# ma921/SOBER

Measured on AMD Instinct MI355X. Metric: recombination-step candidates/sec (N_rec=100000, N_nys=500, d=10, batch=100), higher is better.
Workload: dtype f64

## Files before the change

include/sober_hip.h:

```cpp
#ifndef SOBER_HIP_H
#define SOBER_HIP_H

#include <stdint.h>

#ifdef __cplusplus
extern "C" {
#endif

#define SOBER_ABI_VERSION 7

#define SOBER_KIND_RBF       0
#define SOBER_KIND_MATERN52  1
#define SOBER_KIND_TANIMOTO  2

#define SOBER_E_ARG      -1
#define SOBER_E_DIM      -2
#define SOBER_E_WS       -3
#define SOBER_E_EXCHANGE -5

int sober_abi_version(void);
int sober_diag_build(void);
int sober_reload_switches(void);
int sober_level_job_size(void);
int sober_nystrom_job_size(void);

int sober_padded_dim(int d);
int sober_bit_words(int d);

int sober_mt19937_uniform53(uint8_t* state, int64_t state_bytes, int64_t numel, double* out);
int sober_box_muller(const double* u, int64_t numel, double* out, void* stream);

int sober_scale_points(const double* X, int64_t n, int d, int64_t ldx,
                       const double* lengthscale, int ls_len,
                       double* out, int dt, void* stream);

int sober_scale_points_idx(const double* X, const int32_t* idx, int64_t n, int d, int64_t ldx, const double* lengthscale,
                           int ls_len, double* out, int dt, const double* gather_src, double* gather_out, void* stream);
int sober_pack_bits(const double* X, int64_t n, int d, int64_t ldx,
                    uint64_t* words, int nwords, double* norms, int32_t* bad_flag, void* stream);

int sober_pairwise(int kind, const void* a, const double* a_norm, int64_t m,
                   const void* b, const double* b_norm, const int32_t* idx, int64_t n,
                   int dt, double outputscale, double* out, int64_t ldo, void* stream);

int sober_kernel_matvec(int kind, const void* a, const double* a_norm, const double* v, int64_t m,
                        const void* b, const double* b_norm, int64_t n,
                        int dt, double outputscale, double c0, double* out, void* stream);

int sober_level_reduce(int kind, const void* rows, const double* rows_norm, int n_rows,
                       const void* cand, const double* cand_norm, int dt,
                       const int32_t* idx, int64_t pos0, int64_t count, int S,
                       const double* mu, const double* wmul, double outputscale,
                       int n_chunks, double* partG, int ldg, int col0,
                       double* partTot, int64_t tot_limit, void* stream);
int sober_aug_dim(int d);
int sober_augment_plan(const double* X_nys, int64_t M, int64_t ld_nys, const double* X_obs, int64_t n_obs, int64_t ld_obs,
                       const double* X_cand, int64_t N, int64_t ld_cand, int d, const double* lengthscale, int ls_len,
                       double* center, double* rows_aug, double* cand_aug, int da, void* stream);
int sober_augment_points(const double* X, int64_t n, int d, int64_t ldx, const double* lengthscale,
                         int ls_len, const double* center, int side, double* out, int da, void* stream);
int sober_level_reduce_mfma(int kind, const double* rows, int n_rows, const double* cand, int da,
                            const int32_t* idx, int64_t pos0, int64_t count, int S,
                            const double* mu, const double* wmul, double outputscale,
                            int n_chunks, double* partG, int ldg, int col0,
                            double* partTot, int64_t tot_limit, void* stream);

int64_t sober_nonzero_ws_bytes(int64_t N);
int sober_nonzero_i32(const double* mu, int64_t N, int32_t* idx_out, int64_t* count_out, void* ws, int64_t ws_bytes,
                      void* stream);

int sober_level_chunks(int n_rows, int64_t pos0, int64_t count, int S);
int sober_level_parts_mfma(int n_rows, int64_t pos0, int64_t count, int S);
int sober_level_parts_mfma_cap(int n_rows, int64_t e_total_ub, int S);

int sober_sum_partials(const double* partG, const double* partTot, int n_chunks, int n_rows,
                       int ldg, int S, const double* extraG, const double* extraTot,
                       int n_xchunks, int n_xcols, double* G, int ldo, double* tot, void* stream);

int sober_dgemm(int transa, int transb, int m, int n, int k, double alpha,
                const double* A, int lda, const double* B, int ldb,
                double beta, double* C, int ldc, void* stream);

int sober_barycentres(const double* Xtr, int ldx, int n, int S, const double* tot,
                      double* X_tmp, void* stream);
int sober_dgemm_coldiv_t(int m, int n, int k, const double* A, int lda, const double* B, int ldb, const double* coldiv,
                         double* Ct, int ldct, void* stream);

int sober_level_update(const int32_t* idx_cur, int64_t pos0, int64_t count, int S, int64_t E,
                       const int32_t* keep_rank, const double* w_star, const double* tot,
                       int n_keep, double* mu, int32_t* idx_new, int64_t new_pos0, void* stream);

int sober_scatter_weights(const int32_t* idx_cur, const int32_t* sel, const double* w, int n_sel,
                          double* mu, int64_t* out_idx, void* stream);

int sober_gather_f64(const double* src, const int32_t* idx, int64_t n, double* out, void* stream);
int sober_final_scatter(const int32_t* idx, int n, const int32_t* keep_rank, const double* w_star,
                        int64_t row_offset, double* mu, int64_t* out_idx, double* out_w, void* stream);
int sober_final_commit(const int32_t* idx, int n, const int32_t* keep_rank, const double* w_star, const int32_t* n_keep,
                       int64_t row_offset, double* mu, int64_t N, int64_t* out_idx, double* out_w, void* stream);

int sober_i64_to_i32(const int64_t* in, int64_t n, int32_t* out, void* stream);

int sober_car_pivot_host(double* h_Phi, int N, int m, double* h_mu);
int sober_car_pivot_host_fast(double* h_Phi, int N, int m, double* h_mu);

int sober_car_supported(int N, int m);
int64_t sober_car_ws_bytes(int N, int m);
int sober_car_device(const double* X, int ldx, int N, int m, const double* mu_in,
                     int32_t* keep_rank, double* w_star, int32_t* n_keep, double* mu_out,
                     double* phi_out, void* ws, int64_t ws_bytes, void* stream);
int sober_probe_rcp(const double* x, double* out, int64_t n, void* stream);

#define SOBER_CAR_DEFAULT 0
#define SOBER_CAR_SAFE 1
int sober_car_safe_supported(int N, int m);
int sober_car_giveup_forced(void);
int sober_car_device_ex(const double* X, int ldx, int N, int m, const double* mu_in,
                        int32_t* keep_rank, double* w_star, int32_t* n_keep, double* mu_out,
                        double* phi_out, void* ws, int64_t ws_bytes, int mode, void* stream);
int sober_obj_set_sums(const double* obj, const double* mu, const int32_t* idx, int64_t pos0, int64_t count, int S, int64_t E,
                       double* out, void* stream);
int sober_second_elimination(const double* phi, const double* objp, const double* w1, const int32_t* rank1, int n1,
                             int Nsets, int32_t* keep_rank, double* w_star, int32_t* n_keep, void* stream);
int sober_null_vector_supported(int nfun);
int sober_null_vector(const double* X, int ldx, int Nsets, int nfun, const int32_t* rank1, const int32_t* n_keep1, int n1,
                      double* null_row, int32_t* status, void* stream);
int sober_second_elimination_rows(const double* null_row, const double* obj_row, const double* w1, const int32_t* rank1,
                                  const int32_t* n_keep1, const int32_t* status, int n1, int Nsets, int32_t* keep_rank,
                                  double* w_star, int32_t* n_keep, void* stream);
int sober_obj_set_sums_queued(const double* obj, const double* mu, const int32_t* idx, int S, const int64_t* dR, int64_t R_known,
                              const double* tot, double* xcol, int ldx, double* ocol, void* stream);

int sober_car_mc_supported(int N, int m);
int64_t sober_car_mc_ws_bytes(int N, int m);
int sober_car_mc_device(const double* X, int ldx, int N, int m, const double* mu_in,
                        int32_t* keep_rank, double* w_star, int32_t* n_keep, double* mu_out,
                        double* phi_out, void* ws, int64_t ws_bytes, void* stream);
int sober_car_big_supported(int N, int m);
int64_t sober_car_big_ws_bytes(int N, int m);
int sober_car_big_device(const double* X, int ldx, int N, int m, const double* mu_in,
                         int32_t* keep_rank, double* w_star, int32_t* n_keep, double* mu_out,
                         double* phi_out, void* ws, int64_t ws_bytes, void* stream);
int sober_mc_selftest(const double* in, double* out, void* stream);

int sober_chol_max_n(void);
int sober_nystrom_max_n(void);
int sober_cholesky_probe_batched(const double* src, int n, int ld_src, const double* shifts, int n_shifts,
                                 double* work, int32_t* info, double* min_pivot, void* xinv_ws, int64_t ws_bytes,
                                 void* stream);
int sober_cholesky(double* A, int n, int ld, double shift, int32_t* info, double* min_pivot, void* stream);
int sober_cholesky_inv(double* A, int n, int ld, double shift, int32_t* info, double* min_pivot, double* xinv,
                       void* stream);
int sober_cholesky_inv_ratio(double* A, int n, int ld, double shift, int32_t* info, double* min_pivot, double* xinv,
                             double* ratio_out, void* stream);
int sober_trsm_blocks(const double* Y, int64_t m, int q, int ldy, const double* L, int ldl, const double* Xinv,
                      double* Q, int ldq, void* stream);
int sober_cholesky_probe(const double* src, int n, int ld_src, const double* shifts, int n_shifts,
                         double* work, int32_t* info, void* stream);
int sober_cholesky_probe_piv(const double* src, int n, int ld_src, const double* shifts, int n_shifts,
                             double* work, int32_t* info, double* min_pivot, void* stream);

int64_t sober_cholesky_probe_mc_ws_bytes(int n, int n_shifts);
int sober_cholesky_probe_mc(const double* src, int n, int ld_src, const double* shifts, int n_shifts,
                            double* work, int32_t* info, double* min_pivot, void* ws, int64_t ws_bytes,
                            void* stream);
int sober_abs_sym(const double* C, int n, int ld, double* out, int ldo, int32_t* flag, void* stream);
int sober_abs_sym_dmax(const double* C, int n, int ld, double* out, int ldo, int32_t* flag, double* dmax,
                       void* stream);

int sober_jitter_ladder(double* A, int n, int ld, int k, void* stream);
int sober_jitter_ladder_auto(double* A, int n, int ld, const int32_t* info, int n_rungs, int32_t* k_out,
                             void* stream);

int sober_level_reduce_tani_supported(int dt);
int sober_level_reduce_tani(const void* rows, const double* rows_norm, int n_rows, const void* cand,
                            const double* cand_norm, int dt, const int32_t* idx, int64_t pos0, int64_t count, int S,
                            const double* mu, const double* wmul, double outputscale, int n_chunks, double* partG,
                            int ldg, int col0, double* partTot, int64_t tot_limit, void* stream);

int sober_rank_scatter(const double* X, int ldx, int N, int n, const double* ocol, const int32_t* rank, int n1,
                       double* Xp, double* objp, void* stream);
int sober_set_i64(int64_t* dst, int64_t v, void* stream);

int sober_level_reduce_mfma_queued(int kind, const double* rows, int n_rows, const double* cand, int da,
                                   const int32_t* idx, int64_t count_ub, int S, int S_main, int leftover,
                                   const double* mu, const double* wmul, double outputscale, int n_chunks_ub,
                                   double* partG, int ldg, double* partTot, const int64_t* dR, void* stream);
int sober_level_reduce_mfma_queued_pair(int kind, const double* rows, int n_rows, const double* cand, int da,
                                        const int32_t* idx, int64_t count_ub, int S, int n_xcols, const double* mu,
                                        const double* wmul, double outputscale, int n_chunks_ub, double* partG,
                                        int ldg, double* partTot, int n_xchunks_ub, double* extraG, double* extraTot,
                                        const int64_t* dR, void* stream);
int sober_sum_partials_queued(const double* partG, const double* partTot, int n_rows, int ldg, int S,
                              const double* extraG, const double* extraTot, int n_xcols, double* G, int ldo,
                              double* tot, const int64_t* dR, int chunked, void* stream);
int sober_level_reduce_tani_queued(const void* rows, const double* rows_norm, int n_rows, const void* cand,
                                   const double* cand_norm, int dt, const int32_t* idx, int64_t count_ub, int S,
                                   int S_main, int leftover, const double* mu, const double* wmul, double outputscale,
                                   int n_chunks_ub, double* partG, int ldg, double* partTot, const int64_t* dR,
                                   void* stream);
int sober_level_reduce_tani_queued_pair(const void* rows, const double* rows_norm, int n_rows, const void* cand,
                                        const double* cand_norm, int dt, const int32_t* idx, int64_t count_ub, int S,
                                        int n_xcols, const double* mu, const double* wmul, double outputscale,
                                        int n_chunks_ub, double* partG, int ldg, double* partTot, int n_xchunks_ub,
                                        double* extraG, double* extraTot, const int64_t* dR, void* stream);
int sober_level_chunks_cap(int n_rows, int64_t e_total_ub, int S);
int sober_level_chunks_tani(int n_rows, int64_t pos0, int64_t count, int S);
int sober_level_chunks_tani_cap(int n_rows, int64_t e_total_ub, int S);
int sober_level_update_queued(const int32_t* idx_cur, int64_t R_ub, int S, const int32_t* keep_rank,
                              const double* w_star, const double* tot, double* mu, int32_t* idx_new,
                              const int64_t* dR_cur, int64_t* dR_next, int64_t R_ub_next, void* stream);

int sober_level_class_wpt(int n_rows, int64_t e_total, int S);
int sober_level_class_slots(int wpt);
int sober_level_reduce_mfma_wpt(int kind, const double* rows, int n_rows, const double* cand, int da,
                                const int32_t* idx, int64_t count, int S, const double* mu, const double* wmul,
                                double outputscale, int wpt, int n_chunks, double* partG, int ldg, double* partTot,
                                void* stream);
int sober_class_sum(const double* partG, const double* partTot, int n_chunks, int n_rows, int S, int CL,
                    double* Gc, double* totc, double* G, double* tot, void* stream);
int sober_class_derive_queued(const double* Gc, const double* totc, int n_rows, int S, int CL, const double* scale,
                              const int32_t* sof, double* Gn, double* totn, double* G, double* tot, const int64_t* dR,
                              void* stream);
int sober_level_update_queued_ex(const int32_t* idx_cur, int64_t R_ub, int S, const int32_t* keep_rank,
                                 const double* w_star, const double* tot, double* mu, int32_t* idx_new,
                                 const int64_t* dR_cur, int64_t* dR_next, int64_t R_ub_next, int need_keep,
                                 double* cls_scale, int32_t* cls_sof, int64_t R_known, void* stream);
int sober_level_update_queued_cls(const int32_t* idx_cur, int64_t R_ub, int S, const int32_t* keep_rank,
                                  const double* w_star, const double* tot, double* mu, int32_t* idx_new,
                                  const int64_t* dR_cur, int64_t* dR_next, int64_t R_ub_next, int need_keep,
                                  double* cls_scale, int32_t* cls_sof, void* stream);
#define SOBER_CLASS_MAX_DEPTH 4
int sober_level_class_depth(int variant, int n_rows, int64_t R, int S);

int64_t sober_kmeans_ws_bytes(int64_t N, int d, int K);
int64_t sober_kmeans_stat_offset(int64_t N, int d, int K);
int64_t sober_kmeans_ws_bytes_screened(int64_t N, int d, int K);
int sober_kmeans_lloyd(const double* X, int64_t N, int d, int K, int iters,
                       double* centroids, int32_t* labels, void* ws, int64_t ws_bytes, void* stream);

int sober_predict_fused_supported(int kind, int n_obs, int dt);
int sober_predict_fused(int kind, const void* obs, const double* obs_norm, int n_obs, const void* cand,
                        const double* cand_norm, int64_t N, int dt, double outputscale, const double* W, int ldw,
                        const double* alpha, double c0, double kxx_const, double noise, double* mean_out, double* var_out,
                        double eta, const double* eta_ptr, double* lfi_out, int log_flag, void* stream);
int sober_predict_fused_root(int kind, const void* obs, const double* obs_norm, int n_obs, const void* cand,
                             const double* cand_norm, int64_t N, int dt, double outputscale, const double* St, int ldst,
                             const int32_t* tri_flag, const double* alpha, double c0, double kxx_const, double noise,
                             double* mean_out, double* var_out, double eta, const double* eta_ptr, double* lfi_out, int log_flag,
                             void* stream);
int sober_predict_finish(const double* KX, const double* V, int n_obs, int64_t N, int64_t ld,
                         const double* mean, double kxx_const, const double* norms, double outputscale,
                         double noise, double* var_out, double eta, double* lfi_out, int log_flag,
                         void* stream);

int64_t sober_reduce_ws_bytes(int64_t n);
int sober_cleansing_weights(double* w, int64_t n, double eps, void* ws, int64_t ws_bytes, void* stream);

int sober_wkde_draw(const double* eps, int64_t n, int d, const int32_t* comp, const double* Xobs, int ldx,
                    const double* L, const double* lo, const double* hi, double* x, int32_t* inside,
                    void* stream);

int sober_level_gather(const double* Kmat, int n_rows, int64_t ldk, const int32_t* idx, int64_t pos0,
                       int64_t count, int S, const double* mu, const double* wmul, int n_chunks,
                       double* partG, int ldg, int col0, double* partTot, int64_t tot_limit, void* stream);

int sober_gspace_finish(double* K, const double* corr, int64_t n, int m, int64_t ldk, int64_t ldc,
                        const double* mug_cand, const double* mug_rows, void* stream);

#define SOBER_LEVEL_VALU        0
#define SOBER_LEVEL_MFMA        1
#define SOBER_LEVEL_GATHER      2
#define SOBER_LEVEL_TANI        3
#define SOBER_LEVEL_MAX_CHUNKS  64
#define SOBER_LEVEL_XS          16
typedef struct sober_level_job {
    int32_t variant, kind;
    const void* rows;   const double* rows_norm;
    const void* cand;   const double* cand_norm;
    int32_t n_rows, dim;
    int64_t kmat_ld;
    const double* wmul; double outputscale;
    int32_t S, n;
    const double* P;
    double *partG, *partTot, *extraG, *extraTot;
    double *G, *Xtr, *tot;
    double *X_tmp;
    int32_t* keep_rank;
    double *w_star, *mu_out;
    void* car_ws; int64_t car_ws_bytes;
    int32_t* h_flags;
    void* ev[4];
    const int32_t* idx; int64_t pos0, count, E;
    double* mu;
    int32_t phase;
    int64_t* dR; int64_t* h_dR;
    int32_t car_mode;
    uint64_t ev_used[2];
    int32_t class_depth;
    double* Gc[2]; double* totc[2];
    double* cls_scale; int32_t* cls_sof;
} sober_level_job;
#define SOBER_LEVEL_QUEUE 24
int sober_level_moments(const sober_level_job* job, void* stream);
int sober_level_car(const sober_level_job* job, void* stream);
int sober_level_car_retry(sober_level_job* job, void* stream);
#define SOBER_E_NOPROGRESS -4
int sober_level_loop(sober_level_job* job, int64_t R, int32_t* idx_a, int32_t* idx_b, int first_sums_ready,
                     void** events, int max_levels, int64_t* level_R, int32_t* n_levels, int64_t* R_final,
// ... 90 lines not shown
```

sober_amd/_native.py:

```python
from __future__ import annotations

import ctypes as C
import os
from typing import Optional

import torch

_HERE = os.path.dirname(os.path.abspath(__file__))
LIB_PATH = os.environ.get("SOBER_HIP_LIB") or os.path.join(_HERE, "libsober_hip.so")
ABI_VERSION = 7

KIND_RBF, KIND_MATERN52, KIND_TANIMOTO = 0, 1, 2
KIND_BY_NAME = {"rbf": KIND_RBF, "matern52": KIND_MATERN52, "tanimoto": KIND_TANIMOTO}

_vp, _i32, _i64, _f64 = C.c_void_p, C.c_int, C.c_int64, C.c_double

SIGNATURES = {
    "sober_abi_version": (_i32, []),
    "sober_diag_build": (_i32, []),
    "sober_reload_switches": (_i32, []),
    "sober_level_job_size": (_i32, []),
    "sober_nystrom_job_size": (_i32, []),
    "sober_final_job_size": (_i32, []),
    "sober_set_i64": (_i32, [_vp, _i64, _vp]),
    "sober_rank_scatter": (_i32, [_vp, _i32, _i32, _i32, _vp, _vp, _i32, _vp, _vp, _vp]),
    "sober_plan_rows": (_i32, [_i32, _vp, _i32, _i64, _vp, _i32, _i64, _i32, _vp, _i32, _f64, _vp, _i32, _vp, _i32, _vp,
                               _vp, _vp, _vp, _vp]),
    "sober_level_loop_final": (_i32, [_vp, _vp, _i64, _vp, _vp, _i32, _vp, _i32, _vp, _vp, _vp, _vp, _vp]),
    "sober_padded_dim": (_i32, [_i32]),
    "sober_bit_words": (_i32, [_i32]),
    "sober_scale_points": (_i32, [_vp, _i64, _i32, _i64, _vp, _i32, _vp, _i32, _vp]),
    "sober_augment_plan": (_i32, [_vp, _i64, _i64, _vp, _i64, _i64, _vp, _i64, _i64, _i32, _vp, _i32, _vp, _vp, _vp, _i32, _vp]),
    "sober_scale_points_idx": (_i32, [_vp, _vp, _i64, _i32, _i64, _vp, _i32, _vp, _i32, _vp, _vp, _vp]),
    "sober_pack_bits": (_i32, [_vp, _i64, _i32, _i64, _vp, _i32, _vp, _vp, _vp]),
    "sober_mt19937_uniform53": (_i32, [_vp, _i64, _i64, _vp]),
    "sober_box_muller": (_i32, [_vp, _i64, _vp, _vp]),
    "sober_pairwise": (_i32, [_i32, _vp, _vp, _i64, _vp, _vp, _vp, _i64, _i32, _f64, _vp, _i64, _vp]),
    "sober_kernel_matvec": (_i32, [_i32, _vp, _vp, _vp, _i64, _vp, _vp, _i64, _i32, _f64, _f64, _vp, _vp]),
    "sober_level_reduce": (_i32, [_i32, _vp, _vp, _i32, _vp, _vp, _i32, _vp, _i64, _i64, _i32, _vp, _vp,
                                  _f64, _i32, _vp, _i32, _i32, _vp, _i64, _vp]),
    "sober_nonzero_ws_bytes": (_i64, [_i64]),
    "sober_nonzero_i32": (_i32, [_vp, _i64, _vp, _vp, _vp, _i64, _vp]),
    "sober_dgemm_coldiv_t": (_i32, [_i32, _i32, _i32, _vp, _i32, _vp, _i32, _vp, _vp, _i32, _vp]),
    "sober_level_chunks": (_i32, [_i32, _i64, _i64, _i32]),
    "sober_level_parts_mfma": (_i32, [_i32, _i64, _i64, _i32]),
    "sober_level_parts_mfma_cap": (_i32, [_i32, _i64, _i32]),
    "sober_aug_dim": (_i32, [_i32]),
    "sober_augment_points": (_i32, [_vp, _i64, _i32, _i64, _vp, _i32, _vp, _i32, _vp, _i32, _vp]),
    "sober_level_reduce_mfma": (_i32, [_i32, _vp, _i32, _vp, _i32, _vp, _i64, _i64, _i32, _vp, _vp, _f64, _i32,
                                       _vp, _i32, _i32, _vp, _i64, _vp]),
    "sober_sum_partials": (_i32, [_vp, _vp, _i32, _i32, _i32, _i32, _vp, _vp, _i32, _i32, _vp, _i32, _vp, _vp]),
    "sober_dgemm": (_i32, [_i32, _i32, _i32, _i32, _i32, _f64, _vp, _i32, _vp, _i32, _f64, _vp, _i32, _vp]),
    "sober_barycentres": (_i32, [_vp, _i32, _i32, _i32, _vp, _vp, _vp]),
    "sober_level_update": (_i32, [_vp, _i64, _i64, _i32, _i64, _vp, _vp, _vp, _i32, _vp, _vp, _i64, _vp]),
    "sober_scatter_weights": (_i32, [_vp, _vp, _vp, _i32, _vp, _vp, _vp]),
    "sober_i64_to_i32": (_i32, [_vp, _i64, _vp, _vp]),
    "sober_car_pivot_host": (_i32, [_vp, _i32, _i32, _vp]),
    "sober_car_pivot_host_fast": (_i32, [_vp, _i32, _i32, _vp]),
    "sober_car_supported": (_i32, [_i32, _i32]),
    "sober_car_ws_bytes": (_i64, [_i32, _i32]),
    "sober_car_device": (_i32, [_vp, _i32, _i32, _i32, _vp, _vp, _vp, _vp, _vp, _vp, _vp, _i64, _vp]),
    "sober_probe_rcp": (_i32, [_vp, _vp, _i64, _vp]),
    "sober_second_elimination": (_i32, [_vp, _vp, _vp, _vp, _i32, _i32, _vp, _vp, _vp, _vp]),
    "sober_car_mc_supported": (_i32, [_i32, _i32]),
    "sober_car_mc_ws_bytes": (_i64, [_i32, _i32]),
    "sober_car_mc_device": (_i32, [_vp, _i32, _i32, _i32, _vp, _vp, _vp, _vp, _vp, _vp, _vp, _i64, _vp]),
    "sober_car_big_supported": (_i32, [_i32, _i32]),
    "sober_car_big_ws_bytes": (_i64, [_i32, _i32]),
    "sober_car_big_device": (_i32, [_vp, _i32, _i32, _i32, _vp, _vp, _vp, _vp, _vp, _vp, _vp, _i64, _vp]),
    "sober_car_device_ex": (_i32, [_vp, _i32, _i32, _i32, _vp, _vp, _vp, _vp, _vp, _vp, _vp, _i64, _i32, _vp]),
    "sober_obj_set_sums": (_i32, [_vp, _vp, _vp, _i64, _i64, _i32, _i64, _vp, _vp]),
    "sober_null_vector_supported": (_i32, [_i32]),
    "sober_null_vector": (_i32, [_vp, _i32, _i32, _i32, _vp, _vp, _i32, _vp, _vp, _vp]),
    "sober_second_elimination_rows": (_i32, [_vp, _vp, _vp, _vp, _vp, _vp, _i32, _i32, _vp, _vp, _vp, _vp]),
    "sober_obj_set_sums_queued": (_i32, [_vp, _vp, _vp, _i32, _vp, _i64, _vp, _vp, _i32, _vp, _vp]),
    "sober_obj_job_size": (_i32, []),
    "sober_level_loop_obj": (_i32, [_vp, _vp, _i64, _vp, _vp, _i32, _i32, _vp, _vp, _vp, _vp, _vp]),
    "sober_car_safe_supported": (_i32, [_i32, _i32]),
    "sober_car_giveup_forced": (_i32, []),
    "sober_final_commit": (_i32, [_vp, _i32, _vp, _vp, _vp, _i64, _vp, _i64, _vp, _vp, _vp]),
    "sober_level_car_retry": (_i32, [_vp, _vp]),
    "sober_mc_selftest": (_i32, [_vp, _vp, _vp]),
    "sober_chol_max_n": (_i32, []),
    "sober_nystrom_max_n": (_i32, []),
    "sober_cholesky_probe_batched": (_i32, [_vp, _i32, _i32, _vp, _i32, _vp, _vp, _vp, _vp, _i64, _vp]),
    "sober_cholesky": (_i32, [_vp, _i32, _i32, _f64, _vp, _vp, _vp]),
    "sober_cholesky_inv": (_i32, [_vp, _i32, _i32, _f64, _vp, _vp, _vp, _vp]),
    "sober_cholesky_inv_ratio": (_i32, [_vp, _i32, _i32, _f64, _vp, _vp, _vp, _vp, _vp]),
    "sober_trsm_blocks": (_i32, [_vp, _i64, _i32, _i32, _vp, _i32, _vp, _vp, _i32, _vp]),
    "sober_cholesky_probe": (_i32, [_vp, _i32, _i32, _vp, _i32, _vp, _vp, _vp]),
    "sober_cholesky_probe_piv": (_i32, [_vp, _i32, _i32, _vp, _i32, _vp, _vp, _vp, _vp]),
    "sober_cholesky_probe_mc_ws_bytes": (_i64, [_i32, _i32]),
    "sober_cholesky_probe_mc": (_i32, [_vp, _i32, _i32, _vp, _i32, _vp, _vp, _vp, _vp, _i64, _vp]),
    "sober_abs_sym": (_i32, [_vp, _i32, _i32, _vp, _i32, _vp, _vp]),
    "sober_abs_sym_dmax": (_i32, [_vp, _i32, _i32, _vp, _i32, _vp, _vp, _vp]),
    "sober_jitter_ladder": (_i32, [_vp, _i32, _i32, _i32, _vp]),
    "sober_jitter_ladder_auto": (_i32, [_vp, _i32, _i32, _vp, _i32, _vp, _vp]),
    "sober_kmeans_ws_bytes": (_i64, [_i64, _i32, _i32]),
    "sober_kmeans_stat_offset": (_i64, [_i64, _i32, _i32]),
    "sober_kmeans_ws_bytes_screened": (_i64, [_i64, _i32, _i32]),
    "sober_kmeans_lloyd": (_i32, [_vp, _i64, _i32, _i32, _i32, _vp, _vp, _vp, _i64, _vp]),
    "sober_predict_fused_supported": (_i32, [_i32, _i32, _i32]),
    "sober_predict_fused": (_i32, [_i32, _vp, _vp, _i32, _vp, _vp, _i64, _i32, _f64, _vp, _i32, _vp, _f64, _f64, _f64, _vp, _vp,
                                   _f64, _vp, _vp, _i32, _vp]),
    "sober_predict_fused_root": (_i32, [_i32, _vp, _vp, _i32, _vp, _vp, _i64, _i32, _f64, _vp, _i32, _vp, _vp, _f64, _f64, _f64, _vp,
                                        _vp, _f64, _vp, _vp, _i32, _vp]),
    "sober_predict_finish": (_i32, [_vp, _vp, _i32, _i64, _i64, _vp, _f64, _vp, _f64, _f64, _vp, _f64, _vp, _i32, _vp]),
    "sober_reduce_ws_bytes": (_i64, [_i64]),
    "sober_cleansing_weights": (_i32, [_vp, _i64, _f64, _vp, _i64, _vp]),
    "sober_level_gather": (_i32, [_vp, _i32, _i64, _vp, _i64, _i64, _i32, _vp, _vp, _i32, _vp, _i32, _i32, _vp, _i64,
                                  _vp]),
    "sober_gspace_finish": (_i32, [_vp, _vp, _i64, _i32, _i64, _i64, _vp, _vp, _vp]),
    "sober_wkde_draw": (_i32, [_vp, _i64, _i32, _vp, _vp, _i32, _vp, _vp, _vp, _vp, _vp, _vp]),
    "sober_level_moments": (_i32, [_vp, _vp]),
    "sober_level_car": (_i32, [_vp, _vp]),
    "sober_level_reduce_tani_supported": (_i32, [_i32]),
    "sober_level_reduce_tani": (_i32, [_vp, _vp, _i32, _vp, _vp, _i32, _vp, _i64, _i64, _i32, _vp, _vp, _f64, _i32, _vp,
                                       _i32, _i32, _vp, _i64, _vp]),
    "sober_level_loop_sharded": (_i32, [_vp, _i32, _i32, _vp, _vp, _vp, _i32, _vp, _vp, _i64, _i32, _vp, _vp, _vp, _vp]),
    "sober_rccl_load": (_i32, [C.c_char_p]),
    "sober_rccl_unique_id": (_i32, [_vp]),
    "sober_rccl_comm_init": (_i32, [_vp, _i32, _i32, _vp]),
    "sober_rccl_comm_destroy": (_i32, [_vp]),
    "sober_rccl_allreduce_f64": (_i32, [_vp, _vp, _i64, _vp]),
    "sober_rccl_allreduce_ptr": (_i64, []),
    "sober_peer_region_bytes": (_i64, [_i64]),
    "sober_peer_create": (_i32, [_i32, _i32, _i64, _vp, _vp]),
    "sober_peer_connect": (_i32, [_vp, C.c_char_p]),
    "sober_peer_connect_ptrs": (_i32, [_vp, _vp]),
    "sober_peer_region": (_i64, [_vp]),
    "sober_peer_set_spin_limit": (_i32, [_vp, C.c_uint]),
    "sober_peer_allreduce_f64": (_i32, [_vp, _vp, _i64, _vp]),
    "sober_peer_allreduce_ptr": (_i64, []),
    "sober_peer_status": (_i32, [_vp, _vp, _i64, _vp]),
    "sober_peer_destroy": (_i32, [_vp]),
    "sober_level_reduce_mfma_queued": (_i32, [_i32, _vp, _i32, _vp, _i32, _vp, _i64, _i32, _i32, _i32, _vp, _vp, _f64,
                                              _i32, _vp, _i32, _vp, _vp, _vp]),
    "sober_level_reduce_mfma_queued_pair": (_i32, [_i32, _vp, _i32, _vp, _i32, _vp, _i64, _i32, _i32, _vp, _vp, _f64, _i32,
                                                   _vp, _i32, _vp, _i32, _vp, _vp, _vp, _vp]),
    "sober_sum_partials_queued": (_i32, [_vp, _vp, _i32, _i32, _i32, _vp, _vp, _i32, _vp, _i32, _vp, _vp, _i32, _vp]),
    "sober_level_reduce_tani_queued": (_i32, [_vp, _vp, _i32, _vp, _vp, _i32, _vp, _i64, _i32, _i32, _i32, _vp, _vp, _f64,
                                              _i32, _vp, _i32, _vp, _vp, _vp]),
    "sober_level_reduce_tani_queued_pair": (_i32, [_vp, _vp, _i32, _vp, _vp, _i32, _vp, _i64, _i32, _i32, _vp, _vp, _f64, _i32,
                                                   _vp, _i32, _vp, _i32, _vp, _vp, _vp, _vp]),
    "sober_level_chunks_cap": (_i32, [_i32, _i64, _i32]),
    "sober_level_chunks_tani": (_i32, [_i32, _i64, _i64, _i32]),
    "sober_level_chunks_tani_cap": (_i32, [_i32, _i64, _i32]),
    "sober_level_update_queued": (_i32, [_vp, _i64, _i32, _vp, _vp, _vp, _vp, _vp, _vp, _vp, _i64, _vp]),
    "sober_level_update_queued_ex": (_i32, [_vp, _i64, _i32, _vp, _vp, _vp, _vp, _vp, _vp, _vp, _i64, _i32, _vp, _vp, _i64, _vp]),
    "sober_level_update_queued_cls": (_i32, [_vp, _i64, _i32, _vp, _vp, _vp, _vp, _vp, _vp, _vp, _i64, _i32, _vp, _vp, _vp]),
    "sober_level_class_wpt": (_i32, [_i32, _i64, _i32]),
    "sober_level_class_slots": (_i32, [_i32]),
    "sober_level_class_depth": (_i32, [_i32, _i32, _i64, _i32]),
    "sober_level_reduce_mfma_wpt": (_i32, [_i32, _vp, _i32, _vp, _i32, _vp, _i64, _i32, _vp, _vp, _f64, _i32, _i32, _vp, _i32,
                                           _vp, _vp]),
    "sober_class_sum": (_i32, [_vp, _vp, _i32, _i32, _i32, _i32, _vp, _vp, _vp, _vp, _vp]),
    "sober_class_derive_queued": (_i32, [_vp, _vp, _i32, _i32, _i32, _vp, _vp, _vp, _vp, _vp, _vp, _vp, _vp]),
    "sober_record_event_pair": (_i32, [_vp, _vp, _vp]),
    "sober_set_launch_events": (_i32, [_vp, _vp]),
    "sober_projection": (_i32, [_vp, _i32, _i32, _vp, _vp, _i32, _vp, _vp]),
    "sober_nystrom_flags_bytes": (_i64, [_i32, _i32]),
    "sober_nystrom_basis": (_i32, [_vp, _i32, _vp]),
    "sober_gather_f64": (_i32, [_vp, _vp, _i64, _vp, _vp]),
    "sober_final_scatter": (_i32, [_vp, _i32, _vp, _vp, _i64, _vp, _vp, _vp, _vp]),
    "sober_level_final": (_i32, [_vp, _vp, _vp, _vp, _vp, _i32, _vp, _i32, _i64, _i64, _vp, _vp, _vp, _vp, _vp]),
    "sober_level_final_job": (_i32, [_vp, _vp, _vp, _i32, _vp]),
    "sober_level_loop": (_i32, [_vp, _i64, _vp, _vp, _i32, _vp, _i32, _vp, _vp, _vp, _vp, _vp]),
}

LEVEL_VALU, LEVEL_MFMA, LEVEL_GATHER, LEVEL_TANI = 0, 1, 2, 3
LEVEL_MAX_CHUNKS, LEVEL_XS, LEVEL_QUEUE = 64, 16, 24


class FinalJob(C.Structure):
    _fields_ = [
        ("rows_sc", _vp), ("rows_norm", _vp), ("cand_sc", _vp), ("cand_norm", _vp),
        ("dt", _i32), ("done", _i32), ("N", _i64), ("row_offset", _i64),
        ("K", _vp), ("mu_live", _vp), ("out_idx", _vp), ("out_w", _vp),
        ("cand_raw", _vp), ("ld_raw", _i64), ("d_raw", _i32), ("ls_len", _i32), ("ls", _vp), ("sc_buf", _vp),
    ]


class ObjJob(C.Structure):
    _fields_ = [("obj", _vp), ("X_tmp", _vp), ("ocol", _vp), ("kr1", _vp), ("w1", _vp), ("nk1", _vp), ("null_row", _vp),
                ("status", _vp)]


class NystromJob(C.Structure):
    _fields_ = [
        ("M", _i32), ("s", _i32), ("n_rungs", _i32), ("niter", _i32), ("probe_mc", _i32), ("_pad0", _i32),
        ("G", _vp), ("shifts", _vp), ("R", _vp), ("C", _vp), ("chol_work", _vp),
        ("probe_ws", _vp), ("probe_ws_bytes", _i64),
        ("Y", _vp * 2), ("Gm", _vp), ("xinv", _vp),
        ("flags_block", _vp), ("flags_bytes", _i64), ("h_flags_block", _vp),
        ("Ut", _vp),
        ("T", _vp), ("n_obs", _i32), ("mean_nys", _vp), ("P", _vp),
    ]


class LevelJob(C.Structure):
    _fields_ = [
        ("variant", _i32), ("kind", _i32),
        ("rows", _vp), ("rows_norm", _vp), ("cand", _vp), ("cand_norm", _vp),
        ("n_rows", _i32), ("dim", _i32), ("kmat_ld", _i64),
        ("wmul", _vp), ("outputscale", _f64),
        ("S", _i32), ("n", _i32), ("P", _vp),
        ("partG", _vp), ("partTot", _vp), ("extraG", _vp), ("extraTot", _vp),
        ("G", _vp), ("Xtr", _vp), ("tot", _vp), ("X_tmp", _vp),
        ("keep_rank", _vp), ("w_star", _vp), ("mu_out", _vp),
        ("car_ws", _vp), ("car_ws_bytes", _i64), ("h_flags", _vp),
        ("ev", _vp * 4),
        ("idx", _vp), ("pos0", _i64), ("count", _i64), ("E", _i64), ("mu", _vp),
        ("phase", _i32),
        ("dR", _vp), ("h_dR", _vp),
        ("car_mode", _i32),
        ("ev_used", C.c_uint64 * 2),
        ("class_depth", _i32), ("Gc", _vp * 2), ("totc", _vp * 2), ("cls_scale", _vp), ("cls_sof", _vp),
    ]

E_DIM = -2
E_EXCHANGE = -5
CLASS_MAX_DEPTH = 4
CAR_DEFAULT, CAR_SAFE, CAR_HOST = 0, 1, 2

_lib: Optional[C.CDLL] = None


class SoberHipError(RuntimeError):
    pass


def load() -> C.CDLL:
    global _lib
    if _lib is not None:
        return _lib
    if not os.path.exists(LIB_PATH):
        raise SoberHipError(
            f"{LIB_PATH} not found: build it with `make -C sober_amd/csrc` "
            "(python -c 'import __graft_entry__ as g; g.build()').  sober_amd has no CPU fallback.")
    lib = C.CDLL(LIB_PATH)
    lib.sober_abi_version.restype = _i32
    got = lib.sober_abi_version()
# ... 68 lines not shown

def fused_dim_supported(kind: int, d: int) -> bool:
    r = load().sober_bit_words(d) if kind == KIND_TANIMOTO else load().sober_padded_dim(d)
    return r > 0


def scale_points_idx(X, idx, n, lengthscale, out):
    _req(lengthscale, torch.float64, "lengthscale"); _req(out, torch.float64, "out"); _req(idx, torch.int32, "idx")
    if X.dtype != torch.float64 or X.stride(-1) != 1:
        raise SoberHipError("scale_points_idx: X must be float64 with unit inner stride")
    _check(load().sober_scale_points_idx(X.data_ptr(), idx.data_ptr(), int(n), X.shape[1], X.stride(0), lengthscale.data_ptr(),
                                         lengthscale.numel(), out.data_ptr(), out.shape[1], None, None, _stream(X)),
           "sober_scale_points_idx")


def scale_points(X, lengthscale, out):
    n, d = X.shape
    _req(X, torch.float64, "X"); _req(lengthscale, torch.float64, "lengthscale"); _req(out, torch.float64, "out")
    _check(load().sober_scale_points(X.data_ptr(), n, d, X.stride(0), lengthscale.data_ptr(),
                                     lengthscale.numel(), out.data_ptr(), out.shape[1], _stream(X)),
           "sober_scale_points")


def mt19937_uniform53(state, numel, out):
    _req(state, torch.uint8, "state"); _req(out, torch.float64, "out")
    if state.is_cuda or out.is_cuda or out.numel() < numel + 16:
        raise ValueError("mt19937_uniform53 takes host tensors, out of numel + 16 doubles")
    _check(load().sober_mt19937_uniform53(state.data_ptr(), state.numel(), numel, out.data_ptr()),
           "sober_mt19937_uniform53")


def box_muller(u, numel, out):
    _req(u, torch.float64, "u"); _req(out, torch.float64, "out")
    if u.numel() < numel + 16 or out.numel() < numel:
        raise ValueError("box_muller: u holds numel + 16 uniforms, out numel normals")
    _check(load().sober_box_muller(u.data_ptr(), numel, out.data_ptr(), _stream(out)), "sober_box_muller")


def pack_bits(X, words, norms, bad_flag):
    n, d = X.shape
    _req(X, torch.float64, "X"); _req(words, torch.int64, "words"); _req(norms, torch.float64, "norms")
    _req(bad_flag, torch.int32, "bad_flag")
    _check(load().sober_pack_bits(X.data_ptr(), n, d, X.stride(0), words.data_ptr(), words.shape[1],
                                  norms.data_ptr(), bad_flag.data_ptr(), _stream(X)), "sober_pack_bits")


def rank_scatter(X, n, ocol, rank, n1, Xp, objp):
    _req(X, torch.float64, "X"); _req(ocol, torch.float64, "ocol"); _req(rank, torch.int32, "rank")
    _check(load().sober_rank_scatter(X.data_ptr(), X.stride(0), X.shape[0], n, ocol.data_ptr(), rank.data_ptr(), n1,
                                     Xp.data_ptr(), objp.data_ptr(), _stream(X)), "sober_rank_scatter")


def plan_rows(kind, X_nys, X_obs, lengthscale, outputscale, S_cache, rows, Kall, W, T, G):
    M, d = X_nys.shape
    n_obs = 0 if X_obs is None else X_obs.shape[0]
    for t in (X_nys, X_obs, S_cache, rows, Kall, W, T, G):
        if t is not None and (t.dtype != torch.float64 or t.stride(-1) != 1):
            raise SoberHipError("plan_rows: float64 tensors with unit inner stride")
    _check(load().sober_plan_rows(kind, X_nys.data_ptr(), M, X_nys.stride(0), _ptr(X_obs), n_obs,
                                  X_obs.stride(0) if X_obs is not None else 0, d, lengthscale.data_ptr(),
                                  lengthscale.numel(), float(outputscale), _ptr(S_cache),
                                  S_cache.stride(0) if S_cache is not None else 0, rows.data_ptr(), rows.shape[1],
                                  _ptr(Kall), _ptr(W), _ptr(T), G.data_ptr(), _stream(G)), "sober_plan_rows")


def pairwise(kind, a, a_norm, b, b_norm, idx, n, dt, outputscale, out):
    _check(load().sober_pairwise(kind, a.data_ptr(), _ptr(a_norm), a.shape[0], b.data_ptr(), _ptr(b_norm),
                                 _ptr(idx), n, dt, float(outputscale), out.data_ptr(), out.stride(0),
                                 _stream(out)), "sober_pairwise")


def kernel_matvec(kind, a, a_norm, v, b, b_norm, dt, outputscale, c0, out):
    _check(load().sober_kernel_matvec(kind, a.data_ptr(), _ptr(a_norm), v.data_ptr(), a.shape[0],
                                      b.data_ptr(), _ptr(b_norm), b.shape[0], dt, float(outputscale),
                                      float(c0), out.data_ptr(), _stream(out)), "sober_kernel_matvec")


def nonzero_ws_bytes(N) -> int:
    r = load().sober_nonzero_ws_bytes(N)
    _check(min(int(r), 0), "sober_nonzero_ws_bytes")
    return int(r)


def nonzero_i32(mu, idx_out, count_out, ws):
    _req(mu, torch.float64, "mu"); _req(idx_out, torch.int32, "idx_out"); _req(count_out, torch.int64, "count_out")
    _check(load().sober_nonzero_i32(mu.data_ptr(), mu.numel(), idx_out.data_ptr(), count_out.data_ptr(), ws.data_ptr(),
                                    ws.numel() * ws.element_size(), _stream(mu)), "sober_nonzero_i32")


def level_chunks(n_rows, pos0, count, S) -> int:
    r = load().sober_level_chunks(n_rows, pos0, count, S)
    _check(min(r, 0), "sober_level_chunks")
    return r


def level_parts_mfma(n_rows, pos0, count, S) -> int:
    r = load().sober_level_parts_mfma(n_rows, pos0, count, S)
    _check(min(r, 0), "sober_level_parts_mfma")
    return r


def level_reduce(kind, rows, rows_norm, cand, cand_norm, dt, idx, idx_off, pos0, count, S, mu, wmul,
                 outputscale, n_chunks, partG, ldg, col0, partTot, tot_limit):
    _req(idx, torch.int32, "idx"); _req(mu, torch.float64, "mu")
    _check(load().sober_level_reduce(kind, rows.data_ptr(), _ptr(rows_norm), rows.shape[0], cand.data_ptr(),
                                     _ptr(cand_norm), dt, idx.data_ptr() + 4 * idx_off, pos0, count, S,
                                     mu.data_ptr(), _ptr(wmul), float(outputscale), n_chunks,
                                     partG.data_ptr(), ldg, col0, _ptr(partTot), tot_limit, _stream(mu)),
           "sober_level_reduce")


def aug_dim(d: int) -> int:
    r = load().sober_aug_dim(d)
    return r if r > 0 else -1


def augment_plan(X_nys, X_obs, X_cand, lengthscale, center, rows_aug, cand_aug):
    for t_, nm in ((X_nys, "X_nys"), (X_cand, "X_cand"), (X_obs, "X_obs")):
        if t_ is not None and (t_.dtype != torch.float64 or t_.stride(-1) != 1):
            raise SoberHipError(f"augment_plan: {nm} must be float64 with unit inner stride")
    _req(rows_aug, torch.float64, "rows_aug"); _req(cand_aug, torch.float64, "cand_aug"); _req(center, torch.float64, "center")
    n_obs = 0 if X_obs is None else X_obs.shape[0]
    _check(load().sober_augment_plan(X_nys.data_ptr(), X_nys.shape[0], X_nys.stride(0), _ptr(X_obs), n_obs,
                                     X_obs.stride(0) if n_obs else 0, X_cand.data_ptr(), X_cand.shape[0], X_cand.stride(0),
                                     X_nys.shape[1], lengthscale.data_ptr(), lengthscale.numel(), center.data_ptr(),
                                     rows_aug.data_ptr(), cand_aug.data_ptr(), rows_aug.shape[1], _stream(X_cand)),
           "sober_augment_plan")


def augment_points(X, lengthscale, center, side, out):
    n, d = X.shape
    _req(X, torch.float64, "X"); _req(out, torch.float64, "out"); _req(center, torch.float64, "center")
    _check(load().sober_augment_points(X.data_ptr(), n, d, X.stride(0), lengthscale.data_ptr(),
                                       lengthscale.numel(), center.data_ptr(), side, out.data_ptr(),
                                       out.shape[1], _stream(X)), "sober_augment_points")


def level_reduce_mfma(kind, rows, cand, da, idx, idx_off, pos0, count, S, mu, wmul, outputscale, n_chunks,
                      partG, ldg, col0, partTot, tot_limit):
    _req(idx, torch.int32, "idx"); _req(mu, torch.float64, "mu")
    _check(load().sober_level_reduce_mfma(kind, rows.data_ptr(), rows.shape[0], cand.data_ptr(), da,
                                          idx.data_ptr() + 4 * idx_off, pos0, count, S, mu.data_ptr(),
                                          _ptr(wmul), float(outputscale), n_chunks, partG.data_ptr(), ldg,
                                          col0, _ptr(partTot), tot_limit, _stream(mu)),
           "sober_level_reduce_mfma")


def sum_partials(partG, partTot, n_chunks, n_rows, ldg, S, extraG, extraTot, n_xchunks, n_xcols, G, tot):
    _check(load().sober_sum_partials(partG.data_ptr(), _ptr(partTot), n_chunks, n_rows, ldg, S,
                                     _ptr(extraG), _ptr(extraTot), n_xchunks, n_xcols, G.data_ptr(),
                                     G.stride(0), _ptr(tot), _stream(G)), "sober_sum_partials")


def dgemm(A, B, C_, transa=False, transb=False, alpha=1.0, beta=0.0):
    m, n = C_.shape
    k = A.shape[0] if transa else A.shape[1]
    for t, nm in ((A, "A"), (B, "B"), (C_, "C")):
        if t.dtype != torch.float64 or t.stride(1) != 1:
            raise SoberHipError(f"dgemm {nm}: need float64 with unit inner stride")
    ka = B.shape[1] if transb else B.shape[0]
    ma = A.shape[1] if transa else A.shape[0]
    na = B.shape[0] if transb else B.shape[1]
    if (ma, na, ka) != (m, n, k):
        raise SoberHipError(f"dgemm shape mismatch {A.shape} {B.shape} -> {C_.shape}")
    _check(load().sober_dgemm(int(transa), int(transb), m, n, k, float(alpha), A.data_ptr(), A.stride(0),
                              B.data_ptr(), B.stride(0), float(beta), C_.data_ptr(), C_.stride(0),
                              _stream(C_)), "sober_dgemm")


def barycentres(Xtr, n, S, tot, X_tmp):
    _check(load().sober_barycentres(Xtr.data_ptr(), Xtr.stride(0), n, S, _ptr(tot), X_tmp.data_ptr(),
                                    _stream(X_tmp)), "sober_barycentres")


def level_update(idx_cur, idx_off, pos0, count, S, E, keep_rank, w_star, tot, n_keep, mu, idx_new, new_pos0):
    _check(load().sober_level_update(idx_cur.data_ptr() + 4 * idx_off, pos0, count, S, E,
                                     keep_rank.data_ptr(), w_star.data_ptr(), tot.data_ptr(), n_keep,
                                     mu.data_ptr(), idx_new.data_ptr(), new_pos0, _stream(mu)),
           "sober_level_update")


def scatter_weights(idx_cur, sel, w, n_sel, mu, out_idx):
    _check(load().sober_scatter_weights(idx_cur.data_ptr(), sel.data_ptr(), w.data_ptr(), n_sel,
                                        mu.data_ptr(), out_idx.data_ptr(), _stream(mu)),
           "sober_scatter_weights")


def i64_to_i32(src, dst):
    _check(load().sober_i64_to_i32(src.data_ptr(), src.numel(), dst.data_ptr(), _stream(src)),
           "sober_i64_to_i32")


def car_pivot_host(Phi: torch.Tensor, mu: torch.Tensor, fast=None) -> int:
    if Phi.is_cuda or mu.is_cuda:
        raise SoberHipError("car_pivot_host takes host tensors")
    _req(Phi, torch.float64, "Phi"); _req(mu, torch.float64, "mu")
    N, m = Phi.shape
    fn = load().sober_car_pivot_host_fast if (fast or (fast is None and N > 200)) else load().sober_car_pivot_host
    r = fn(Phi.data_ptr(), N, m, mu.data_ptr())
    _check(min(r, 0), "sober_car_pivot_host")
    return r


_CAR_WS = {}


def car_supported(N: int, m: int) -> bool:
    return bool(load().sober_car_supported(N, m))


def car_safe_supported(N: int, m: int) -> bool:
    return bool(load().sober_car_safe_supported(N, m))


def probe_rcp(x):
    out = torch.empty_like(x)
    _check(load().sober_probe_rcp(x.data_ptr(), out.data_ptr(), x.numel(), _stream(x)), "sober_probe_rcp")
    return out


def car_device(X, mu_in, keep_rank, w_star, n_keep, mu_out, phi_out=None, multi_cu=False, mode=CAR_DEFAULT, big=False):
    N, n = X.shape
    lib = load()
    if mode != CAR_DEFAULT and not multi_cu and not big:
        nbytes = lib.sober_car_ws_bytes(N, n + 1)
        ws = _CAR_WS.get(X.device)
        if ws is None or ws.numel() * 8 < nbytes:
            ws = _CAR_WS[X.device] = torch.empty(max(nbytes // 8, 1), dtype=torch.float64, device=X.device)
        _check(lib.sober_car_device_ex(X.data_ptr(), X.stride(0), N, n + 1, mu_in.data_ptr(), keep_rank.data_ptr(),
                                       w_star.data_ptr(), n_keep.data_ptr(), mu_out.data_ptr(), _ptr(phi_out),
                                       ws.data_ptr(), nbytes, int(mode), _stream(X)), "sober_car_device_ex")
        return
    nbytes = max(lib.sober_car_ws_bytes(N, n + 1), lib.sober_car_mc_ws_bytes(N, n + 1) if multi_cu else 0,
                 lib.sober_car_big_ws_bytes(N, n + 1) if big else 0)
    ws = _CAR_WS.get(X.device)
    if ws is None or ws.numel() * 8 < nbytes:
        ws = torch.empty(max(nbytes // 8, 1), dtype=torch.float64, device=X.device)
        _CAR_WS[X.device] = ws
    fn, name = (lib.sober_car_big_device, "sober_car_big_device") if big else \
        (lib.sober_car_mc_device, "sober_car_mc_device") if multi_cu else (lib.sober_car_device, "sober_car_device")
    _check(fn(X.data_ptr(), X.stride(0), N, n + 1, mu_in.data_ptr(), keep_rank.data_ptr(),
              w_star.data_ptr(), n_keep.data_ptr(), mu_out.data_ptr(), _ptr(phi_out),
              ws.data_ptr(), nbytes, _stream(X)), name)


def obj_set_sums(obj, mu, idx, pos0, count, S, E, out):
    _req(obj, torch.float64, "obj"); _req(mu, torch.float64, "mu"); _req(idx, torch.int32, "idx"); _req(out, torch.float64, "out")
    _check(load().sober_obj_set_sums(obj.data_ptr(), mu.data_ptr(), idx.data_ptr(), int(pos0), int(count), int(S), int(E),
                                     out.data_ptr(), _stream(mu)), "sober_obj_set_sums")


def null_vector(X, nfun, rank1, n_keep1, n1, null_row, status):
    _check(load().sober_null_vector(X.data_ptr(), X.stride(0), X.shape[0], int(nfun), rank1.data_ptr(), n_keep1.data_ptr(),
                                    int(n1), null_row.data_ptr(), status.data_ptr(), _stream(X)), "sober_null_vector")


def second_elimination_rows(null_row, obj_row, w1, rank1, n_keep1, n1, keep_rank, w_star, n_keep, status=None):
    _check(load().sober_second_elimination_rows(null_row.data_ptr(), obj_row.data_ptr(), w1.data_ptr(), rank1.data_ptr(),
                                                n_keep1.data_ptr(), _ptr(status), int(n1), rank1.numel(), keep_rank.data_ptr(),
                                                w_star.data_ptr(), n_keep.data_ptr(), _stream(null_row)),
           "sober_second_elimination_rows")


def level_loop_obj(job, obj_job, R, idx_a, idx_b, first_sums_ready, stream):
    level_R = (_i64 * MAX_LEVELS)()
    n_levels, in_b, R_final = _i32(0), _i32(0), _i64(0)
    _check(load().sober_level_loop_obj(C.addressof(job), C.addressof(obj_job), R, idx_a.data_ptr(), idx_b.data_ptr(),
                                       int(bool(first_sums_ready)), MAX_LEVELS, level_R, C.byref(n_levels), C.byref(R_final),
                                       C.byref(in_b), stream), "sober_level_loop_obj")
    return list(level_R[:n_levels.value]), int(R_final.value), bool(in_b.value)


def second_elimination(phi, objp, w1, rank1, n1, keep_rank, w_star, n_keep):
    _check(load().sober_second_elimination(phi.data_ptr(), objp.data_ptr(), w1.data_ptr(), rank1.data_ptr(), int(n1),
                                           rank1.numel(), keep_rank.data_ptr(), w_star.data_ptr(), n_keep.data_ptr(),
                                           _stream(phi)), "sober_second_elimination")


def mc_selftest(x: torch.Tensor) -> torch.Tensor:
    out = torch.empty(128, dtype=torch.float64, device=x.device)
    _check(load().sober_mc_selftest(x.data_ptr(), out.data_ptr(), _stream(x)), "sober_mc_selftest")
    return out


def chol_max_n() -> int:
    return load().sober_chol_max_n()


def nystrom_max_n() -> int:
    return load().sober_nystrom_max_n()


def cholesky(A, shift, info, min_pivot=None):
    n = A.shape[0]
    _check(load().sober_cholesky(A.data_ptr(), n, A.stride(0), float(shift), info.data_ptr(), _ptr(min_pivot),
                                 _stream(A)), "sober_cholesky")


def cholesky_inv(A, shift, info, min_pivot, xinv, ratio=None):
    n = A.shape[0]
    if xinv.numel() < ((n + 31) // 32) * 1024:
        raise SoberHipError("cholesky_inv: xinv too small")
    _check(load().sober_cholesky_inv_ratio(A.data_ptr(), n, A.stride(0), float(shift), info.data_ptr(), _ptr(min_pivot),
                                           xinv.data_ptr(), _ptr(ratio), _stream(A)), "sober_cholesky_inv")


def trsm_blocks(Y, L, xinv, Q):
    m, q = Y.shape
    _check(load().sober_trsm_blocks(Y.data_ptr(), m, q, Y.stride(0), L.data_ptr(), L.stride(0), xinv.data_ptr(),
                                    Q.data_ptr(), Q.stride(0), _stream(Y)), "sober_trsm_blocks")


def cholesky_probe(src, shifts, work, info, min_pivot=None):
    n = src.shape[0]
    _check(load().sober_cholesky_probe_piv(src.data_ptr(), n, src.stride(0), shifts.data_ptr(), shifts.numel(),
                                           work.data_ptr(), info.data_ptr(), _ptr(min_pivot), _stream(src)),
           "sober_cholesky_probe_piv")


PROBE_NO_VERDICT = -7


def cholesky_probe_mc_ws_bytes(n: int, n_shifts: int) -> int:
    return int(load().sober_cholesky_probe_mc_ws_bytes(n, n_shifts))


def cholesky_probe_mc(src, shifts, work, info, min_pivot, ws):
    n = src.shape[0]
    _check(load().sober_cholesky_probe_mc(src.data_ptr(), n, src.stride(0), shifts.data_ptr(), shifts.numel(),
                                          work.data_ptr(), info.data_ptr(), _ptr(min_pivot), ws.data_ptr(),
                                          ws.numel() * ws.element_size(), _stream(src)), "sober_cholesky_probe_mc")


def abs_sym(C_, out, flag, dmax=None):
    n = C_.shape[0]
    _check(load().sober_abs_sym_dmax(C_.data_ptr(), n, C_.stride(0), out.data_ptr(), out.stride(0), flag.data_ptr(),
                                     _ptr(dmax), _stream(C_)), "sober_abs_sym")


def kmeans_lloyd(X, K, iters, centroids, labels):
    N, d = X.shape
    _req(X, torch.float64, "X"); _req(centroids, torch.float64, "centroids"); _req(labels, torch.int32, "labels")
    nbytes = int(load().sober_kmeans_ws_bytes(N, d, K))
    ws = torch.empty(max(nbytes, 8), dtype=torch.uint8, device=X.device)
    _check(load().sober_kmeans_lloyd(X.data_ptr(), N, d, K, iters, centroids.data_ptr(), labels.data_ptr(),
                                     ws.data_ptr(), nbytes, _stream(X)), "sober_kmeans_lloyd")


def predict_fused_supported(kind: int, n_obs: int, dt: int) -> bool:
    return bool(load().sober_predict_fused_supported(int(kind), int(n_obs), int(dt)))


def predict_fused(kind, obs, obs_norm, cand, cand_norm, n, dt, outputscale, W, alpha, c0, kxx_const, noise, mean_out,
                  var_out, eta=0.0, lfi_out=None, log=False, eta_dev=None, root_tri=None):
    if W.dtype != torch.float64 or W.dim() != 2 or W.stride(1) != 1:
        raise SoberHipError(f"predict_fused: W must be float64 with unit inner stride, got {W.dtype} strides {tuple(W.stride())}")
    if cand.dtype == torch.float64 and (cand.dim() != 2 or cand.stride(1) != 1 or cand.stride(0) != dt):
        raise SoberHipError(f"predict_fused: candidates must be rows of {dt} contiguous float64, got strides {tuple(cand.stride())}")
    for t_, nm in ((alpha, "alpha"), (mean_out, "mean_out"), (var_out, "var_out"), (lfi_out, "lfi_out"), (eta_dev, "eta_dev")):
        if t_ is not None:
            _req(t_, torch.float64, "predict_fused: " + nm)
    if alpha is not None and alpha.numel() != obs.shape[0]:
        raise SoberHipError(f"predict_fused: alpha has {alpha.numel()} entries for {obs.shape[0]} observations")
    if root_tri is not None:
        _req(root_tri, torch.int32, "predict_fused: root_tri")
        if W.shape[0] != W.shape[1] or W.shape[0] != obs.shape[0]:
            raise SoberHipError(f"predict_fused: the root must be {obs.shape[0]} x {obs.shape[0]}, got {tuple(W.shape)}")
        _check(load().sober_predict_fused_root(int(kind), obs.data_ptr(), _ptr(obs_norm), obs.shape[0], cand.data_ptr(),
                                               _ptr(cand_norm), int(n), int(dt), float(outputscale), W.data_ptr(), W.stride(0),
                                               root_tri.data_ptr(), _ptr(alpha), float(c0), float(kxx_const), float(noise),
                                               _ptr(mean_out), var_out.data_ptr(), float(eta), _ptr(eta_dev), _ptr(lfi_out),
                                               int(bool(log)), _stream(cand)), "sober_predict_fused_root")
        return
    _check(load().sober_predict_fused(int(kind), obs.data_ptr(), _ptr(obs_norm), obs.shape[0], cand.data_ptr(),
                                      _ptr(cand_norm), int(n), int(dt), float(outputscale), W.data_ptr(), W.stride(0),
                                      _ptr(alpha), float(c0), float(kxx_const), float(noise), _ptr(mean_out),
                                      var_out.data_ptr(), float(eta), _ptr(eta_dev), _ptr(lfi_out), int(bool(log)),
                                      _stream(cand)),
           "sober_predict_fused")


def predict_finish(KX, V, mean, kxx_const, norms, outputscale, noise, var_out, eta=0.0, lfi_out=None, log=False):
    n_obs, N = KX.shape
    _check(load().sober_predict_finish(KX.data_ptr(), V.data_ptr(), n_obs, N, KX.stride(0), _ptr(mean),
                                       float(kxx_const), _ptr(norms), float(outputscale), float(noise),
                                       var_out.data_ptr(), float(eta), _ptr(lfi_out), int(bool(log)),
                                       _stream(KX)), "sober_predict_finish")


def cleansing_weights(w, eps):
    _req(w, torch.float64, "weights")
    nbytes = load().sober_reduce_ws_bytes(w.numel())
    ws = torch.empty(nbytes // 8 + 1, dtype=torch.float64, device=w.device)
    _check(load().sober_cleansing_weights(w.data_ptr(), w.numel(), float(eps), ws.data_ptr(), nbytes,
                                          _stream(w)), "sober_cleansing_weights")


def wkde_draw(eps, comp, Xobs, L, lo, hi, x, inside):
    n, d = eps.shape
    _check(load().sober_wkde_draw(eps.data_ptr(), n, d, comp.data_ptr(), Xobs.data_ptr(), Xobs.stride(0),
                                  L.data_ptr(), lo.data_ptr() if lo is not None else None,
                                  hi.data_ptr() if hi is not None else None, x.data_ptr(),
                                  inside.data_ptr() if inside is not None else None, _stream(eps)),
           "sober_wkde_draw")


def level_gather(Kmat, idx, idx_off, pos0, count, S, mu, wmul, n_chunks, partG, ldg, col0, partTot, tot_limit):
    _req(idx, torch.int32, "idx"); _req(mu, torch.float64, "mu"); _req(Kmat, torch.float64, "Kmat")
    if Kmat.stride(1) != 1:
        raise SoberHipError("level_gather: Kmat needs unit inner stride")
    _check(load().sober_level_gather(Kmat.data_ptr(), Kmat.shape[1], Kmat.stride(0),
                                     idx.data_ptr() + 4 * idx_off, pos0, count, S, mu.data_ptr(), _ptr(wmul),
                                     n_chunks, partG.data_ptr(), ldg, col0, _ptr(partTot), tot_limit,
                                     _stream(partG)), "sober_level_gather")


def gspace_finish(K, corr, mug_cand, mug_rows):
    n, m = K.shape
    _check(load().sober_gspace_finish(K.data_ptr(), corr.data_ptr(), n, m, K.stride(0), corr.stride(0),
                                      mug_cand.data_ptr(), mug_rows.data_ptr(), _stream(K)), "sober_gspace_finish")


def car_ws_bytes(N: int, m: int) -> int:
    return load().sober_car_ws_bytes(N, m)


def level_moments(job: LevelJob, stream: int):
    _check(load().sober_level_moments(C.addressof(job), stream), "sober_level_moments")


def level_car(job: LevelJob, stream: int):
    _check(load().sober_level_car(C.addressof(job), stream), "sober_level_car")


def level_car_retry(job: LevelJob, stream: int) -> bool:
    rc = load().sober_level_car_retry(C.addressof(job), stream)
    if rc == E_EXCHANGE:
        return False
    _check(rc, "sober_level_car_retry")
    return True


E_NOPROGRESS = -4
MAX_LEVELS = 64


def level_loop(job: LevelJob, R: int, idx_a, idx_b, first_sums_ready: bool, events, stream: int, final: "FinalJob" = None):
    level_R = (_i64 * MAX_LEVELS)()
    n_levels, in_b, R_final = _i32(0), _i32(0), _i64(0)
    ev = None
    if events is not None:
        ev = (_vp * (4 * MAX_LEVELS))(*events)
    if final is not None:
        rc = load().sober_level_loop_final(C.addressof(job), C.addressof(final), R, idx_a.data_ptr(), idx_b.data_ptr(),
                                           int(bool(first_sums_ready)), ev, MAX_LEVELS, level_R, C.byref(n_levels),
                                           C.byref(R_final), C.byref(in_b), stream)
    else:
        rc = load().sober_level_loop(C.addressof(job), R, idx_a.data_ptr(), idx_b.data_ptr(), int(bool(first_sums_ready)),
                                     ev, MAX_LEVELS, level_R, C.byref(n_levels), C.byref(R_final), C.byref(in_b), stream)
    if rc == E_NOPROGRESS:
        raise RuntimeError("recombination made no progress (the Caratheodory step cancelled nothing, "
                           "SOBER/_rchq.py:241-242); the reference would loop forever here")
    if rc != E_EXCHANGE:
# ... 163 lines not shown
```

sober_amd/_ops_nystrom.py:

```python
from __future__ import annotations

import os
import warnings

import torch

from . import _native as nat
from . import _rng
from ._ops_plan import Plan


class _NystromOps:

    NITER = 2

    def nystrom_basis_device(self, p: Plan, s: int, max_iter: int = 10, overlap=None, early=None):
        dev, M = self.device, p.M
        if M > nat.nystrom_max_n() or s > 2 * nat.chol_max_n() or s >= M:
            if s < M:
                self.size_cliff("nystrom", f"N_nys = {M}, batch = {s + 1}: beyond the device Nystrom route (N_nys <= "
                                           f"{nat.nystrom_max_n()}, batch <= {2 * nat.chol_max_n() + 1}); make_cov_psd and svd_lowrank run on host LAPACK "
                                           "instead -- about 5-10x the device route's time for this phase")
            self.gram(p)
            return None
        G = self.gram(p)
        n_r, niter = max_iter + 1, self.NITER
        n_orth2 = 2 * (1 + 2 * niter)
        if getattr(p, "ws", None) is None:
            p.ws = {}
        key = ("nys", M, s, n_r)
        st = self._pin.get(key)
        if st is None:
            f64 = torch.float64
            nbytes = nat.nystrom_flags_bytes(n_r, niter)
            st = self._pin[key] = {
                "job": nat.NystromJob(), "C": torch.empty(M, M, dtype=f64, device=dev),
                "Y0": torch.empty(M, s, dtype=f64, device=dev), "Y1": torch.empty(M, s, dtype=f64, device=dev),
                "Gm": torch.empty(s, s, dtype=f64, device=dev),
                "xinv": torch.empty(((s + 31) // 32) * 1024, dtype=f64, device=dev),
                "flags": torch.empty(nbytes, dtype=torch.uint8, device=dev),
                "h_flags": torch.empty(nbytes, dtype=torch.uint8, pin_memory=True),
                "Ut": torch.empty(s, M, dtype=f64, device=dev),
            }
            skey = ("shifts", n_r)
            if skey not in self._pin:
                self._pin[skey] = torch.tensor([1e-5 * (2 ** k - 1) for k in range(n_r)], dtype=f64, device=dev)
            j = st["job"]
            j.M, j.s, j.n_rungs, j.niter = M, s, n_r, niter
            j.shifts, j.C = self._pin[skey].data_ptr(), st["C"].data_ptr()
            j.Y[0], j.Y[1], j.Gm, j.xinv = st["Y0"].data_ptr(), st["Y1"].data_ptr(), st["Gm"].data_ptr(), st["xinv"].data_ptr()
            j.flags_block, j.flags_bytes, j.h_flags_block = st["flags"].data_ptr(), nbytes, st["h_flags"].data_ptr()
            j.Ut = st["Ut"].data_ptr()
        j = st["job"]
        work = self._buf(p, "chol_work", n_r * M * M)
        j.G, j.chol_work = G.data_ptr(), work.data_ptr()
        j.probe_mc = 1 if (M >= self.PROBE_MC_MIN and n_r <= 16 and self._probe_mc and M <= nat.chol_max_n()) else 0
        if j.probe_mc:
            pws = self._buf_u8(p, "chol_mc_ws", nat.cholesky_probe_mc_ws_bytes(M, n_r))
            j.probe_ws, j.probe_ws_bytes = pws.data_ptr(), pws.numel()
        elif M > nat.chol_max_n():
            pws = self._buf_u8(p, "chol_cb_ws", n_r * 8192)
            j.probe_ws, j.probe_ws_bytes = pws.data_ptr(), pws.numel()
        proj = hasattr(p, "weighted")
        if proj:
            T = p.T
            P = torch.empty(s, p.Mtot if T is not None else M, dtype=torch.float64, device=dev)
            j.T, j.n_obs = nat._ptr(T), (T.shape[1] if T is not None else 0)
            j.mean_nys, j.P = (p.mean_nys.data_ptr() if p.weighted else None), P.data_ptr()
        else:
            j.P = None
        stream = torch.cuda.current_stream(dev)
        nat.nystrom_basis(j, 1, stream.cuda_stream)
        if early is not None:
            early()
        rng_state = torch.get_rng_state()
        R = _rng.device_randn(M, s, dev)
        j.R = R.data_ptr()
        nat.nystrom_basis(j, 2, stream.cuda_stream)
        ev = torch.cuda.Event()
        ev.record(stream)
        Ut = st["Ut"]
        if proj:
            p.P, p.n, p._proj_src = P, s, Ut
        if overlap is not None:
            overlap()
        ev.synchronize()
        hb = st["h_flags"]
        n8 = 8 * (n_r + 1 + n_orth2)
        f64s, i32s = hb[:n8].view(torch.float64), hb[n8:].view(torch.int32)
        piv_h, pivs_rf = f64s[:n_r + 1], f64s[n_r + 1:n_r + 1 + n_orth2]
        flags_h, infos_rf = i32s[:2 + n_r], i32s[2 + n_r:]
        if any(int(v) == nat.PROBE_NO_VERDICT for v in flags_h[2:]):
            self._probe_mc = False
            warnings.warn("sober_amd: the multi-CU Cholesky probe lost contact between its workgroups; "
                          "falling back to one workgroup per rung")
            torch.set_rng_state(rng_state)
            return None
        last = 2 * niter
        if os.environ.get("SOBER_NYSTROM_DEBUG"):
            print("nystrom: pivot ratios of the range finder's blocks", [float(pivs_rf[k + 1]) for k in range(0, n_orth2, 2)])
        single = [k for k in range(0, n_orth2, 2) if k // 2 != last]
        rank_lost = bool((infos_rf != 0).any()) or float(pivs_rf[2 * last + 1]) < 0.5 \
            or any(not (float(pivs_rf[k + 1]) >= self.ORTH1_MIN_RATIO) for k in single)
        if int(flags_h[0]) == 0 or rank_lost or self.ladder_borderline(flags_h[2:], piv_h[:n_r], float(piv_h[n_r])):
            torch.set_rng_state(rng_state)
            return None
        warnings.warn("Estimated covariance matrix was not positive semi-definite. Conveting...")
        return Ut, G

    LADDER_GUARD = 1e-9
    PROBE_MC_MIN = 160

    @classmethod
    def ladder_borderline(cls, info, min_pivot, dmax) -> bool:
        thr = cls.LADDER_GUARD * max(dmax, 0.0)
        ok = [int(v) == 0 for v in info]
        piv = [float(v) for v in min_pivot]
        if not (dmax == dmax) or any(v != v for v in piv):
            return True
        k = ok.index(True) if any(ok) else len(ok)
        if k < len(ok) and piv[k] < thr:
            return True
        if k > 0 and piv[k - 1] > -thr:
            return True
        return False

    def _orth(self, Y, infos, pivs, slot, passes: int = 2):
        q = Y.shape[1]
        for it in range(passes):
            Gm = torch.empty(q, q, dtype=torch.float64, device=self.device)
            nat.dgemm(Y, Y, Gm, transa=True)
            Lc = Gm
            xinv = torch.empty(((q + 31) // 32) * 1024, dtype=torch.float64, device=self.device)
            nat.cholesky_inv(Lc, 0.0, infos[slot + it:slot + it + 1], pivs[slot + it:slot + it + 1], xinv,
                             ratio=pivs[slot + 1:slot + 2] if passes == 1 else None)
            Q = torch.empty_like(Y)
            nat.trsm_blocks(Y, Lc, xinv, Q)
            Y = Q
        return Y

    ORTH1_MIN_RATIO = 1e-10
```

sober_amd/_ops_plan.py:

```python
from __future__ import annotations


import torch

from . import _native as nat
from ._kernel import KernelSpec, PointSet, posterior_mean, prepare_points, woodbury


class Plan:
    _POOL_FIELDS = ("cand", "cand_raw", "cand_aug", "rows_aug", "wmul")

    def __getattr__(self, name):
        if name in Plan._POOL_FIELDS:
            prep = self.__dict__.get("_pool_prep")
            if prep is not None:
                self.__dict__["_pool_prep"] = None
                prep()
                if name in self.__dict__:
                    return self.__dict__[name]
        raise AttributeError(name)



class _PlanOps:

    def build_plan(self, spec: KernelSpec, mode: str, X_nys, X_cand, pool_owner=None) -> Plan:
        p = Plan()
        pool_owner = X_cand if pool_owner is None else pool_owner
        p.spec, p.mode = spec, mode
        p.X_nys_raw, p.X_cand_raw = X_nys, X_cand
        p.kind = nat.KIND_BY_NAME[spec.kind]
        p.M = X_nys.shape[0]
        dev = self.device
        corrected = mode != "kernel"
        p.n_obs = spec.X_obs.shape[0] if corrected else 0
        p.weighted = mode == "weighted_predictive_covariance"
        p.mean_nys = None
        p.T = None
        Xn64 = X_nys.to(torch.float64)
        native_rows = (p.kind != nat.KIND_TANIMOTO and not p.weighted and Xn64.stride(-1) == 1
                       and (not corrected or (spec.X_obs.dtype == torch.float64 and spec.X_obs.stride(-1) == 1
                                              and spec.S_cache.dtype == torch.float64 and spec.S_cache.stride(-1) == 1
                                              and spec.S_cache.dim() == 2
                                              and spec.S_cache.shape[0] == spec.S_cache.shape[1] == spec.X_obs.shape[0])))
        if native_rows:
            f64 = torch.float64
            p.Mtot = p.M + p.n_obs
            dt = nat.padded_dim(X_nys.shape[1], generic=True)
            rows = torch.empty(p.Mtot, dt, dtype=f64, device=dev)
            G = torch.empty(p.M, p.M, dtype=f64, device=dev)
            Kall = W = T = None
            if corrected:
                Kall = torch.empty(p.Mtot, p.M, dtype=f64, device=dev)
                W = torch.empty(p.n_obs, p.n_obs, dtype=f64, device=dev)
                T = torch.empty(p.M, p.n_obs, dtype=f64, device=dev)
            nat.plan_rows(p.kind, Xn64, spec.X_obs if corrected else None, spec.lengthscale, spec.outputscale,
                          spec.S_cache if corrected else None, rows, Kall, W, T, G)
            p.rows = PointSet(rows, None, dt)
            p.T, p._gram = T, G
            if corrected:
                p.Kall = Kall
            stacked = None
        else:
            stacked = torch.cat([Xn64, spec.X_obs], 0) if corrected else X_nys
            p.rows = prepare_points(spec, stacked)
            p.Mtot = len(p.rows)
            if p.weighted:
                p.mean_nys = posterior_mean(spec, p.rows.rows(0, p.M))
            if corrected:
                Kall = torch.empty(p.Mtot, p.M, dtype=torch.float64, device=dev)
                nys = p.rows.rows(0, p.M)
                nat.pairwise(p.kind, p.rows.data, p.rows.norm, nys.data, nys.norm, None, p.M, p.rows.dt,
                             spec.outputscale, Kall)
                p.Kall = Kall
                W = woodbury(spec)
                p.T = torch.empty(p.M, p.n_obs, dtype=torch.float64, device=dev)
                nat.dgemm(Kall[p.M:], W, p.T, transa=True)
        p.da = nat.aug_dim(X_nys.shape[1]) if (p.kind != nat.KIND_TANIMOTO and self.use_mfma) else -1

        def pool_prep():
            Xc64 = X_cand if (X_cand.dtype == torch.float64 and X_cand.stride(-1) == 1) else X_cand.to(torch.float64).contiguous()
            if p.da > 0 and not p.weighted and p.kind != nat.KIND_TANIMOTO and self.lazy_scaled_pool:
                p.cand, p.cand_raw = None, Xc64
            else:
                p.cand = self._packed_pool(spec, X_cand, pool_owner)
                p.cand_raw = None
            p.wmul = self._pool_mean(spec, p.cand, X_cand, pool_owner) if p.weighted else None
            if p.da > 0:
                p.rows_aug = torch.empty(p.Mtot, p.da, dtype=torch.float64, device=dev)
                p.cand_aug = torch.empty(X_cand.shape[0], p.da, dtype=torch.float64, device=dev)
                Xo = spec.X_obs if corrected else None
                if Xn64.shape[1] <= 30 and (Xo is None or (Xo.dtype == torch.float64 and Xo.stride(-1) == 1)):
                    center = torch.empty(Xn64.shape[1], dtype=torch.float64, device=dev)
                    nat.augment_plan(Xn64 if Xn64.stride(-1) == 1 else Xn64.contiguous(), Xo, Xc64, spec.lengthscale, center,
                                     p.rows_aug, p.cand_aug)
                else:
                    st = stacked if stacked is not None else (torch.cat([Xn64, spec.X_obs], 0) if corrected else Xn64)
                    center = Xn64.mean(0).contiguous()
                    nat.augment_points(st.to(torch.float64).contiguous(), spec.lengthscale, center, 0, p.rows_aug)
                    nat.augment_points(Xc64, spec.lengthscale, center, 1, p.cand_aug)
            else:
                p.rows_aug = p.cand_aug = None
        p._pool_prep = pool_prep
        p.P = None
        p.ws = {}
        return p

    def _packed_pool(self, spec, X_cand, owner):
        if spec.kind != "tanimoto":
            return prepare_points(spec, X_cand)
        if not self._shares_storage(X_cand, owner):
            self._pool_cache = None
            return prepare_points(spec, X_cand)
        import weakref
        key = (X_cand.data_ptr(), tuple(X_cand.shape), tuple(X_cand.stride()), X_cand.dtype, X_cand._version,
               owner.data_ptr(), owner._version)
        hit = getattr(self, "_pool_cache", None)
        if hit is not None and hit[0] == key and hit[1]() is owner:
            return hit[2]
        self._pool_cache = None
        pts = prepare_points(spec, X_cand)
        self._pool_cache = (key, weakref.ref(owner), pts)
        return pts

    def _pool_mean(self, spec, cand, X_cand, owner):
        if not self._shares_storage(X_cand, owner):
            self._mean_cache = None
            return posterior_mean(spec, cand)
        key = (X_cand.data_ptr(), tuple(X_cand.shape), tuple(X_cand.stride()), X_cand.dtype, X_cand._version,
               owner.data_ptr(), owner._version,
               id(spec.alpha), spec.alpha._version, id(spec.X_obs), spec.X_obs._version,
               id(spec.lengthscale), spec.lengthscale._version, spec.kind, float(spec.outputscale), float(spec.mean_const))
        hit = getattr(self, "_mean_cache", None)
        if hit is not None and hit[0] == key and hit[1]() is owner and hit[2]() is spec.alpha and hit[3]() is spec.X_obs:
            return hit[4]
        import weakref
        self._mean_cache = None
        out = posterior_mean(spec, cand)
        self._mean_cache = (key, weakref.ref(owner), weakref.ref(spec.alpha), weakref.ref(spec.X_obs), out)
        return out

    @staticmethod
    def _shares_storage(X_cand, owner):
        return (isinstance(owner, torch.Tensor) and owner.device == X_cand.device and owner.dtype == X_cand.dtype
                and owner.data_ptr() == X_cand.data_ptr())

    def clear_cache(self):
        self._pool_cache = None
        self._mean_cache = None

    def gram(self, p: Plan):
        dev = self.device
        G = getattr(p, "_gram", None)
        if G is not None:
            p._gram = None
            return G
        if p.T is None:
            nys = p.rows
            G = torch.empty(p.M, p.M, dtype=torch.float64, device=dev)
            nat.pairwise(p.kind, nys.data, nys.norm, nys.data, nys.norm, None, p.M, nys.dt,
                         p.spec.outputscale, G)
            return G
        G = p.Kall[:p.M].clone()
        nat.dgemm(p.T, p.Kall[p.M:], G, alpha=-1.0, beta=1.0)
        if p.weighted:
            G = p.mean_nys.unsqueeze(1) * G * p.mean_nys.unsqueeze(0)
        return G

    def set_projection(self, p: Plan, U):
        if getattr(p, "_proj_src", None) is U:
            return
        p._proj_src = U
        U = U.to(self.device, torch.float64).contiguous()
        p.n = U.shape[0]
        P = torch.empty(p.n, p.Mtot if p.T is not None else p.M, dtype=torch.float64, device=self.device)
        nat.projection(U, p.mean_nys if p.weighted else None, p.T, P)
        p.P = P
```

sober_amd/csrc/chol.hip:

```cpp
#include "common.hpp"
#include "internal.hpp"

namespace sober {

constexpr int CH_NB = 32;
constexpr int CH_T = 512;
constexpr int CH_LDPP = CH_NB + 4;
constexpr int CH_MAXN = 536;

typedef double ch_double4 __attribute__((ext_vector_type(4)));

constexpr int CH_G = 4;
__device__ double ch_sink[CH_T];
#ifdef CM_STAMPS
__device__ double ch_dbg[2];
#endif

__device__ __forceinline__ double ch_rdlane(double v, int l) {
    return __hiloint2double(__builtin_amdgcn_readlane(__double2hiint(v), l),
                            __builtin_amdgcn_readlane(__double2loint(v), l));
}

template <int NC>
__device__ __attribute__((noinline)) void ch_diag_block_n(double* __restrict__ D, double* __restrict__ Xs, double* __restrict__ s_dinv,
                                              int* __restrict__ s_fail_p, double* __restrict__ s_minp_p, int nb, int kb,
                                              int lane, double* __restrict__ xout) {
    constexpr int LDP = CH_NB + 1;
    int& s_fail = *s_fail_p;
    double& s_minp = *s_minp_p;

            const int i = lane & (CH_NB - 1);
            const bool xh = lane >= CH_NB;
            double v[CH_NB];
#ifdef CM_STAMPS
            const long long dbg0 = wall_clock64();
#endif
#pragma unroll
            for (int c = 0; c < CH_NB; ++c) {
                double dv = D[i * LDP + c];
                asm volatile("" : "+v"(dv));
                v[c] = (xh | (i >= nb)) ? ((c == i) ? 1.0 : 0.0) : dv;
            }
            const bool xw = xout != nullptr && xh;
            double* xo = xw ? xout + (size_t)(kb / CH_NB) * CH_NB * CH_NB : ch_sink;
            const int xo_ld = xw ? CH_NB : 0, xo_i = xw ? i : lane;
            double* const o_base = xh ? Xs + i : D + i * LDP;
            const int o_step = xh ? LDP : 1;
            int fail = 0;
            double minp = s_minp;
#pragma unroll
            for (int j = 0; j < NC; ++j) {
                const double djj = ch_rdlane(v[j], j);
                const bool live = (j < nb) & (fail == 0);
                minp = live ? fmin(minp, djj) : minp;
                fail = (live & !(djj > 0.0)) ? kb + j + 1 : fail;
                double rinv = __builtin_amdgcn_rsq(djj);
                {
                    double h = 0.5 * rinv, e = fma(-(djj * rinv), h, 0.5);
                    rinv = fma(rinv, e, rinv);
                    h = 0.5 * rinv; e = fma(-(djj * rinv), h, 0.5);
                    rinv = fma(rinv, e, rinv);
                }
                double l = djj * rinv;
                l = fma(fma(-l, l, djj), 0.5 * rinv, l);
                const double sc = v[j] * rinv;
                v[j] = xh ? sc : ((i == j) ? l : ((i > j) ? sc : 0.0));
                o_base[j * o_step] = v[j];
                xo[j * xo_ld + xo_i] = v[j];
#pragma unroll
                for (int c = j + 1; c < NC; ++c) {
                    const double lcj = ch_rdlane(v[j], c);
                    v[c] = fma(-v[j], lcj, v[c]);
                }
            }
#pragma unroll
            for (int j = NC; j < CH_NB; ++j) { o_base[j * o_step] = v[j]; xo[j * xo_ld + xo_i] = v[j]; }
            if (lane == 0) { s_fail = fail; s_minp = minp; }
#ifdef CM_STAMPS
            if (lane == 0) { ch_dbg[0] = (double)(wall_clock64() - dbg0); ch_dbg[1] = 0.0; }
#endif
        }

__device__ __forceinline__ void ch_diag_block(double* __restrict__ D, double* __restrict__ Xs, double* __restrict__ s_dinv,
                                              int* __restrict__ s_fail_p, double* __restrict__ s_minp_p, int nb, int kb,
                                              int lane, double* __restrict__ xout) {
    if (nb <= 8) ch_diag_block_n<8>(D, Xs, s_dinv, s_fail_p, s_minp_p, nb, kb, lane, xout);
    else if (nb <= 16) ch_diag_block_n<16>(D, Xs, s_dinv, s_fail_p, s_minp_p, nb, kb, lane, xout);
    else ch_diag_block_n<CH_NB>(D, Xs, s_dinv, s_fail_p, s_minp_p, nb, kb, lane, xout);
}

constexpr int CH_SMALLN = 120;
template <bool SMALL>
__global__ __launch_bounds__(CH_T) void k_chol(double* __restrict__ A, int n, int ld, double shift,
                                              int32_t* __restrict__ info, double* __restrict__ min_pivot,
                                              const double* __restrict__ src, int lds_src,
                                              const double* __restrict__ shifts, double* __restrict__ xout,
                                              double* __restrict__ ratio_out) {
    extern __shared__ double lds[];
    if (src != nullptr) {
        A += (size_t)blockIdx.x * n * ld;
        info += blockIdx.x;
        if (min_pivot) min_pivot += blockIdx.x;
        shift = shifts[blockIdx.x];
        for (int i = threadIdx.x >> 6; i < n; i += CH_T / 64)
            for (int j = threadIdx.x & 63; j <= i; j += 64) A[(size_t)i * ld + j] = src[(size_t)i * lds_src + j];
        __threadfence_block();
        __syncthreads();
    }
    constexpr int LDP = CH_NB + 1;
    double* D = lds;
    double* Xs = lds + CH_NB * LDP;
    constexpr int LDPP = CH_LDPP;
    double* P = lds + 2 * CH_NB * LDP;
    double* const A_glob = A;
    const int ld_glob = ld;
    double* As = nullptr;
    if constexpr (SMALL) {
        As = P + (size_t)(n > CH_NB ? n - CH_NB : 0) * LDPP;
    }
    __shared__ int s_fail;
    __shared__ double s_minp;
    __shared__ double s_dinv[CH_NB];
    const int tid = threadIdx.x, lane = tid & 63, wave = tid >> 6;
    const int li = lane & 15, lk = lane >> 4;
    if (tid == 0) { s_fail = 0; s_minp = __builtin_inf(); }
    __shared__ double s_dm[CH_T / 64];
    if (ratio_out != nullptr) {
        double dl = -__builtin_inf();
        for (int i = tid; i < n; i += CH_T) dl = fmax(dl, A_glob[(size_t)i * ld_glob + i] + shift);
#pragma unroll
        for (int o = 32; o > 0; o >>= 1) dl = fmax(dl, __shfl_xor(dl, o, 64));
        if (lane == 0) s_dm[wave] = dl;
    }
    __syncthreads();
    bool ahead0 = false;
    if constexpr (SMALL) {
        const int nb0 = min(CH_NB, n);
#pragma unroll
        for (int t = tid; t < CH_NB * CH_NB; t += CH_T) {
            const int i = t >> 5, j = t & 31;
            double v = (i < nb0 && j <= i) ? A_glob[(size_t)i * ld_glob + j] : 0.0;
            if (i == j && i < nb0) v += shift;
            D[i * LDP + j] = v;
        }
        __syncthreads();
        if (wave == 0) {
            ch_diag_block(D, Xs, s_dinv, &s_fail, &s_minp, nb0, 0, lane, xout);
        } else {
            for (int i = wave - 1; i < n; i += CH_T / 64 - 1)
                for (int j = lane; j <= i; j += 64) As[i * (n + 1) + j] = A_glob[(size_t)i * ld_glob + j];
        }
        A = As;
        ld = n + 1;
        __syncthreads();
        ahead0 = true;
    }
#ifdef CH_STAMPS
    long long st_t[5] = {0, 0, 0, 0, 0}, st_last = wall_clock64();
#define CH_STAMP(K) { const long long now_ = wall_clock64(); st_t[K] += now_ - st_last; st_last = now_; }
#else
#define CH_STAMP(K)
#endif

    bool ahead = ahead0;
    for (int kb = 0; kb < n; kb += CH_NB) {
        const int nb = min(CH_NB, n - kb);
        const int nr = n - kb - nb;
        if (!ahead) {
#pragma unroll
            for (int t = tid; t < CH_NB * CH_NB; t += CH_T) {
                const int i = t >> 5, j = t & 31;
                double v = (i < nb && j <= i) ? A[(size_t)(kb + i) * ld + kb + j] : 0.0;
                if (i == j && i < nb) v += shift;
                D[i * LDP + j] = v;
            }
            __syncthreads();
            CH_STAMP(0)
            if (wave == 0) ch_diag_block(D, Xs, s_dinv, &s_fail, &s_minp, nb, kb, lane, xout);
            __syncthreads();
            CH_STAMP(1)
        }
        if (s_fail != 0) break;
#pragma unroll
        for (int t = tid; t < CH_NB * CH_NB; t += CH_T) {
            const int i = t >> 5, j = t & 31;
            if (i < nb && j <= i) A[(size_t)(kb + i) * ld + kb + j] = D[i * LDP + j];
        }
        if (nr == 0) break;
        {
            const int ntile = (nr + 15) / 16;
            double af[8], an[8];
            if (wave < ntile) {
                const double* arow = A + (size_t)(kb + nb + min(wave * 16 + li, nr - 1)) * ld + kb;
#pragma unroll
                for (int u = 0; u < 8; ++u) af[u] = arow[min(4 * u + lk, nb - 1)];
            }
            for (int t = wave; t < ntile; t += CH_T / 64) {
                const int r0 = t * 16;
                {
                    const int tn = min(t + CH_T / 64, ntile - 1);
                    const double* arow = A + (size_t)(kb + nb + min(tn * 16 + li, nr - 1)) * ld + kb;
#pragma unroll
                    for (int u = 0; u < 8; ++u) an[u] = arow[min(4 * u + lk, nb - 1)];
                }
                ch_double4 acc0 = (ch_double4){0.0, 0.0, 0.0, 0.0}, acc1 = acc0;
#pragma unroll
                for (int u = 0; u < 8; ++u) {
                    const int k = 4 * u + lk;
                    const double a = (k < nb) ? af[u] : 0.0;
                    acc0 = __builtin_amdgcn_mfma_f64_16x16x4f64(a, Xs[li * LDP + k], acc0, 0, 0, 0);
                    acc1 = __builtin_amdgcn_mfma_f64_16x16x4f64(a, Xs[(16 + li) * LDP + k], acc1, 0, 0, 0);
                }
#pragma unroll
                for (int r = 0; r < 4; ++r) {
                    const int row = r0 + lk + 4 * r;
                    if (row < nr) {
                        P[row * LDPP + li] = acc0[r];
                        P[row * LDPP + 16 + li] = acc1[r];
                    }
                }
#pragma unroll
                for (int u = 0; u < 8; ++u) af[u] = an[u];
            }
        }
        __syncthreads();
        CH_STAMP(2)
        for (int r = tid >> 5; r < nr; r += CH_T / 32) {
            const int j = tid & 31;
            if (j < nb) A[(size_t)(kb + nb + r) * ld + kb + j] = P[r * LDPP + j];
        }
        {
            const int nt = (nr + 15) / 16;
            const int wv = __builtin_amdgcn_readfirstlane(wave);
            const bool look = nt * (nt + 1) / 2 >= 8;
            const int t_step = look ? (wv == 0 ? 1 : CH_T / 64 - 1) : CH_T / 64;
            const int nt_mine = (look && wv == 0) ? min(nt, 2) : nt;
            int ntr = 0, ntc = look ? (wv == 0 ? 0 : 2 + wv) : wv;
            while (ntc > ntr) { ntc -= ntr + 1; ++ntr; }
            int tr[CH_G], tc[CH_G], trn[CH_G], tcn[CH_G];
            double cv[CH_G][4], cn[CH_G][4];
            double* const a22 = A + (size_t)(kb + nb) * ld + kb + nb;
#define CH_TAKE(R, C)                                                       \
            { R = ntr; C = ntc; ntc += t_step; while (ntc > ntr) { ntc -= ntr + 1; ++ntr; } }
#define CH_LOAD(DST, R, C)                                                  \
            _Pragma("unroll") for (int e = 0; e < 4; ++e)                   \
                DST[e] = a22[(size_t)min((R) * 16 + lk + 4 * e, nr - 1) * ld + min((C) * 16 + li, nr - 1)];
#pragma unroll
            for (int g = 0; g < CH_G; ++g) { CH_TAKE(tr[g], tc[g]) CH_LOAD(cv[g], tr[g], tc[g]) }
            while (tr[0] < nt_mine) {
#pragma unroll
                for (int g = 0; g < CH_G; ++g) { CH_TAKE(trn[g], tcn[g]) CH_LOAD(cn[g], trn[g], tcn[g]) }
                ch_double4 acc[CH_G][2];
#pragma unroll
                for (int g = 0; g < CH_G; ++g) {
                    acc[g][0] = (ch_double4){0.0, 0.0, 0.0, 0.0};
                    acc[g][1] = acc[g][0];
                    const int ra = min(tr[g] * 16 + li, nr - 1), rb = min(tc[g] * 16 + li, nr - 1);
#pragma unroll
                    for (int u = 0; u < 8; u += 2) {
                        acc[g][0] = __builtin_amdgcn_mfma_f64_16x16x4f64(P[ra * LDPP + 4 * u + lk],
                                                                         P[rb * LDPP + 4 * u + lk], acc[g][0], 0, 0, 0);
                        acc[g][1] = __builtin_amdgcn_mfma_f64_16x16x4f64(P[ra * LDPP + 4 * u + 4 + lk],
                                                                         P[rb * LDPP + 4 * u + 4 + lk], acc[g][1], 0, 0, 0);
                    }
                }
#pragma unroll
                for (int g = 0; g < CH_G; ++g) {
#pragma unroll
                    for (int e = 0; e < 4; ++e) {
                        const int row = tr[g] * 16 + lk + 4 * e, col = tc[g] * 16 + li;
                        double* dst = (row < nr && col <= row && tr[g] < nt_mine) ? a22 + (size_t)row * ld + col : ch_sink + tid;
                        *dst = cv[g][e] - (acc[g][0][e] + acc[g][1][e]);
                    }
                }
#pragma unroll
                for (int g = 0; g < CH_G; ++g) {
                    tr[g] = trn[g]; tc[g] = tcn[g];
#pragma unroll
                    for (int e = 0; e < 4; ++e) cv[g][e] = cn[g][e];
                }
            }
#undef CH_TAKE
#undef CH_LOAD
            if (look && wave == 0) {
                __builtin_amdgcn_s_waitcnt(0);
                const int kb2 = kb + nb, nb2 = min(CH_NB, n - kb2);
#pragma unroll
                for (int t = lane; t < CH_NB * CH_NB; t += 64) {
                    const int i = t >> 5, j = t & 31;
                    double v = (i < nb2 && j <= i) ? A[(size_t)(kb2 + i) * ld + kb2 + j] : 0.0;
                    if (i == j && i < nb2) v += shift;
                    D[i * LDP + j] = v;
                }
                __builtin_amdgcn_wave_barrier();
                ch_diag_block(D, Xs, s_dinv, &s_fail, &s_minp, nb2, kb2, lane, xout);
            }
            ahead = look;
        }
        __threadfence_block();
        __syncthreads();
        CH_STAMP(3)
    }
    if constexpr (SMALL) {
        __syncthreads();
        for (int i = tid >> 6; i < n; i += CH_T / 64)
            for (int j = tid & 63; j <= i; j += 64) A_glob[(size_t)i * ld_glob + j] = A[i * (n + 1) + j];
    }
#ifdef CH_STAMPS
    {
        CH_STAMP(4)
        if (tid == 0 && n >= 16)
            for (int k = 0; k < 5; ++k) A_glob[8 + k] = (double)st_t[k];
    }
#endif
    if (tid == 0) {
        *info = s_fail;
        if (min_pivot) *min_pivot = s_minp;
        if (ratio_out) {
            double dm = s_dm[0];
#pragma unroll
            for (int w = 1; w < CH_T / 64; ++w) dm = fmax(dm, s_dm[w]);
            *ratio_out = s_minp / dm;
        }
    }
}

constexpr int CM_G = 8;
constexpr int CM_MAXB = (CH_MAXN + CH_NB - 1) / CH_NB;
constexpr unsigned CM_SPIN = 1u << 19;
constexpr unsigned CM_OFF_TICKET = 0, CM_OFF_ERR = 64, CM_HDR = 128;
constexpr unsigned CM_RUNG_BYTES = 1024;
constexpr unsigned CM_OFF_FX = 0, CM_OFF_FP = CM_MAXB * 4, CM_OFF_MP = 768;
static_assert(CM_OFF_FP + CM_MAXB * CM_G * 4 <= CM_OFF_MP && CM_OFF_MP + CM_MAXB * 8 <= CM_RUNG_BYTES, "flag layout");
__device__ __forceinline__ int cm_owner(int j) { const int r = j % (2 * CM_G); return r < CM_G ? r : 2 * CM_G - 1 - r; }
__device__ __forceinline__ int cm_row(int g, int idx) { return (idx >> 1) * 2 * CM_G + ((idx & 1) ? 2 * CM_G - 1 - g : g); }
constexpr int CM_INFO_EXCHANGE = -7;
typedef __amdgpu_buffer_rsrc_t ch_rsrc_t;
typedef unsigned int ch_u32x4 __attribute__((ext_vector_type(4)));

constexpr int CM_POLL = 16 | (int)0x80000000;
__device__ __forceinline__ unsigned cm_poll(ch_rsrc_t rs, unsigned off) {
    unsigned spins = 0, v;
    while ((v = (unsigned)__builtin_amdgcn_raw_buffer_load_b32(rs, off, 0, CM_POLL)) == 0u) {
        if (++spins > CM_SPIN) return 0xffu;
        if ((spins & 255u) == 0u && (unsigned)__builtin_amdgcn_raw_buffer_load_b32(rs, CM_OFF_ERR, 0, CM_POLL) != 0u) return 0xffu;
        __builtin_amdgcn_s_sleep(1);
    }
    return v;
}

__global__ __launch_bounds__(CH_T) void k_chol_mc(double* __restrict__ work, int n, int ld, int32_t* __restrict__ info,
                                                  double* __restrict__ min_pivot, const double* __restrict__ src,
                                                  int lds_src, const double* __restrict__ shifts, int n_rungs,
                                                  unsigned char* ws, unsigned ws_bytes, unsigned x_off) {
    extern __shared__ double lds[];
    constexpr int LDP = CH_NB + 1, LDPP = CH_LDPP;
    double* D = lds;
    double* Xs = lds + CH_NB * LDP;
    double* P = lds + 2 * CH_NB * LDP;
    __shared__ int s_role, s_fail;
    __shared__ double s_minp;
    __shared__ double s_dinv[CH_NB];
    __shared__ unsigned s_flag;
    __shared__ int s_sub;
    int sub_epoch = 0;
    const int tid = threadIdx.x, lane = tid & 63, wave = __builtin_amdgcn_readfirstlane(tid >> 6);
    const int li = lane & 15, lk = lane >> 4;
    const ch_rsrc_t rs = __builtin_amdgcn_make_buffer_rsrc(ws, 0, (int)ws_bytes, 0x00020000);
    if (tid == 0) {
        const unsigned xcc = __builtin_amdgcn_s_getreg(20 | (0 << 6) | (3 << 11)) & 7u;
        const unsigned t = __hip_atomic_fetch_add((unsigned*)(ws + CM_OFF_TICKET) + xcc, 1u, __ATOMIC_RELAXED,
                                                  __HIP_MEMORY_SCOPE_AGENT);
        const unsigned rung = xcc + 8u * (t / CM_G);
        s_role = rung < (unsigned)n_rungs ? (int)(rung * CM_G + t % CM_G) : -1;
        s_fail = 0;
        s_flag = 0u;
        s_sub = 0;
        s_minp = __builtin_inf();
    }
    __syncthreads();
    if (s_role < 0) return;
    const int rung = s_role / CM_G, g = s_role % CM_G;
    const int nblk = (n + CH_NB - 1) / CH_NB;
    if (g >= nblk) return;
    int jmax = g;
    for (int q = 1; cm_row(g, q) < nblk; ++q) jmax = cm_row(g, q);
    double* const A = work + (size_t)rung * n * ld;
    const ch_rsrc_t ra = __builtin_amdgcn_make_buffer_rsrc(A, 0, (int)((size_t)n * ld * sizeof(double)), 0x00020000);
    const double shift = shifts[rung];
    const unsigned fbase = CM_HDR + (unsigned)rung * CM_RUNG_BYTES;
    const unsigned xbase = x_off + (unsigned)rung * CM_MAXB * (CH_NB * CH_NB * 8);
    for (int q = 0; cm_row(g, q) < nblk; ++q) {
        const int j = cm_row(g, q);
        const int r1 = min(n, CH_NB * (j + 1));
        for (int i = CH_NB * j + (tid >> 6); i < r1; i += CH_T / 64)
            for (int c = lane; c <= i; c += 64) A[(size_t)i * ld + c] = src[(size_t)i * lds_src + c];
    }
    __threadfence_block();
    __syncthreads();

#ifdef CM_STAMPS
    long long cs_t[8] = {0, 0, 0, 0, 0, 0, 0, 0}, cs_last = wall_clock64();
#define CM_STAMP(K) { const long long now_ = wall_clock64(); cs_t[K] += now_ - cs_last; cs_last = now_; if (tid == 0 && n >= 480 && k < 16) A[(size_t)g * ld + 300 + 6 * k + K] = (double)now_; }
#else
#define CM_STAMP(K)
#endif
    bool ahead = false;
    int verdict = -1;
    for (int k = 0; k <= jmax; ++k) {
        const int kb = CH_NB * k, nb = min(CH_NB, n - kb);
        const bool own_k = cm_owner(k) == g;
        if (own_k) {
            if (!ahead) {
#pragma unroll
                for (int t = tid; t < CH_NB * CH_NB; t += CH_T) {
                    const int i = t >> 5, j = t & 31;
                    double v = (i < nb && j <= i) ? A[(size_t)(kb + i) * ld + kb + j] : 0.0;
                    if (i == j && i < nb) v += shift;
                    D[i * LDP + j] = v;
                }
                __syncthreads();
                if (wave == 0) ch_diag_block(D, Xs, s_dinv, &s_fail, &s_minp, nb, kb, lane, nullptr);
                __syncthreads();
            }
            if (tid == 0) {
                const double mp = s_minp;
                __builtin_amdgcn_raw_buffer_store_b32(__double2loint(mp), rs, fbase + CM_OFF_MP + 8 * k, 0, 0);
                __builtin_amdgcn_raw_buffer_store_b32(__double2hiint(mp), rs, fbase + CM_OFF_MP + 8 * k + 4, 0, 0);
            }
            if (s_fail != 0 || k == nblk - 1) {
                if (tid == 0) {
                    __builtin_amdgcn_s_waitcnt(0);
                    __builtin_amdgcn_raw_buffer_store_b32(2, rs, fbase + CM_OFF_FX + 4 * k, 0, 0);
                }
                verdict = k;
                break;
            }
            for (int t = tid; t < CH_NB * CH_NB / 2; t += CH_T) {
                const int i = t >> 4, j = (t & 15) * 2;
                ch_u32x4 v;
                v.x = (unsigned)__double2loint(Xs[i * LDP + j]);     v.y = (unsigned)__double2hiint(Xs[i * LDP + j]);
                v.z = (unsigned)__double2loint(Xs[i * LDP + j + 1]); v.w = (unsigned)__double2hiint(Xs[i * LDP + j + 1]);
                __builtin_amdgcn_raw_buffer_store_b128(v, rs, xbase + (unsigned)k * (CH_NB * CH_NB * 8) + (unsigned)t * 16, 0, 0);
            }
            __builtin_amdgcn_s_waitcnt(0);
            __syncthreads();
            if (tid == 0) __builtin_amdgcn_raw_buffer_store_b32(1, rs, fbase + CM_OFF_FX + 4 * k, 0, 0);
        } else {
            if (tid == 0) s_flag = cm_poll(rs, fbase + CM_OFF_FX + 4 * k);
            __syncthreads();
            if (s_flag != 1u) {
                if (s_flag == 0xffu && tid == 0) {
                    __builtin_amdgcn_raw_buffer_store_b32(1, rs, CM_OFF_ERR, 0, 16);
                    info[rung] = CM_INFO_EXCHANGE;
                }
                break;
            }
            for (int t = tid; t < CH_NB * CH_NB / 2; t += CH_T) {
                const int i = t >> 4, j = (t & 15) * 2;
                const ch_u32x4 v = __builtin_amdgcn_raw_buffer_load_b128(rs, xbase + (unsigned)k * (CH_NB * CH_NB * 8) + (unsigned)t * 16, 0, 16);
                Xs[i * LDP + j] = __hiloint2double((int)v.y, (int)v.x);
                Xs[i * LDP + j + 1] = __hiloint2double((int)v.w, (int)v.z);
            }
            __syncthreads();
        }
        CM_STAMP(0)
        ahead = false;
        if (k == jmax) break;
        int i_first = 0;
        while (cm_row(g, i_first) <= k) ++i_first;
        int n_own = 0;
        while (cm_row(g, i_first + n_own) < nblk) ++n_own;
        for (int t = wave; t < 2 * n_own; t += CH_T / 64) {
            const int j = cm_row(g, i_first + (t >> 1)), r0 = CH_NB * j + 16 * (t & 1);
            const double* arow = A + (size_t)min(r0 + li, n - 1) * ld + kb;
            double af[8];
#pragma unroll
// ... 41 lines not shown
                unsigned v = 1u;
                if (jf <= jmax) v = cm_poll(rs, fbase + CM_OFF_FP + 4 * (k * CM_G + o));
                if (v != 1u) s_flag = 0xffu;
            }
        };
        auto gather = [&](int t0, int nthr) {
            for (int cb = k + 1; cb <= jmax; cb += 8)
                for (int gi = t0; gi < CH_NB * CH_NB / 2; gi += nthr) {
                    const int i = gi >> 4, j = (gi & 15) * 2;
                    ch_u32x4 v[8];
#pragma unroll
                    for (int q = 0; q < 8; ++q) {
                        const int c = cb + q, row = min(CH_NB * c + i, n - 1);
                        if (c <= jmax && cm_owner(c) != g)
                            v[q] = __builtin_amdgcn_raw_buffer_load_b128(ra, (unsigned)(((size_t)row * ld + kb + j) * 8), 0, 16);
                    }
#pragma unroll
                    for (int q = 0; q < 8; ++q) {
                        const int c = cb + q, row = CH_NB * c + i;
                        if (c <= jmax && cm_owner(c) != g && row < n) {
                            double* pr = P + (size_t)(row - kb - CH_NB) * LDPP + j;
                            pr[0] = __hiloint2double((int)v[q].y, (int)v[q].x);
                            pr[1] = __hiloint2double((int)v[q].w, (int)v[q].z);
                        }
                    }
                }
        };
        auto walk = [&](int cs0, int wslot, int nwalk) {
            int cs = cs0, ct = wslot;
                int tr[CH_G], tc[CH_G], trn[CH_G], tcn[CH_G];
                double cv[CH_G][4], cn[CH_G][4];
#define CM_TAKE(R, C)                                                                           \
                { while (cs < n_strips && ct > strip_r0(cs) / 16) { ct -= strip_r0(cs) / 16 + 1; ++cs; }   \
                  R = cs < n_strips ? strip_r0(cs) : -1; C = cs < n_strips ? 16 * ct : 0; ct += nwalk; }
#define CM_LOAD(DST, R, C)                                                                      \
                _Pragma("unroll") for (int e = 0; e < 4; ++e)                                   \
                    DST[e] = a22[(size_t)min(max(R, 0) + lk + 4 * e, nr - 1) * ld + min((C) + li, nr - 1)];
#pragma unroll
                for (int q = 0; q < CH_G; ++q) { CM_TAKE(tr[q], tc[q]) CM_LOAD(cv[q], tr[q], tc[q]) }
                while (tr[0] >= 0) {
#pragma unroll
                    for (int q = 0; q < CH_G; ++q) { CM_TAKE(trn[q], tcn[q]) CM_LOAD(cn[q], trn[q], tcn[q]) }
                    ch_double4 acc[CH_G][2];
#pragma unroll
                    for (int q = 0; q < CH_G; ++q) {
                        acc[q][0] = (ch_double4){0.0, 0.0, 0.0, 0.0};
                        acc[q][1] = acc[q][0];
                        const int pa = min(max(tr[q], 0) + li, nr - 1), pb = min(tc[q] + li, nr - 1);
#pragma unroll
                        for (int u = 0; u < 8; u += 2) {
                            acc[q][0] = __builtin_amdgcn_mfma_f64_16x16x4f64(P[pa * LDPP + 4 * u + lk], P[pb * LDPP + 4 * u + lk], acc[q][0], 0, 0, 0);
                            acc[q][1] = __builtin_amdgcn_mfma_f64_16x16x4f64(P[pa * LDPP + 4 * u + 4 + lk], P[pb * LDPP + 4 * u + 4 + lk], acc[q][1], 0, 0, 0);
                        }
                    }
#pragma unroll
                    for (int q = 0; q < CH_G; ++q)
#pragma unroll
                        for (int e = 0; e < 4; ++e) {
                            const int row = tr[q] + lk + 4 * e, col = tc[q] + li;
                            double* dst = (tr[q] >= 0 && row < nr && col <= row) ? a22 + (size_t)row * ld + col : ch_sink + tid;
                            *dst = cv[q][e] - (acc[q][0][e] + acc[q][1][e]);
                        }
#pragma unroll
                    for (int q = 0; q < CH_G; ++q) {
                        tr[q] = trn[q]; tc[q] = tcn[q];
#pragma unroll
                        for (int e = 0; e < 4; ++e) cv[q][e] = cn[q][e];
                    }
                }
#undef CM_TAKE
#undef CM_LOAD
        };
        if (!look) {
            poll_others(tid);
            __syncthreads();
            CM_STAMP(2)
            if (s_flag != 0xffu) gather(tid, CH_T);
            __syncthreads();
            CM_STAMP(3)
            if (s_flag != 0xffu) walk(0, wave, CH_T / 64);
        } else if (wave == 0) {
            __builtin_amdgcn_s_setprio(3);
            const int R0[3] = {0, 16, 16}, C0[3] = {0, 0, 16};
            double cv[3][4];
#pragma unroll
            for (int q = 0; q < 3; ++q)
#pragma unroll
                for (int e = 0; e < 4; ++e)
                    cv[q][e] = a22[(size_t)min(R0[q] + lk + 4 * e, nr - 1) * ld + min(C0[q] + li, nr - 1)];
#pragma unroll
            for (int q = 0; q < 3; ++q) {
                ch_double4 acc0 = (ch_double4){0.0, 0.0, 0.0, 0.0}, acc1 = acc0;
                const int pa = min(R0[q] + li, nr - 1), pb = min(C0[q] + li, nr - 1);
#pragma unroll
                for (int u = 0; u < 8; u += 2) {
                    acc0 = __builtin_amdgcn_mfma_f64_16x16x4f64(P[pa * LDPP + 4 * u + lk], P[pb * LDPP + 4 * u + lk], acc0, 0, 0, 0);
                    acc1 = __builtin_amdgcn_mfma_f64_16x16x4f64(P[pa * LDPP + 4 * u + 4 + lk], P[pb * LDPP + 4 * u + 4 + lk], acc1, 0, 0, 0);
                }
#pragma unroll
                for (int e = 0; e < 4; ++e) {
                    const int row = R0[q] + lk + 4 * e, col = C0[q] + li;
                    double* dst = (row < nr && col <= row) ? a22 + (size_t)row * ld + col : ch_sink + tid;
                    *dst = cv[q][e] - (acc0[e] + acc1[e]);
                }
            }
            __builtin_amdgcn_s_waitcnt(0);
            const int kb2 = kb + CH_NB, nb2 = min(CH_NB, n - kb2);
#pragma unroll
            for (int t = lane; t < CH_NB * CH_NB; t += 64) {
                const int i = t >> 5, j = t & 31;
                double v = (i < nb2 && j <= i) ? A[(size_t)(kb2 + i) * ld + kb2 + j] : 0.0;
                if (i == j && i < nb2) v += shift;
                D[i * LDP + j] = v;
            }
            __builtin_amdgcn_wave_barrier();
            ch_diag_block(D, Xs, s_dinv, &s_fail, &s_minp, nb2, kb2, lane, nullptr);
            __builtin_amdgcn_s_setprio(0);
        } else {
            if (wave == 1) poll_others(lane);
            sub_barrier();
            if (s_flag != 0xffu) gather(tid - 64, CH_T - 64);
            sub_barrier();
            if (s_flag != 0xffu) walk(2, wave - 1, CH_T / 64 - 1);
        }
        CM_STAMP(4)
        ahead = look;
        __threadfence_block();
        __syncthreads();
        CM_STAMP(5)
        if (s_flag == 0xffu) {
            if (tid == 0) {
                __builtin_amdgcn_raw_buffer_store_b32(1, rs, CM_OFF_ERR, 0, 16);
                info[rung] = CM_INFO_EXCHANGE;
            }
            break;
        }
    }
#ifdef CM_STAMPS
    if (tid == 0 && n >= 480) { for (int q = 0; q < 6; ++q) A[(size_t)g * ld + 400 + q] = (double)cs_t[q]; A[(size_t)g * ld + 410] = ch_dbg[0]; A[(size_t)g * ld + 411] = ch_dbg[1]; }
#endif
    if (verdict >= 0 && tid == 0) {
        double mp = s_minp;
        for (int q = 0; q < verdict; ++q) {
            const unsigned lo = (unsigned)__builtin_amdgcn_raw_buffer_load_b32(rs, fbase + CM_OFF_MP + 8 * q, 0, 16);
            const unsigned hi = (unsigned)__builtin_amdgcn_raw_buffer_load_b32(rs, fbase + CM_OFF_MP + 8 * q + 4, 0, 16);
            mp = fmin(mp, __hiloint2double((int)hi, (int)lo));
        }
        info[rung] = s_fail;
        if (min_pivot) min_pivot[rung] = mp;
    }
}

constexpr int TB_WAVES = 2;
__global__ __launch_bounds__(TB_WAVES * 64) void k_trsm_blocks(const double* __restrict__ Y, int64_t m, int q, int ldy,
                                                              const double* __restrict__ L, int ldl,
                                                              const double* __restrict__ Xinv,
                                                              double* __restrict__ Q, int ldq) {
    extern __shared__ double tb_lds[];
    const int lane = threadIdx.x & 63, wave = threadIdx.x >> 6;
    const int li = lane & 15, lk = lane >> 4;
    const int qpad = ((q + 31) / 32) * 32, LS = qpad + 4;
    double* stash = tb_lds + (size_t)wave * (16 * LS + 16 * 36);
    double* tbuf = stash + 16 * LS;
    const int64_t R0 = ((int64_t)blockIdx.x * TB_WAVES + wave) * 16;
    if (R0 >= m) return;
    const int nblk = qpad / 32;
    for (int jb = 0; jb < nblk; ++jb) {
        const int c0 = 32 * jb;
        ch_double4 acc[2];
#pragma unroll
        for (int jt = 0; jt < 2; ++jt)
#pragma unroll
            for (int r = 0; r < 4; ++r) {
                const int64_t row = min(R0 + lk + 4 * r, m - 1);
                const int col = c0 + 16 * jt + li;
                const double v = Y[row * ldy + min(col, q - 1)];
                acc[jt][r] = (col < q) ? v : 0.0;
            }
        for (int kb = 0; kb < jb; ++kb) {
#pragma unroll
            for (int u = 0; u < 8; ++u) {
                const int kc = 32 * kb + 4 * u + lk;
                const double a = -stash[li * LS + kc];
#pragma unroll
                for (int jt = 0; jt < 2; ++jt) {
                    const int lr = c0 + 16 * jt + li;
                    const double b = L[(size_t)min(lr, q - 1) * ldl + kc];
                    acc[jt] = __builtin_amdgcn_mfma_f64_16x16x4f64(a, (lr < q) ? b : 0.0, acc[jt], 0, 0, 0);
                }
            }
        }
#pragma unroll
        for (int jt = 0; jt < 2; ++jt)
#pragma unroll
            for (int r = 0; r < 4; ++r) tbuf[(lk + 4 * r) * 36 + 16 * jt + li] = acc[jt][r];
        __builtin_amdgcn_wave_barrier();
        const double* X = Xinv + (size_t)jb * 32 * 32;
        ch_double4 out[2] = {(ch_double4){0.0, 0.0, 0.0, 0.0}, (ch_double4){0.0, 0.0, 0.0, 0.0}};
#pragma unroll
        for (int u = 0; u < 8; ++u) {
            const double a = tbuf[li * 36 + 4 * u + lk];
#pragma unroll
            for (int jt = 0; jt < 2; ++jt)
                out[jt] = __builtin_amdgcn_mfma_f64_16x16x4f64(a, X[(16 * jt + li) * 32 + 4 * u + lk], out[jt], 0, 0, 0);
        }
        __builtin_amdgcn_wave_barrier();
#pragma unroll
        for (int jt = 0; jt < 2; ++jt)
#pragma unroll
            for (int r = 0; r < 4; ++r) {
                const int64_t row = R0 + lk + 4 * r;
                const int col = c0 + 16 * jt + li;
                stash[(lk + 4 * r) * LS + col] = out[jt][r];
                if (row < m && col < q) Q[row * ldq + col] = out[jt][r];
            }
        __builtin_amdgcn_wave_barrier();
    }
}

__global__ __launch_bounds__(256) void k_abs_sym(const double* __restrict__ C, int n, int ld,
                                                 double* __restrict__ out, int ldo, int32_t* __restrict__ flag,
                                                 unsigned long long* __restrict__ dmax_bits) {
    __shared__ double tm[32][33];
    const int tx = threadIdx.x & 31, ty = threadIdx.x >> 5;
    const int i0 = blockIdx.y * 32, j0 = blockIdx.x * 32;
    for (int r = ty; r < 32; r += 8) {
        const int i = j0 + r, j = i0 + tx;
        tm[r][tx] = (i < n && j < n) ? C[(size_t)i * ld + j] : 0.0;
    }
    __syncthreads();
    bool asym = false;
    const double big = 1.7976931348623157e308;
    for (int r = ty; r < 32; r += 8) {
        const int i = i0 + r, j = j0 + tx;
        if (i < n && j < n) {
            double a = C[(size_t)i * ld + j], b = tm[tx][r];
            asym |= !(a == b);
            a = (a != a) ? 0.0 : fmin(fmax(a, -big), big);
            b = (b != b) ? 0.0 : fmin(fmax(b, -big), big);
            const double v = sqrt(a * b);
            out[(size_t)i * ldo + j] = v;
            if (dmax_bits != nullptr && i == j) atomicMax(dmax_bits, (unsigned long long)__double_as_longlong(v));
        }
    }
    if (__syncthreads_or(asym) && threadIdx.x == 0) atomicOr(flag, 1);
}

__global__ void k_jitter_ladder(double* __restrict__ A, int n, int ld, int k) {
    const int i = blockIdx.x * blockDim.x + threadIdx.x;
    if (i >= n) return;
    double d = A[(size_t)i * ld + i], jit = 1e-5;
    for (int t = 0; t < k; ++t) { d = __dadd_rn(d, jit); jit = __dmul_rn(jit, 2.0); }
    A[(size_t)i * ld + i] = d;
}

__global__ void k_jitter_ladder_auto(double* __restrict__ A, int n, int ld, const int32_t* __restrict__ info,
                                     int n_rungs, int32_t* __restrict__ k_out) {
    const int j = blockIdx.x * blockDim.x + threadIdx.x, i = blockIdx.y;
    int k = 0;
    while (k < n_rungs && info[k] != 0) ++k;
    if (i == 0 && j == 0) *k_out = k;
    if (j >= n) return;
    if (i == j) {
        double d = A[(size_t)i * ld + i], jit = 1e-5;
        for (int t = 0; t < k; ++t) { d = __dadd_rn(d, jit); jit = __dmul_rn(jit, 2.0); }
        A[(size_t)i * ld + i] = d;
    } else if (k == n_rungs) {
        A[(size_t)i * ld + j] = 0.0;
    }
}

}

namespace sober {
__global__ void k_probe_mc_init(uint32_t* __restrict__ ws, int64_t n_words, int32_t* __restrict__ info, int n_info, int32_t value,
                                uint32_t* __restrict__ pre, int64_t n_pre) {
    const int64_t t = (int64_t)blockIdx.x * blockDim.x + threadIdx.x;
    if (t < n_words) ws[t] = 0u;
    if (pre != nullptr) {
        const int64_t i0 = (uint32_t*)info - pre;
        if (t < n_pre && !(t >= i0 && t < i0 + n_info)) pre[t] = 0u;
    }
    if (t < n_info) info[t] = value;
}
}

namespace sober {
constexpr int CB_MAXN = 2048;
constexpr int CB_TILE = 64;

__global__ __launch_bounds__(256) void k_cb_init(double* __restrict__ work, int n, const double* __restrict__ src, int ld_src,
                                                 int32_t* __restrict__ info, double* __restrict__ min_pivot, int n_rungs) {
    const int i = blockIdx.x, rung = blockIdx.y;
    double* A = work + (size_t)rung * n * n;
    for (int c = threadIdx.x; c <= i; c += 256) A[(size_t)i * n + c] = src[(size_t)i * ld_src + c];
    if (i == 0 && threadIdx.x == 0) { info[rung] = 0; if (min_pivot) min_pivot[rung] = __builtin_inf(); }
}

__global__ __launch_bounds__(64) void k_cb_diag(double* __restrict__ work, int n, int kb, const double* __restrict__ shifts,
                                                double* __restrict__ xinv, int32_t* __restrict__ info,
                                                double* __restrict__ min_pivot) {
    constexpr int LDP = CH_NB + 1;
    __shared__ double D[CH_NB * LDP], Xs[CH_NB * LDP], s_dinv[CH_NB];
    __shared__ int s_fail;
    __shared__ double s_minp;
    const int rung = blockIdx.x, lane = threadIdx.x;
    double* A = work + (size_t)rung * n * n;
    const int nb = min(CH_NB, n - kb);
    const double shift = shifts[rung];
#pragma unroll
    for (int t = lane; t < CH_NB * CH_NB; t += 64) {
        const int i = t >> 5, j = t & 31;
        double v = (i < nb && j <= i) ? A[(size_t)(kb + i) * n + kb + j] : 0.0;
        if (i == j && i < nb) v += shift;
        D[i * LDP + j] = v;
    }
    if (lane == 0) { s_fail = 0; s_minp = __builtin_inf(); }
    __syncthreads();
    ch_diag_block(D, Xs, s_dinv, &s_fail, &s_minp, nb, kb, lane, nullptr);
    __syncthreads();
    double* xo = xinv + (size_t)rung * CH_NB * CH_NB;
#pragma unroll
    for (int t = lane; t < CH_NB * CH_NB; t += 64) xo[t] = Xs[(t >> 5) * LDP + (t & 31)];
    if (lane == 0 && info[rung] == 0) {
        if (min_pivot) min_pivot[rung] = fmin(min_pivot[rung], s_minp);
        if (s_fail != 0) info[rung] = s_fail;
    }
}

__global__ __launch_bounds__(256) void k_cb_update(double* __restrict__ work, int n, int kb, const double* __restrict__ xinv) {
    constexpr int LDP = CH_NB + 1, LDPP = CH_LDPP;
    __shared__ double Xs[CH_NB * LDP], Pr[CB_TILE * LDPP], Pc[CB_TILE * LDPP];
    const int rung = blockIdx.y, tid = threadIdx.x, lane = tid & 63, wave = tid >> 6;
    const int li = lane & 15, lk = lane >> 4;
    double* A = work + (size_t)rung * n * n;
    const int base = kb + CH_NB;
    int bi = 0, rest = blockIdx.x;
    while (rest > bi) { rest -= bi + 1; ++bi; }
    const int bj = rest;
    const int R0 = base + CB_TILE * bi, C0 = base + CB_TILE * bj;
    const double* xi = xinv + (size_t)rung * CH_NB * CH_NB;
    for (int t = tid; t < CH_NB * CH_NB; t += 256) Xs[(t >> 5) * LDP + (t & 31)] = xi[t];
    __syncthreads();
#pragma unroll
    for (int side = 0; side < 2; ++side) {
        if (side == 1 && bi == bj) break;
        const int r0 = (side == 0 ? R0 : C0) + 16 * wave;
        const double* arow = A + (size_t)min(r0 + li, n - 1) * n + kb;
        double af[8];
#pragma unroll
        for (int u = 0; u < 8; ++u) af[u] = arow[4 * u + lk];
        ch_double4 acc0 = (ch_double4){0.0, 0.0, 0.0, 0.0}, acc1 = acc0;
#pragma unroll
        for (int u = 0; u < 8; ++u) {
            const int k = 4 * u + lk;
            acc0 = __builtin_amdgcn_mfma_f64_16x16x4f64(af[u], Xs[li * LDP + k], acc0, 0, 0, 0);
            acc1 = __builtin_amdgcn_mfma_f64_16x16x4f64(af[u], Xs[(16 + li) * LDP + k], acc1, 0, 0, 0);
        }
        double* P = side == 0 ? Pr : Pc;
#pragma unroll
        for (int r = 0; r < 4; ++r) {
            const int row = 16 * wave + lk + 4 * r;
            P[row * LDPP + li] = acc0[r];
            P[row * LDPP + 16 + li] = acc1[r];
        }
    }
    __syncthreads();
    const double* Pcol = (bi == bj) ? Pr : Pc;
#pragma unroll
    for (int ct = 0; ct < 4; ++ct) {
        if (bi == bj && ct > wave) break;
        double cv[4];
#pragma unroll
        for (int e = 0; e < 4; ++e)
            cv[e] = A[(size_t)min(R0 + 16 * wave + lk + 4 * e, n - 1) * n + min(C0 + 16 * ct + li, n - 1)];
        ch_double4 acc0 = (ch_double4){0.0, 0.0, 0.0, 0.0}, acc1 = acc0;
        const int pa = 16 * wave + li, pb = 16 * ct + li;
#pragma unroll
        for (int u = 0; u < 8; u += 2) {
            acc0 = __builtin_amdgcn_mfma_f64_16x16x4f64(Pr[pa * LDPP + 4 * u + lk], Pcol[pb * LDPP + 4 * u + lk], acc0, 0, 0, 0);
            acc1 = __builtin_amdgcn_mfma_f64_16x16x4f64(Pr[pa * LDPP + 4 * u + 4 + lk], Pcol[pb * LDPP + 4 * u + 4 + lk], acc1, 0, 0, 0);
        }
#pragma unroll
        for (int e = 0; e < 4; ++e) {
            const int row = R0 + 16 * wave + lk + 4 * e, col = C0 + 16 * ct + li;
            if (row < n && col <= row) A[(size_t)row * n + col] = cv[e] - (acc0[e] + acc1[e]);
        }
    }
}
}

namespace sober {
__global__ void k_orth_merge(int32_t* __restrict__ info, double* __restrict__ piv, double* __restrict__ ratio,
                             const int32_t* __restrict__ info2, const double* __restrict__ piv2, const double* __restrict__ ratio2) {
    if (threadIdx.x != 0 || blockIdx.x != 0) return;
    if (*info == 0) *info = *info2;
    *piv = fmin(*piv, *piv2);
    if (*piv2 != *piv2) *piv = *piv2;
    if (ratio != nullptr) {
        *ratio = fmin(*ratio, *ratio2);
        if (*ratio2 != *ratio2) *ratio = *ratio2;
    }
}
}
int sober::orth_merge(int32_t* info, double* piv, double* ratio, const int32_t* info2, const double* piv2, const double* ratio2,
                      void* stream) {
    if (!info || !piv || !info2 || !piv2 || (ratio && !ratio2)) return SOBER_E_ARG;
    hipLaunchKernelGGL(sober::k_orth_merge, dim3(1), dim3(64), 0, (hipStream_t)stream, info, piv, ratio, info2, piv2, ratio2);
    LAUNCH_CHECK();
    return 0;
}

extern "C" int sober_nystrom_max_n(void) { return sober::CB_MAXN; }

extern "C" int sober_cholesky_probe_batched(const double* src, int n, int ld_src, const double* shifts, int n_shifts,
                                            double* work, int32_t* info, double* min_pivot, void* xinv_ws,
                                            int64_t ws_bytes, void* stream) {
    if (!src || !shifts || !work || !info || !xinv_ws || n <= 0 || ld_src < n || n_shifts <= 0) return SOBER_E_ARG;
    if (n > sober::CB_MAXN || n_shifts > 64) return SOBER_E_DIM;
    if (ws_bytes < (int64_t)n_shifts * sober::CH_NB * sober::CH_NB * 8) return SOBER_E_WS;
    hipStream_t st = (hipStream_t)stream;
    hipLaunchKernelGGL(sober::k_cb_init, dim3(n, n_shifts), dim3(256), 0, st, work, n, src, ld_src, info, min_pivot, n_shifts);
    LAUNCH_CHECK();
    for (int kb = 0; kb < n; kb += sober::CH_NB) {
        hipLaunchKernelGGL(sober::k_cb_diag, dim3(n_shifts), dim3(64), 0, st, work, n, kb, shifts, (double*)xinv_ws, info,
                           min_pivot);
        LAUNCH_CHECK();
        const int rest = n - kb - sober::CH_NB;
        if (rest <= 0) break;
        const int T = (rest + sober::CB_TILE - 1) / sober::CB_TILE;
        hipLaunchKernelGGL(sober::k_cb_update, dim3(T * (T + 1) / 2, n_shifts), dim3(256), 0, st, work, n, kb,
                           (const double*)xinv_ws);
        LAUNCH_CHECK();
    }
    return 0;
}

namespace sober {
}

extern "C" int sober_chol_max_n(void) { return sober::CH_MAXN; }

extern "C" int sober_cholesky_inv_ratio(double* A, int n, int ld, double shift, int32_t* info, double* min_pivot,
                                        double* xinv, double* ratio_out, void* stream);
extern "C" int sober_cholesky_inv(double* A, int n, int ld, double shift, int32_t* info, double* min_pivot,
                                  double* xinv, void* stream) {
    return sober_cholesky_inv_ratio(A, n, ld, shift, info, min_pivot, xinv, nullptr, stream);
}

extern "C" int sober_cholesky_inv_ratio(double* A, int n, int ld, double shift, int32_t* info, double* min_pivot,
                                        double* xinv, double* ratio_out, void* stream) {
    if (!A || !info || n <= 0 || ld < n) return SOBER_E_ARG;
    if (n > sober::CH_MAXN) return SOBER_E_DIM;
    const int nr = n > sober::CH_NB ? n - sober::CH_NB : 0;
    size_t bytes = ((size_t)2 * sober::CH_NB * (sober::CH_NB + 1) + (size_t)nr * sober::CH_LDPP) * sizeof(double);
    static std::atomic<unsigned long long> attr_set{0};
    if (sober_attr_needed(attr_set)) {
        HIP_TRY(hipFuncSetAttribute((const void*)sober::k_chol<false>, hipFuncAttributeMaxDynamicSharedMemorySize,
                                    160 * 1024 - 512));
        HIP_TRY(hipFuncSetAttribute((const void*)sober::k_chol<true>, hipFuncAttributeMaxDynamicSharedMemorySize,
                                    160 * 1024 - 512));
        sober_attr_done(attr_set);
    }
    if (n <= sober::CH_SMALLN) {
        bytes += (size_t)n * (n + 1) * sizeof(double);
        hipLaunchKernelGGL(sober::k_chol<true>, dim3(1), dim3(sober::CH_T), bytes, (hipStream_t)stream, A, n, ld, shift,
                           info, min_pivot, (const double*)nullptr, 0, (const double*)nullptr, xinv, ratio_out);
    } else {
        hipLaunchKernelGGL(sober::k_chol<false>, dim3(1), dim3(sober::CH_T), bytes, (hipStream_t)stream, A, n, ld, shift,
                           info, min_pivot, (const double*)nullptr, 0, (const double*)nullptr, xinv, ratio_out);
    }
    LAUNCH_CHECK();
    return 0;
}

extern "C" int sober_cholesky(double* A, int n, int ld, double shift, int32_t* info, double* min_pivot,
                              void* stream) {
    return sober_cholesky_inv(A, n, ld, shift, info, min_pivot, nullptr, stream);
}

extern "C" int sober_trsm_blocks(const double* Y, int64_t m, int q, int ldy, const double* L, int ldl,
                                 const double* Xinv, double* Q, int ldq, void* stream) {
    if (!Y || !L || !Xinv || !Q || m <= 0 || q <= 0 || q > sober::CH_MAXN || ldy < q || ldl < q || ldq < q) return SOBER_E_ARG;
    const int qpad = ((q + 31) / 32) * 32;
    const size_t bytes = (size_t)sober::TB_WAVES * (16 * (qpad + 4) + 16 * 36) * sizeof(double);
    static std::atomic<unsigned long long> attr_set{0};
    if (sober_attr_needed(attr_set)) {
        HIP_TRY(hipFuncSetAttribute((const void*)sober::k_trsm_blocks, hipFuncAttributeMaxDynamicSharedMemorySize,
                                    160 * 1024 - 512));
        sober_attr_done(attr_set);
    }
    const int64_t row_blocks = (m + 15) / 16;
    hipLaunchKernelGGL(sober::k_trsm_blocks, dim3((unsigned)((row_blocks + sober::TB_WAVES - 1) / sober::TB_WAVES)),
                       dim3(sober::TB_WAVES * 64), bytes, (hipStream_t)stream, Y, m, q, ldy, L, ldl, Xinv, Q, ldq);
    LAUNCH_CHECK();
    return 0;
}

extern "C" int sober_cholesky_probe_piv(const double* src, int n, int ld_src, const double* shifts, int n_shifts,
                                        double* work, int32_t* info, double* min_pivot, void* stream);
extern "C" int sober_cholesky_probe(const double* src, int n, int ld_src, const double* shifts, int n_shifts,
                                    double* work, int32_t* info, void* stream) {
    return sober_cholesky_probe_piv(src, n, ld_src, shifts, n_shifts, work, info, nullptr, stream);
}

extern "C" int sober_cholesky_probe_piv(const double* src, int n, int ld_src, const double* shifts, int n_shifts,
                                        double* work, int32_t* info, double* min_pivot, void* stream) {
    if (!src || !shifts || !work || !info || n <= 0 || ld_src < n || n_shifts <= 0) return SOBER_E_ARG;
    if (n > sober::CH_MAXN) return SOBER_E_DIM;
    const int nr = n > sober::CH_NB ? n - sober::CH_NB : 0;
    const size_t bytes = ((size_t)2 * sober::CH_NB * (sober::CH_NB + 1) + (size_t)nr * sober::CH_LDPP) * sizeof(double);
    HIP_TRY(hipFuncSetAttribute((const void*)sober::k_chol<false>, hipFuncAttributeMaxDynamicSharedMemorySize,
                                160 * 1024 - 512));
    hipLaunchKernelGGL(sober::k_chol<false>, dim3(n_shifts), dim3(sober::CH_T), bytes, (hipStream_t)stream, work, n, n, 0.0,
                       info, min_pivot, src, ld_src, shifts, (double*)nullptr, (double*)nullptr);
    LAUNCH_CHECK();
    return 0;
}

extern "C" int64_t sober_cholesky_probe_mc_ws_bytes(int n, int n_shifts) {
    if (n <= 0 || n_shifts <= 0 || n_shifts > 16 || n > sober::CH_MAXN) return 0;
    const int64_t flags = ((int64_t)sober::CM_HDR + (int64_t)n_shifts * sober::CM_RUNG_BYTES + 255) / 256 * 256;
    return flags + (int64_t)n_shifts * sober::CM_MAXB * sober::CH_NB * sober::CH_NB * 8;
}

int64_t sober::probe_mc_flag_bytes(int n_shifts) {
    return ((int64_t)sober::CM_HDR + (int64_t)n_shifts * sober::CM_RUNG_BYTES + 255) / 256 * 256;
}

int sober::nystrom_flags_init(void* flags_block, int64_t flags_bytes, void* probe_ws, int64_t ws_flag_bytes, int32_t* info,
                              int n_info, void* stream) {
    if (!flags_block || !probe_ws || !info || flags_bytes <= 0 || (flags_bytes & 3) || ws_flag_bytes <= 0 || n_info <= 0)
        return SOBER_E_ARG;
    const int64_t n_pre = flags_bytes / 4, n_ws = ws_flag_bytes / 4;
    const int64_t n = n_pre > n_ws ? n_pre : n_ws;
    hipLaunchKernelGGL(sober::k_probe_mc_init, dim3((unsigned)((n + 255) / 256)), dim3(256), 0, (hipStream_t)stream,
                       (uint32_t*)probe_ws, n_ws, info, n_info, (int32_t)sober::CM_INFO_EXCHANGE, (uint32_t*)flags_block, n_pre);
    LAUNCH_CHECK();
    return 0;
}

int sober::cholesky_probe_mc(const double* src, int n, int ld_src, const double* shifts, int n_shifts, double* work,
                             int32_t* info, double* min_pivot, void* ws, int64_t ws_bytes, bool init, void* stream) {
    if (!src || !shifts || !work || !info || !ws || n <= 0 || ld_src < n || n_shifts <= 0) return SOBER_E_ARG;
    if (n > sober::CH_MAXN || n_shifts > 16) return SOBER_E_DIM;
    const int64_t need = sober_cholesky_probe_mc_ws_bytes(n, n_shifts);
    if (ws_bytes < need || need > 0x7fffffff) return SOBER_E_WS;
    const int64_t flags = sober::probe_mc_flag_bytes(n_shifts);
    const int nr = n > sober::CH_NB ? n - sober::CH_NB : 0;
    const size_t bytes = ((size_t)2 * sober::CH_NB * (sober::CH_NB + 1) + (size_t)nr * sober::CH_LDPP) * sizeof(double);
    static std::atomic<unsigned long long> attr_set{0};
    if (sober_attr_needed(attr_set)) {
        HIP_TRY(hipFuncSetAttribute((const void*)sober::k_chol_mc, hipFuncAttributeMaxDynamicSharedMemorySize,
                                    160 * 1024 - 512));
        sober_attr_done(attr_set);
    }
    if (init) {
        hipLaunchKernelGGL(sober::k_probe_mc_init, dim3((unsigned)((flags / 4 + 255) / 256)), dim3(256), 0, (hipStream_t)stream,
                           (uint32_t*)ws, (int64_t)(flags / 4), info, n_shifts, (int32_t)sober::CM_INFO_EXCHANGE,
                           (uint32_t*)nullptr, (int64_t)0);
        LAUNCH_CHECK();
    }
    const size_t lds_bytes = bytes > (size_t)84 * 1024 ? bytes : (size_t)84 * 1024;
    hipLaunchKernelGGL(sober::k_chol_mc, dim3(256), dim3(sober::CH_T), lds_bytes, (hipStream_t)stream, work, n, n, info,
                       min_pivot, src, ld_src, shifts, n_shifts, (unsigned char*)ws, (unsigned)need, (unsigned)flags);
    LAUNCH_CHECK();
    return 0;
}

extern "C" int sober_cholesky_probe_mc(const double* src, int n, int ld_src, const double* shifts, int n_shifts,
                                       double* work, int32_t* info, double* min_pivot, void* ws, int64_t ws_bytes,
                                       void* stream) {
    return sober::cholesky_probe_mc(src, n, ld_src, shifts, n_shifts, work, info, min_pivot, ws, ws_bytes, true, stream);
}

extern "C" int sober_abs_sym_dmax(const double* C, int n, int ld, double* out, int ldo, int32_t* flag, double* dmax,
                                  void* stream) {
    if (!C || !out || !flag || n <= 0 || ld < n || ldo < n || n > 65535) return SOBER_E_ARG;
    hipLaunchKernelGGL(sober::k_abs_sym, dim3((n + 31) / 32, (n + 31) / 32), dim3(256), 0, (hipStream_t)stream, C, n,
                       ld, out, ldo, flag, (unsigned long long*)dmax);
    LAUNCH_CHECK();
    return 0;
}

extern "C" int sober_abs_sym(const double* C, int n, int ld, double* out, int ldo, int32_t* flag, void* stream) {
    return sober_abs_sym_dmax(C, n, ld, out, ldo, flag, nullptr, stream);
}

extern "C" int sober_jitter_ladder(double* A, int n, int ld, int k, void* stream) {
    if (!A || n <= 0 || ld < n || k < 0) return SOBER_E_ARG;
    if (k == 0) return 0;
    hipLaunchKernelGGL(sober::k_jitter_ladder, dim3((n + 255) / 256), dim3(256), 0, (hipStream_t)stream, A, n, ld, k);
    LAUNCH_CHECK();
    return 0;
}

extern "C" int sober_jitter_ladder_auto(double* A, int n, int ld, const int32_t* info, int n_rungs, int32_t* k_out,
                                        void* stream) {
    if (!A || !info || !k_out || n <= 0 || ld < n || n_rungs <= 0) return SOBER_E_ARG;
    hipLaunchKernelGGL(sober::k_jitter_ladder_auto, dim3((n + 255) / 256, n), dim3(256), 0, (hipStream_t)stream, A, n,
                       ld, info, n_rungs, k_out);
    LAUNCH_CHECK();
    return 0;
}
```

sober_amd/csrc/dgemm.hip:

```cpp
#include "common.hpp"

namespace sober {

typedef double double4_t __attribute__((ext_vector_type(4)));

__device__ __forceinline__ double ld_op(const double* M, int ld, int trans, int r, int c, int R, int C) {
    const bool ok = (r < R) & (c < C);
    const int rc = min(r, R - 1), cc = min(c, C - 1);
    const double v = trans ? M[(size_t)cc * ld + rc] : M[(size_t)rc * ld + cc];
    return ok ? v : 0.0;
}

template <int SPLIT>
__global__ __launch_bounds__(256) void k_dgemm(int transa, int transb, int m, int n, int k,
                                               double alpha, const double* __restrict__ A, int lda,
                                               const double* __restrict__ B, int ldb, double beta,
                                               double* __restrict__ C, int ldc,
                                               const double* __restrict__ coldiv, double* __restrict__ Ct, int ldct) {
    __shared__ double red[SPLIT == 4 ? 3 * 256 : 1];
    const int wave = threadIdx.x >> 6, lane = threadIdx.x & 63;
    int i0, j0, kbeg, kend;
    if constexpr (SPLIT == 4) {
        i0 = blockIdx.y * 16;
        j0 = blockIdx.x * 16;
        const int kq = (((k + 3) / 4) + 15) / 16 * 16;
        kbeg = min(wave * kq, k);
        kend = min(kbeg + kq, k);
    } else {
        i0 = blockIdx.y * 32 + (wave >> 1) * 16;
        j0 = blockIdx.x * 32 + (wave & 1) * 16;
        kbeg = 0;
        kend = k;
        if (i0 >= m || j0 >= n) return;
    }
    const int li = lane & 15, lk = lane >> 4;

    double4_t acc = (double4_t){0.0, 0.0, 0.0, 0.0};
    double af[4], bf[4], an[4], bn[4];
#define DG_LOAD(AF, BF, K0)                                                                   \
    _Pragma("unroll") for (int u = 0; u < 4; ++u) {                                           \
        AF[u] = ld_op(A, lda, transa, i0 + li, (K0) + 4 * u + lk, m, kend);                   \
        BF[u] = ld_op(B, ldb, transb, (K0) + 4 * u + lk, j0 + li, kend, n);                   \
    }
    DG_LOAD(af, bf, kbeg)
    for (int k0 = kbeg; k0 < kend; k0 += 16) {
        DG_LOAD(an, bn, k0 + 16)
#pragma unroll
        for (int u = 0; u < 4; ++u)
            acc = __builtin_amdgcn_mfma_f64_16x16x4f64(af[u], bf[u], acc, 0, 0, 0);
#pragma unroll
        for (int u = 0; u < 4; ++u) { af[u] = an[u]; bf[u] = bn[u]; }
    }
#undef DG_LOAD
    if constexpr (SPLIT == 4) {
        if (wave > 0) {
#pragma unroll
            for (int r = 0; r < 4; ++r) red[(wave - 1) * 256 + r * 64 + lane] = acc[r];
        }
        __syncthreads();
        if (wave > 0) return;
#pragma unroll
        for (int r = 0; r < 4; ++r) acc[r] = ((acc[r] + red[r * 64 + lane]) + red[256 + r * 64 + lane]) + red[512 + r * 64 + lane];
    }
#pragma unroll
    for (int r = 0; r < 4; ++r) {
        const int row = i0 + lk + 4 * r;
        const int col = j0 + li;
        if (row < m && col < n) {
            const double v = alpha * acc[r];
            if (Ct != nullptr) {
                Ct[(size_t)col * ldct + row] = coldiv ? v / coldiv[col] : v;
            } else {
                double* c = C + (size_t)row * ldc + col;
                *c = (beta == 0.0) ? v : fma(beta, *c, v);
            }
        }
    }
}

}

extern "C" int sober_dgemm(int transa, int transb, int m, int n, int k, double alpha, const double* A,
                           int lda, const double* B, int ldb, double beta, double* C, int ldc,
                           void* stream) {
    if (!A || !B || !C || m <= 0 || n <= 0 || k <= 0) return SOBER_E_ARG;
    if (lda < (transa ? m : k) || ldb < (transb ? k : n) || ldc < n) return SOBER_E_ARG;
    const long tiles = (long)((n + 15) / 16) * ((m + 15) / 16);
    if (tiles <= 2048 && k >= 64) {
        dim3 grid((n + 15) / 16, (m + 15) / 16);
        hipLaunchKernelGGL(sober::k_dgemm<4>, grid, dim3(256), 0, (hipStream_t)stream, transa, transb, m, n, k,
                           alpha, A, lda, B, ldb, beta, C, ldc, (const double*)nullptr, (double*)nullptr, 0);
    } else {
        dim3 grid((n + 31) / 32, (m + 31) / 32);
        hipLaunchKernelGGL(sober::k_dgemm<1>, grid, dim3(256), 0, (hipStream_t)stream, transa, transb, m, n, k,
                           alpha, A, lda, B, ldb, beta, C, ldc, (const double*)nullptr, (double*)nullptr, 0);
    }
    LAUNCH_CHECK();
    return 0;
}

extern "C" int sober_dgemm_coldiv_t(int m, int n, int k, const double* A, int lda, const double* B, int ldb,
                                    const double* coldiv, double* Ct, int ldct, void* stream) {
    if (!A || !B || !Ct || m <= 0 || n <= 0 || k <= 0 || lda < k || ldb < n || ldct < m) return SOBER_E_ARG;
    const long tiles = (long)((n + 15) / 16) * ((m + 15) / 16);
    if (tiles <= 2048 && k >= 64) {
        dim3 grid((n + 15) / 16, (m + 15) / 16);
        hipLaunchKernelGGL(sober::k_dgemm<4>, grid, dim3(256), 0, (hipStream_t)stream, 0, 0, m, n, k, 1.0, A, lda, B, ldb,
                           0.0, (double*)nullptr, 0, coldiv, Ct, ldct);
    } else {
        dim3 grid((n + 31) / 32, (m + 31) / 32);
        hipLaunchKernelGGL(sober::k_dgemm<1>, grid, dim3(256), 0, (hipStream_t)stream, 0, 0, m, n, k, 1.0, A, lda, B, ldb,
                           0.0, (double*)nullptr, 0, coldiv, Ct, ldct);
    }
    LAUNCH_CHECK();
    return 0;
}
```

sober_amd/csrc/internal.hpp:

```cpp
#pragma once
#include <cstdint>

namespace sober {

int scale_points2(const double* Xa, int64_t na, int64_t lda, const double* Xb, int64_t nb, int64_t ldb, int d,
                  const double* lengthscale, int ls_len, double* out, int dt, void* stream);

int transpose_projection(const double* Q, int s, int M, const double* mean, double* Ut, double* P, int ldp, void* stream);

int64_t probe_mc_flag_bytes(int n_shifts);
int nystrom_flags_init(void* flags_block, int64_t flags_bytes, void* probe_ws, int64_t ws_flag_bytes, int32_t* info,
                       int n_info, void* stream);
int cholesky_probe_mc(const double* src, int n, int ld_src, const double* shifts, int n_shifts, double* work, int32_t* info,
                      double* min_pivot, void* ws, int64_t ws_bytes, bool init, void* stream);

int orth_merge(int32_t* info, double* piv, double* ratio, const int32_t* info2, const double* piv2, const double* ratio2, void* stream);

}
```

sober_amd/csrc/nystrom_exec.cpp:

```cpp
#include <hip/hip_runtime.h>

#include "../../include/sober_hip.h"
#include "internal.hpp"

extern "C" int sober_nystrom_job_size(void) { return (int)sizeof(sober_nystrom_job); }

#define NX_TRY(call)                 \
    do {                             \
        const int rc_ = (call);      \
        if (rc_ != 0) return rc_;    \
    } while (0)
#define NX_HIP(call)                                   \
    do {                                               \
        const hipError_t e_ = (call);                  \
        if (e_ != hipSuccess) return (int)e_;          \
    } while (0)

extern "C" int64_t sober_nystrom_flags_bytes(int n_rungs, int niter) {
    const int64_t n_orth2 = 2 * (1 + 2 * (int64_t)niter);
    return 8 * (n_rungs + 1 + n_orth2) + 4 * (2 + n_rungs + n_orth2);
}

static int nx_orth_halves(const sober_nystrom_job* j, double* Y, double* O, int32_t* info, double* piv, double* ratio, void* stream) {
    const int M = j->M, s = j->s, s1 = (s + 1) / 2, s2 = s - s1;
    double* G1 = j->Gm;
    double* W = j->Gm + (size_t)s1 * s1;
    double* tail = j->xinv + (size_t)((s + 31) / 32 - 1) * 1024;
    double *piv2 = tail, *ratio2 = tail + 1;
    int32_t* info2 = (int32_t*)(tail + 2);
    NX_TRY(sober_dgemm(1, 0, s1, s1, M, 1.0, Y, s, Y, s, 0.0, G1, s1, stream));
    NX_TRY(sober_cholesky_inv_ratio(G1, s1, s1, 0.0, info, piv, j->xinv, ratio, stream));
    NX_TRY(sober_trsm_blocks(Y, M, s1, s, G1, s1, j->xinv, O, s, stream));
    NX_TRY(sober_dgemm(1, 0, s1, s2, M, 1.0, O, s, Y + s1, s, 0.0, W, s2, stream));
    NX_TRY(sober_dgemm(0, 0, M, s2, s1, -1.0, O, s, W, s2, 1.0, Y + s1, s, stream));
    NX_TRY(sober_dgemm(1, 0, s2, s2, M, 1.0, Y + s1, s, Y + s1, s, 0.0, G1, s2, stream));
    NX_TRY(sober_cholesky_inv_ratio(G1, s2, s2, 0.0, info2, piv2, j->xinv, ratio ? ratio2 : nullptr, stream));
    NX_TRY(sober_trsm_blocks(Y + s1, M, s2, s, G1, s2, j->xinv, O + s1, s, stream));
    return sober::orth_merge(info, piv, ratio, info2, piv2, ratio ? ratio2 : nullptr, stream);
}

static int nx_orth(const sober_nystrom_job* j, double** Y, double** other, int32_t* infos, double* pivs, int slot,
                   int passes, void* stream) {
    const int M = j->M, s = j->s;
    for (int it = 0; it < passes; ++it) {
        if (s > sober_chol_max_n()) {
            NX_TRY(nx_orth_halves(j, *Y, *other, infos + slot + it, pivs + slot + it, passes == 1 ? pivs + slot + 1 : nullptr, stream));
        } else {
            NX_TRY(sober_dgemm(1, 0, s, s, M, 1.0, *Y, s, *Y, s, 0.0, j->Gm, s, stream));
            NX_TRY(sober_cholesky_inv_ratio(j->Gm, s, s, 0.0, infos + slot + it, pivs + slot + it, j->xinv,
                                            passes == 1 ? pivs + slot + 1 : nullptr, stream));
            NX_TRY(sober_trsm_blocks(*Y, M, s, s, j->Gm, s, j->xinv, *other, s, stream));
        }
        double* t = *Y; *Y = *other; *other = t;
    }
    return 0;
}

extern "C" int sober_nystrom_basis(const sober_nystrom_job* j, int phase, void* stream) {
    if (phase < 0 || phase > 2) return SOBER_E_ARG;
    if (!j || !j->G || !j->shifts || (!j->R && phase != 1) || !j->C || !j->chol_work || !j->Y[0] || !j->Y[1] || !j->Gm ||
        !j->xinv || !j->flags_block || !j->h_flags_block || !j->Ut)
        return SOBER_E_ARG;
    const int M = j->M, s = j->s, n_r = j->n_rungs, niter = j->niter;
    if (M <= 0 || s <= 0 || s >= M || s > 2 * sober_chol_max_n() || n_r <= 0 || n_r > 64 || niter < 0 || niter > 8) return SOBER_E_ARG;
    if (M > sober_nystrom_max_n()) return SOBER_E_DIM;
    if (j->flags_bytes < sober_nystrom_flags_bytes(n_r, niter)) return SOBER_E_WS;
    hipStream_t st = (hipStream_t)stream;
    const int n_orth2 = 2 * (1 + 2 * niter);
    double* pivots = (double*)j->flags_block;
    double* pivs_rf = pivots + n_r + 1;
    int32_t* flags = (int32_t*)(pivs_rf + n_orth2);
    int32_t* infos_rf = flags + 2 + n_r;
    if (phase != 2) {
        const bool mc = M <= sober_chol_max_n() && j->probe_mc && j->probe_ws && (j->flags_bytes & 3) == 0 &&
                        j->probe_ws_bytes >= sober_cholesky_probe_mc_ws_bytes(M, n_r);
        if (mc) NX_TRY(sober::nystrom_flags_init(j->flags_block, j->flags_bytes, j->probe_ws, sober::probe_mc_flag_bytes(n_r),
                                                 flags + 2, n_r, stream));
        else NX_HIP(hipMemsetAsync(j->flags_block, 0, (size_t)j->flags_bytes, st));
        NX_TRY(sober_abs_sym_dmax(j->G, M, M, j->C, M, flags, pivots + n_r, stream));
        if (M > sober_chol_max_n()) {
            if (!j->probe_ws) return SOBER_E_ARG;
            NX_TRY(sober_cholesky_probe_batched(j->C, M, M, j->shifts, n_r, j->chol_work, flags + 2, pivots, j->probe_ws,
                                                j->probe_ws_bytes, stream));
        } else if (j->probe_mc) {
            if (!j->probe_ws) return SOBER_E_ARG;
            NX_TRY(sober::cholesky_probe_mc(j->C, M, M, j->shifts, n_r, j->chol_work, flags + 2, pivots, j->probe_ws,
                                            j->probe_ws_bytes, !mc, stream));
        } else {
            NX_TRY(sober_cholesky_probe_piv(j->C, M, M, j->shifts, n_r, j->chol_work, flags + 2, pivots, stream));
        }
        NX_TRY(sober_jitter_ladder_auto(j->C, M, M, flags + 2, n_r, flags + 1, stream));
    }
    if (phase == 1) return 0;
    const int last = 2 * niter;
    double *Q = j->Y[0], *free_buf = j->Y[1];
    NX_TRY(sober_dgemm(0, 0, M, s, M, 1.0, j->C, M, j->R, s, 0.0, Q, s, stream));
    NX_TRY(nx_orth(j, &Q, &free_buf, infos_rf, pivs_rf, 0, last > 0 ? 1 : 2, stream));
    int slot = 2, k = 0;
    for (int it = 0; it < niter; ++it) {
        for (int half = 0; half < 2; ++half) {
            ++k;
            NX_TRY(sober_dgemm(half == 0 ? 1 : 0, 0, M, s, M, 1.0, j->C, M, Q, s, 0.0, free_buf, s, stream));
            double* t = Q; Q = free_buf; free_buf = t;
            NX_TRY(nx_orth(j, &Q, &free_buf, infos_rf, pivs_rf, slot, (half == 1 && k == last) ? 2 : 1, stream));
            slot += 2;
        }
    }
    if (j->P && (j->T ? j->n_obs <= 0 : false)) return SOBER_E_ARG;
    const int ldp = M + (j->T ? j->n_obs : 0);
    NX_TRY(sober::transpose_projection(Q, s, M, j->mean_nys, j->Ut, j->P, ldp, stream));
    if (j->P && j->T) NX_TRY(sober_dgemm(0, 0, s, j->n_obs, M, -1.0, j->P, ldp, j->T, j->n_obs, 0.0, j->P + M, ldp, stream));
    NX_HIP(hipMemcpyAsync(j->h_flags_block, j->flags_block, (size_t)sober_nystrom_flags_bytes(n_r, niter),
                          hipMemcpyDeviceToHost, st));
    return 0;
}

extern "C" int sober_plan_rows(int kind, const double* X_nys, int M, int64_t ld_nys, const double* X_obs, int n_obs,
                               int64_t ld_obs, int d, const double* lengthscale, int ls_len, double outputscale,
                               const double* S_cache, int ld_s, double* rows, int dt, double* Kall, double* W, double* T,
                               double* G, void* stream) {
    if (!X_nys || !lengthscale || !rows || !G || M <= 0 || d <= 0 || n_obs < 0 || dt < d) return SOBER_E_ARG;
    if (kind != SOBER_KIND_RBF && kind != SOBER_KIND_MATERN52) return SOBER_E_ARG;
    if (n_obs == 0) {
        NX_TRY(sober_scale_points(X_nys, M, d, ld_nys, lengthscale, ls_len, rows, dt, stream));
        return sober_pairwise(kind, rows, nullptr, M, rows, nullptr, nullptr, M, dt, outputscale, G, M, stream);
    }
    if (!X_obs || !S_cache || !Kall || !W || !T || ld_s < n_obs) return SOBER_E_ARG;
    NX_TRY(sober::scale_points2(X_nys, M, ld_nys, X_obs, n_obs, ld_obs, d, lengthscale, ls_len, rows, dt, stream));
    NX_TRY(sober_pairwise(kind, rows, nullptr, (int64_t)M + n_obs, rows, nullptr, nullptr, M, dt, outputscale, Kall, M, stream));
    NX_TRY(sober_dgemm(0, 1, n_obs, n_obs, n_obs, 1.0, S_cache, ld_s, S_cache, ld_s, 0.0, W, n_obs, stream));
    const double* KXn = Kall + (size_t)M * M;
    NX_TRY(sober_dgemm(1, 0, M, n_obs, n_obs, 1.0, KXn, M, W, n_obs, 0.0, T, n_obs, stream));
    NX_HIP(hipMemcpyAsync(G, Kall, sizeof(double) * (size_t)M * M, hipMemcpyDeviceToDevice, (hipStream_t)stream));
    return sober_dgemm(0, 0, M, M, n_obs, -1.0, T, n_obs, KXn, M, 1.0, G, M, stream);
}
```

Baseline: 27.42 million.

## Fuse CholQR factor and triangular solve into one pass; fold copy into dgemm addend

Replaces the separate Cholesky-inverse and block-triangular-solve launches in the Nyström orthogonalisation with a single cholqr_pass kernel. On the final pass it can also carry out the transpose projection. Separately, the device-to-device copy of Kall before the rank update is removed by giving dgemm a distinct input addend (Cin). The aim is fewer kernel launches and less memory traffic in the Nyström/plan setup, at the cost of a larger fused kernel with more complex synchronisation.

```diff
diff --git a/include/sober_hip.h b/include/sober_hip.h
--- a/include/sober_hip.h
+++ b/include/sober_hip.h
@@ -7,7 +7,7 @@
 extern "C" {
 #endif
 
-#define SOBER_ABI_VERSION 7
+#define SOBER_ABI_VERSION 8
 
 #define SOBER_KIND_RBF       0
 #define SOBER_KIND_MATERN52  1
@@ -80,6 +80,9 @@
 int sober_dgemm(int transa, int transb, int m, int n, int k, double alpha,
                 const double* A, int lda, const double* B, int ldb,
                 double beta, double* C, int ldc, void* stream);
+int sober_dgemm_add(int transa, int transb, int m, int n, int k, double alpha,
+                    const double* A, int lda, const double* B, int ldb,
+                    double beta, const double* Cin, int ldcin, double* C, int ldc, void* stream);
 
 int sober_barycentres(const double* Xtr, int ldx, int n, int S, const double* tot,
                       double* X_tmp, void* stream);
@@ -155,6 +158,8 @@
                              double* ratio_out, void* stream);
 int sober_trsm_blocks(const double* Y, int64_t m, int q, int ldy, const double* L, int ldl, const double* Xinv,
                       double* Q, int ldq, void* stream);
+int sober_cholqr_pass(double* G, int q, int ldg, const double* Y, int64_t m, int ldy, double* Q, int ldq,
+                      int32_t* info, double* min_pivot, double* ratio, double* xinv, double* L, int ldl, void* stream);
 int sober_cholesky_probe(const double* src, int n, int ld_src, const double* shifts, int n_shifts,
                          double* work, int32_t* info, void* stream);
 int sober_cholesky_probe_piv(const double* src, int n, int ld_src, const double* shifts, int n_shifts,
diff --git a/sober_amd/_native.py b/sober_amd/_native.py
--- a/sober_amd/_native.py
+++ b/sober_amd/_native.py
@@ -8,7 +8,7 @@
 
 _HERE = os.path.dirname(os.path.abspath(__file__))
 LIB_PATH = os.environ.get("SOBER_HIP_LIB") or os.path.join(_HERE, "libsober_hip.so")
-ABI_VERSION = 7
+ABI_VERSION = 8
 
 KIND_RBF, KIND_MATERN52, KIND_TANIMOTO = 0, 1, 2
 KIND_BY_NAME = {"rbf": KIND_RBF, "matern52": KIND_MATERN52, "tanimoto": KIND_TANIMOTO}
@@ -51,6 +51,7 @@
                                        _vp, _i32, _i32, _vp, _i64, _vp]),
     "sober_sum_partials": (_i32, [_vp, _vp, _i32, _i32, _i32, _i32, _vp, _vp, _i32, _i32, _vp, _i32, _vp, _vp]),
     "sober_dgemm": (_i32, [_i32, _i32, _i32, _i32, _i32, _f64, _vp, _i32, _vp, _i32, _f64, _vp, _i32, _vp]),
+    "sober_dgemm_add": (_i32, [_i32, _i32, _i32, _i32, _i32, _f64, _vp, _i32, _vp, _i32, _f64, _vp, _i32, _vp, _i32, _vp]),
     "sober_barycentres": (_i32, [_vp, _i32, _i32, _i32, _vp, _vp, _vp]),
     "sober_level_update": (_i32, [_vp, _i64, _i64, _i32, _i64, _vp, _vp, _vp, _i32, _vp, _vp, _i64, _vp]),
     "sober_scatter_weights": (_i32, [_vp, _vp, _vp, _i32, _vp, _vp, _vp]),
@@ -88,6 +89,7 @@
     "sober_cholesky_inv": (_i32, [_vp, _i32, _i32, _f64, _vp, _vp, _vp, _vp]),
     "sober_cholesky_inv_ratio": (_i32, [_vp, _i32, _i32, _f64, _vp, _vp, _vp, _vp, _vp]),
     "sober_trsm_blocks": (_i32, [_vp, _i64, _i32, _i32, _vp, _i32, _vp, _vp, _i32, _vp]),
+    "sober_cholqr_pass": (_i32, [_vp, _i32, _i32, _vp, _i64, _i32, _vp, _i32, _vp, _vp, _vp, _vp, _vp, _i32, _vp]),
     "sober_cholesky_probe": (_i32, [_vp, _i32, _i32, _vp, _i32, _vp, _vp, _vp]),
     "sober_cholesky_probe_piv": (_i32, [_vp, _i32, _i32, _vp, _i32, _vp, _vp, _vp, _vp]),
     "sober_cholesky_probe_mc_ws_bytes": (_i64, [_i32, _i32]),
@@ -462,17 +464,24 @@
                                      G.stride(0), _ptr(tot), _stream(G)), "sober_sum_partials")
 
 
-def dgemm(A, B, C_, transa=False, transb=False, alpha=1.0, beta=0.0):
+def dgemm(A, B, C_, transa=False, transb=False, alpha=1.0, beta=0.0, Cin=None):
     m, n = C_.shape
     k = A.shape[0] if transa else A.shape[1]
-    for t, nm in ((A, "A"), (B, "B"), (C_, "C")):
-        if t.dtype != torch.float64 or t.stride(1) != 1:
+    if Cin is not None and Cin.shape != C_.shape:
+        raise SoberHipError(f"dgemm: addend {tuple(Cin.shape)} for a result {tuple(C_.shape)}")
+    for t, nm in ((A, "A"), (B, "B"), (C_, "C"), (Cin, "Cin")):
+        if t is not None and (t.dtype != torch.float64 or t.stride(1) != 1):
             raise SoberHipError(f"dgemm {nm}: need float64 with unit inner stride")
     ka = B.shape[1] if transb else B.shape[0]
     ma = A.shape[1] if transa else A.shape[0]
     na = B.shape[0] if transb else B.shape[1]
     if (ma, na, ka) != (m, n, k):
         raise SoberHipError(f"dgemm shape mismatch {A.shape} {B.shape} -> {C_.shape}")
+    if Cin is not None:
+        _check(load().sober_dgemm_add(int(transa), int(transb), m, n, k, float(alpha), A.data_ptr(), A.stride(0),
+                                      B.data_ptr(), B.stride(0), float(beta), Cin.data_ptr(), Cin.stride(0), C_.data_ptr(),
+                                      C_.stride(0), _stream(C_)), "sober_dgemm_add")
+        return
     _check(load().sober_dgemm(int(transa), int(transb), m, n, k, float(alpha), A.data_ptr(), A.stride(0),
                               B.data_ptr(), B.stride(0), float(beta), C_.data_ptr(), C_.stride(0),
                               _stream(C_)), "sober_dgemm")
@@ -619,6 +628,20 @@
     m, q = Y.shape
     _check(load().sober_trsm_blocks(Y.data_ptr(), m, q, Y.stride(0), L.data_ptr(), L.stride(0), xinv.data_ptr(),
                                     Q.data_ptr(), Q.stride(0), _stream(Y)), "sober_trsm_blocks")
+
+
+def cholqr_pass(G, Y, Q, info, min_pivot, xinv, ratio=None, L=None):
+    m, q = Y.shape
+    for t, nm in ((G, "G"), (Y, "Y"), (Q, "Q"), (L, "L")):
+        if t is not None and (t.dtype != torch.float64 or t.dim() != 2 or t.stride(1) != 1):
+            raise SoberHipError(f"cholqr_pass {nm}: need a float64 matrix with unit inner stride")
+    if G.shape != (q, q) or Q.shape != (m, q) or (L is not None and L.shape != (q, q)):
+        raise SoberHipError(f"cholqr_pass shape mismatch: G {tuple(G.shape)}, Y {tuple(Y.shape)}, Q {tuple(Q.shape)}")
+    if xinv.numel() < ((q + 31) // 32) * 1024:
+        raise SoberHipError("cholqr_pass: xinv too small")
+    _check(load().sober_cholqr_pass(G.data_ptr(), q, G.stride(0), Y.data_ptr(), m, Y.stride(0), Q.data_ptr(), Q.stride(0),
+                                    info.data_ptr(), _ptr(min_pivot), _ptr(ratio), xinv.data_ptr(), _ptr(L),
+                                    L.stride(0) if L is not None else 0, _stream(Y)), "sober_cholqr_pass")
 
 
 def cholesky_probe(src, shifts, work, info, min_pivot=None):
diff --git a/sober_amd/_ops_nystrom.py b/sober_amd/_ops_nystrom.py
--- a/sober_amd/_ops_nystrom.py
+++ b/sober_amd/_ops_nystrom.py
@@ -130,12 +130,10 @@
         for it in range(passes):
             Gm = torch.empty(q, q, dtype=torch.float64, device=self.device)
             nat.dgemm(Y, Y, Gm, transa=True)
-            Lc = Gm
             xinv = torch.empty(((q + 31) // 32) * 1024, dtype=torch.float64, device=self.device)
-            nat.cholesky_inv(Lc, 0.0, infos[slot + it:slot + it + 1], pivs[slot + it:slot + it + 1], xinv,
-                             ratio=pivs[slot + 1:slot + 2] if passes == 1 else None)
             Q = torch.empty_like(Y)
-            nat.trsm_blocks(Y, Lc, xinv, Q)
+            nat.cholqr_pass(Gm, Y, Q, infos[slot + it:slot + it + 1], pivs[slot + it:slot + it + 1], xinv,
+                            ratio=pivs[slot + 1:slot + 2] if passes == 1 else None)
             Y = Q
         return Y
 
diff --git a/sober_amd/_ops_plan.py b/sober_amd/_ops_plan.py
--- a/sober_amd/_ops_plan.py
+++ b/sober_amd/_ops_plan.py
@@ -161,8 +161,8 @@
             nat.pairwise(p.kind, nys.data, nys.norm, nys.data, nys.norm, None, p.M, nys.dt,
                          p.spec.outputscale, G)
             return G
-        G = p.Kall[:p.M].clone()
-        nat.dgemm(p.T, p.Kall[p.M:], G, alpha=-1.0, beta=1.0)
+        G = torch.empty(p.M, p.M, dtype=torch.float64, device=dev)
+        nat.dgemm(p.T, p.Kall[p.M:], G, alpha=-1.0, beta=1.0, Cin=p.Kall[:p.M])
         if p.weighted:
             G = p.mean_nys.unsqueeze(1) * G * p.mean_nys.unsqueeze(0)
         return G
diff --git a/sober_amd/csrc/chol.hip b/sober_amd/csrc/chol.hip
--- a/sober_amd/csrc/chol.hip
+++ b/sober_amd/csrc/chol.hip
@@ -24,7 +24,7 @@
 template <int NC>
 __device__ __attribute__((noinline)) void ch_diag_block_n(double* __restrict__ D, double* __restrict__ Xs, double* __restrict__ s_dinv,
                                               int* __restrict__ s_fail_p, double* __restrict__ s_minp_p, int nb, int kb,
-                                              int lane, double* __restrict__ xout) {
+                                              int lane, double* __restrict__ xout, int xld) {
     constexpr int LDP = CH_NB + 1;
     int& s_fail = *s_fail_p;
     double& s_minp = *s_minp_p;
@@ -42,8 +42,8 @@
                 v[c] = (xh | (i >= nb)) ? ((c == i) ? 1.0 : 0.0) : dv;
             }
             const bool xw = xout != nullptr && xh;
-            double* xo = xw ? xout + (size_t)(kb / CH_NB) * CH_NB * CH_NB : ch_sink;
-            const int xo_ld = xw ? CH_NB : 0, xo_i = xw ? i : lane;
+            double* xo = xw ? xout + (size_t)(kb / CH_NB) * CH_NB * xld : ch_sink;
+            const int xo_ld = xw ? xld : 0, xo_i = xw ? i : lane;
             double* const o_base = xh ? Xs + i : D + i * LDP;
             const int o_step = xh ? LDP : 1;
             int fail = 0;
@@ -83,13 +83,240 @@
 
 __device__ __forceinline__ void ch_diag_block(double* __restrict__ D, double* __restrict__ Xs, double* __restrict__ s_dinv,
                                               int* __restrict__ s_fail_p, double* __restrict__ s_minp_p, int nb, int kb,
-                                              int lane, double* __restrict__ xout) {
-    if (nb <= 8) ch_diag_block_n<8>(D, Xs, s_dinv, s_fail_p, s_minp_p, nb, kb, lane, xout);
-    else if (nb <= 16) ch_diag_block_n<16>(D, Xs, s_dinv, s_fail_p, s_minp_p, nb, kb, lane, xout);
-    else ch_diag_block_n<CH_NB>(D, Xs, s_dinv, s_fail_p, s_minp_p, nb, kb, lane, xout);
+                                              int lane, double* __restrict__ xout, int xld = CH_NB) {
+    if (nb <= 8) ch_diag_block_n<8>(D, Xs, s_dinv, s_fail_p, s_minp_p, nb, kb, lane, xout, xld);
+    else if (nb <= 16) ch_diag_block_n<16>(D, Xs, s_dinv, s_fail_p, s_minp_p, nb, kb, lane, xout, xld);
+    else ch_diag_block_n<CH_NB>(D, Xs, s_dinv, s_fail_p, s_minp_p, nb, kb, lane, xout, xld);
 }
 
 constexpr int CH_SMALLN = 120;
+struct ch_verdict {
+    int fail;
+    double minp;
+    double dm[CH_T / 64];
+};
+#ifdef CH_STAMPS
+#define CH_STAMP_PARAMS , long long (&st_t)[5], long long& st_last
+#define CH_STAMP_ARGS , st_t, st_last
+#else
+#define CH_STAMP_PARAMS
+#define CH_STAMP_ARGS
+#endif
+
+template <bool SMALL>
+__device__ __forceinline__ void ch_factor(double* A, int n, int ld, double shift, double* __restrict__ lds,
+                                          double* As, double* __restrict__ xout, int xld, bool want_dm,
+                                          ch_verdict* __restrict__ sh CH_STAMP_PARAMS) {
+    constexpr int LDP = CH_NB + 1;
+    double* D = lds;
+    double* Xs = lds + CH_NB * LDP;
+    constexpr int LDPP = CH_LDPP;
+    double* P = lds + 2 * CH_NB * LDP;
+    double* const A_glob = A;
+    const int ld_glob = ld;
+    int& s_fail = sh->fail;
+    double& s_minp = sh->minp;
+    double* const s_dinv = nullptr;
+    double* const s_dm = sh->dm;
+    const int tid = threadIdx.x, lane = tid & 63, wave = tid >> 6;
+    const int li = lane & 15, lk = lane >> 4;
+    if (tid == 0) { s_fail = 0; s_minp = __builtin_inf(); }
+    if (want_dm) {
+        double dl = -__builtin_inf();
+        for (int i = tid; i < n; i += CH_T) dl = fmax(dl, A_glob[(size_t)i * ld_glob + i] + shift);
+#pragma unroll
+        for (int o = 32; o > 0; o >>= 1) dl = fmax(dl, __shfl_xor(dl, o, 64));
+        if (lane == 0) s_dm[wave] = dl;
+    }
+    __syncthreads();
+    bool ahead0 = false;
+    if constexpr (SMALL) {
+        const int nb0 = min(CH_NB, n);
+#pragma unroll
+        for (int t = tid; t < CH_NB * CH_NB; t += CH_T) {
+            const int i = t >> 5, j = t & 31;
+            double v = (i < nb0 && j <= i) ? A_glob[(size_t)i * ld_glob + j] : 0.0;
+            if (i == j && i < nb0) v += shift;
+            D[i * LDP + j] = v;
+        }
+        __syncthreads();
+        if (wave == 0) {
+            ch_diag_block(D, Xs, s_dinv, &s_fail, &s_minp, nb0, 0, lane, xout, xld);
+        } else {
+            for (int i = wave - 1; i < n; i += CH_T / 64 - 1)
+                for (int j = lane; j <= i; j += 64) As[i * (n + 1) + j] = A_glob[(size_t)i * ld_glob + j];
+        }
+        A = As;
+        ld = n + 1;
+        __syncthreads();
+        ahead0 = true;
+    }
+#ifdef CH_STAMPS
+    st_last = wall_clock64();
+#define CH_STAMP(K) { const long long now_ = wall_clock64(); st_t[K] += now_ - st_last; st_last = now_; }
+#else
+#define CH_STAMP(K)
+#endif
+
+    bool ahead = ahead0;
+    for (int kb = 0; kb < n; kb += CH_NB) {
+        const int nb = min(CH_NB, n - kb);
+        const int nr = n - kb - nb;
+        if (!ahead) {
+#pragma unroll
+            for (int t = tid; t < CH_NB * CH_NB; t += CH_T) {
+                const int i = t >> 5, j = t & 31;
+                double v = (i < nb && j <= i) ? A[(size_t)(kb + i) * ld + kb + j] : 0.0;
+                if (i == j && i < nb) v += shift;
+                D[i * LDP + j] = v;
+            }
+            __syncthreads();
+            CH_STAMP(0)
+            if (wave == 0) ch_diag_block(D, Xs, s_dinv, &s_fail, &s_minp, nb, kb, lane, xout, xld);
+            __syncthreads();
+            CH_STAMP(1)
+        }
+        if (s_fail != 0) break;
+#pragma unroll
+        for (int t = tid; t < CH_NB * CH_NB; t += CH_T) {
+            const int i = t >> 5, j = t & 31;
+            if (i < nb && j <= i) A[(size_t)(kb + i) * ld + kb + j] = D[i * LDP + j];
+        }
+        if (nr == 0) break;
+        {
+            const int ntile = (nr + 15) / 16;
+            double af[8], an[8];
+            if (wave < ntile) {
+                const double* arow = A + (size_t)(kb + nb + min(wave * 16 + li, nr - 1)) * ld + kb;
+#pragma unroll
+                for (int u = 0; u < 8; ++u) af[u] = arow[min(4 * u + lk, nb - 1)];
+            }
+            for (int t = wave; t < ntile; t += CH_T / 64) {
+                const int r0 = t * 16;
+                {
+                    const int tn = min(t + CH_T / 64, ntile - 1);
+                    const double* arow = A + (size_t)(kb + nb + min(tn * 16 + li, nr - 1)) * ld + kb;
+#pragma unroll
+                    for (int u = 0; u < 8; ++u) an[u] = arow[min(4 * u + lk, nb - 1)];
+                }
+                ch_double4 acc0 = (ch_double4){0.0, 0.0, 0.0, 0.0}, acc1 = acc0;
+#pragma unroll
+                for (int u = 0; u < 8; ++u) {
+                    const int k = 4 * u + lk;
+                    const double a = (k < nb) ? af[u] : 0.0;
+                    acc0 = __builtin_amdgcn_mfma_f64_16x16x4f64(a, Xs[li * LDP + k], acc0, 0, 0, 0);
+                    acc1 = __builtin_amdgcn_mfma_f64_16x16x4f64(a, Xs[(16 + li) * LDP + k], acc1, 0, 0, 0);
+                }
+#pragma unroll
+                for (int r = 0; r < 4; ++r) {
+                    const int row = r0 + lk + 4 * r;
+                    if (row < nr) {
+                        P[row * LDPP + li] = acc0[r];
+                        P[row * LDPP + 16 + li] = acc1[r];
+                    }
+                }
+#pragma unroll
+                for (int u = 0; u < 8; ++u) af[u] = an[u];
+            }
+        }
+        __syncthreads();
+        CH_STAMP(2)
+        for (int r = tid >> 5; r < nr; r += CH_T / 32) {
+            const int j = tid & 31;
+            if (j < nb) A[(size_t)(kb + nb + r) * ld + kb + j] = P[r * LDPP + j];
+        }
+        {
+            const int nt = (nr + 15) / 16;
+            const int wv = __builtin_amdgcn_readfirstlane(wave);
+            const bool look = nt * (nt + 1) / 2 >= 8;
+            const int t_step = look ? (wv == 0 ? 1 : CH_T / 64 - 1) : CH_T / 64;
+            const int nt_mine = (look && wv == 0) ? min(nt, 2) : nt;
+            int ntr = 0, ntc = look ? (wv == 0 ? 0 : 2 + wv) : wv;
+            while (ntc > ntr) { ntc -= ntr + 1; ++ntr; }
+            int tr[CH_G], tc[CH_G], trn[CH_G], tcn[CH_G];
+            double cv[CH_G][4], cn[CH_G][4];
+            double* const a22 = A + (size_t)(kb + nb) * ld + kb + nb;
+#define CH_TAKE(R, C)                                                       \
+            { R = ntr; C = ntc; ntc += t_step; while (ntc > ntr) { ntc -= ntr + 1; ++ntr; } }
+#define CH_LOAD(DST, R, C)                                                  \
+            _Pragma("unroll") for (int e = 0; e < 4; ++e)                   \
+                DST[e] = a22[(size_t)min((R) * 16 + lk + 4 * e, nr - 1) * ld + min((C) * 16 + li, nr - 1)];
+#pragma unroll
+            for (int g = 0; g < CH_G; ++g) { CH_TAKE(tr[g], tc[g]) CH_LOAD(cv[g], tr[g], tc[g]) }
+            while (tr[0] < nt_mine) {
+#pragma unroll
+                for (int g = 0; g < CH_G; ++g) { CH_TAKE(trn[g], tcn[g]) CH_LOAD(cn[g], trn[g], tcn[g]) }
+                ch_double4 acc[CH_G][2];
+#pragma unroll
+                for (int g = 0; g < CH_G; ++g) {
+                    acc[g][0] = (ch_double4){0.0, 0.0, 0.0, 0.0};
+                    acc[g][1] = acc[g][0];
+                    const int ra = min(tr[g] * 16 + li, nr - 1), rb = min(tc[g] * 16 + li, nr - 1);
+#pragma unroll
+                    for (int u = 0; u < 8; u += 2) {
+                        acc[g][0] = __builtin_amdgcn_mfma_f64_16x16x4f64(P[ra * LDPP + 4 * u + lk],
+                                                                         P[rb * LDPP + 4 * u + lk], acc[g][0], 0, 0, 0);
+                        acc[g][1] = __builtin_amdgcn_mfma_f64_16x16x4f64(P[ra * LDPP + 4 * u + 4 + lk],
+                                                                         P[rb * LDPP + 4 * u + 4 + lk], acc[g][1], 0, 0, 0);
+                    }
+                }
+#pragma unroll
+                for (int g = 0; g < CH_G; ++g) {
+#pragma unroll
+                    for (int e = 0; e < 4; ++e) {
+                        const int row = tr[g] * 16 + lk + 4 * e, col = tc[g] * 16 + li;
+                        double* dst = (row < nr && col <= row && tr[g] < nt_mine) ? a22 + (size_t)row * ld + col : ch_sink + tid;
+                        *dst = cv[g][e] - (acc[g][0][e] + acc[g][1][e]);
+                    }
+                }
+#pragma unroll
+                for (int g = 0; g < CH_G; ++g) {
+                    tr[g] = trn[g]; tc[g] = tcn[g];
+#pragma unroll
+                    for (int e = 0; e < 4; ++e) cv[g][e] = cn[g][e];
+                }
+            }
+#undef CH_TAKE
+#undef CH_LOAD
+            if (look && wave == 0) {
+                __builtin_amdgcn_s_waitcnt(0);
+                const int kb2 = kb + nb, nb2 = min(CH_NB, n - kb2);
+#pragma unroll
+                for (int t = lane; t < CH_NB * CH_NB; t += 64) {
+                    const int i = t >> 5, j = t & 31;
+                    double v = (i < nb2 && j <= i) ? A[(size_t)(kb2 + i) * ld + kb2 + j] : 0.0;
+                    if (i == j && i < nb2) v += shift;
+                    D[i * LDP + j] = v;
+                }
+                __builtin_amdgcn_wave_barrier();
+                ch_diag_block(D, Xs, s_dinv, &s_fail, &s_minp, nb2, kb2, lane, xout, xld);
+            }
+            ahead = look;
+        }
+        __threadfence_block();
+        __syncthreads();
+        CH_STAMP(3)
+    }
+}
+
+__device__ __forceinline__ void ch_report(const ch_verdict* __restrict__ sh, int32_t* __restrict__ info,
+                                          double* __restrict__ min_pivot, double* __restrict__ ratio_out) {
+    *info = sh->fail;
+    if (min_pivot) *min_pivot = sh->minp;
+    if (ratio_out) {
+        double dm = sh->dm[0];
+#pragma unroll
+        for (int w = 1; w < CH_T / 64; ++w) dm = fmax(dm, sh->dm[w]);
+        *ratio_out = sh->minp / dm;
+    }
+}
+
+__device__ __forceinline__ void ch_store_factor(const double* __restrict__ As, int n, double* __restrict__ L, int ldl,
+                                                int w0, int nw, int lane) {
+    for (int i = w0; i < n; i += nw)
+        for (int j = lane; j <= i; j += 64) L[(size_t)i * ldl + j] = As[i * (n + 1) + j];
+}
+
 template <bool SMALL>
 __global__ __launch_bounds__(CH_T) void k_chol(double* __restrict__ A, int n, int ld, double shift,
                                               int32_t* __restrict__ info, double* __restrict__ min_pivot,
@@ -107,222 +334,26 @@
         __threadfence_block();
         __syncthreads();
     }
-    constexpr int LDP = CH_NB + 1;
-    double* D = lds;
-    double* Xs = lds + CH_NB * LDP;
-    constexpr int LDPP = CH_LDPP;
-    double* P = lds + 2 * CH_NB * LDP;
-    double* const A_glob = A;
-    const int ld_glob = ld;
+    __shared__ ch_verdict sh;
+    const int tid = threadIdx.x;
     double* As = nullptr;
-    if constexpr (SMALL) {
-        As = P + (size_t)(n > CH_NB ? n - CH_NB : 0) * LDPP;
-    }
-    __shared__ int s_fail;
-    __shared__ double s_minp;
-    __shared__ double s_dinv[CH_NB];
-    const int tid = threadIdx.x, lane = tid & 63, wave = tid >> 6;
-    const int li = lane & 15, lk = lane >> 4;
-    if (tid == 0) { s_fail = 0; s_minp = __builtin_inf(); }
-    __shared__ double s_dm[CH_T / 64];
-    if (ratio_out != nullptr) {
-        double dl = -__builtin_inf();
-        for (int i = tid; i < n; i += CH_T) dl = fmax(dl, A_glob[(size_t)i * ld_glob + i] + shift);
-#pragma unroll
-        for (int o = 32; o > 0; o >>= 1) dl = fmax(dl, __shfl_xor(dl, o, 64));
-        if (lane == 0) s_dm[wave] = dl;
-    }
-    __syncthreads();
-    bool ahead0 = false;
-    if constexpr (SMALL) {
-        const int nb0 = min(CH_NB, n);
-#pragma unroll
-        for (int t = tid; t < CH_NB * CH_NB; t += CH_T) {
-            const int i = t >> 5, j = t & 31;
-            double v = (i < nb0 && j <= i) ? A_glob[(size_t)i * ld_glob + j] : 0.0;
-            if (i == j && i < nb0) v += shift;
-            D[i * LDP + j] = v;
-        }
-        __syncthreads();
-        if (wave == 0) {
-            ch_diag_block(D, Xs, s_dinv, &s_fail, &s_minp, nb0, 0, lane, xout);
-        } else {
-            for (int i = wave - 1; i < n; i += CH_T / 64 - 1)
-                for (int j = lane; j <= i; j += 64) As[i * (n + 1) + j] = A_glob[(size_t)i * ld_glob + j];
-        }
-        A = As;
-        ld = n + 1;
-        __syncthreads();
-        ahead0 = true;
-    }
+    if constexpr (SMALL) As = lds + 2 * CH_NB * (CH_NB + 1) + (size_t)(n > CH_NB ? n - CH_NB : 0) * CH_LDPP;
 #ifdef CH_STAMPS
-    long long st_t[5] = {0, 0, 0, 0, 0}, st_last = wall_clock64();
-#define CH_STAMP(K) { const long long now_ = wall_clock64(); st_t[K] += now_ - st_last; st_last = now_; }
-#else
-#define CH_STAMP(K)
+    long long st_t[5] = {0, 0, 0, 0, 0}, st_last = 0;
 #endif
-
-    bool ahead = ahead0;
-    for (int kb = 0; kb < n; kb += CH_NB) {
-        const int nb = min(CH_NB, n - kb);
-        const int nr = n - kb - nb;
-        if (!ahead) {
-#pragma unroll
-            for (int t = tid; t < CH_NB * CH_NB; t += CH_T) {
-                const int i = t >> 5, j = t & 31;
-                double v = (i < nb && j <= i) ? A[(size_t)(kb + i) * ld + kb + j] : 0.0;
-                if (i == j && i < nb) v += shift;
-                D[i * LDP + j] = v;
-            }
-            __syncthreads();
-            CH_STAMP(0)
-            if (wave == 0) ch_diag_block(D, Xs, s_dinv, &s_fail, &s_minp, nb, kb, lane, xout);
-            __syncthreads();
-            CH_STAMP(1)
-        }
-        if (s_fail != 0) break;
-#pragma unroll
-        for (int t = tid; t < CH_NB * CH_NB; t += CH_T) {
-            const int i = t >> 5, j = t & 31;
-            if (i < nb && j <= i) A[(size_t)(kb + i) * ld + kb + j] = D[i * LDP + j];
-        }
-        if (nr == 0) break;
-        {
-            const int ntile = (nr + 15) / 16;
-            double af[8], an[8];
-            if (wave < ntile) {
-                const double* arow = A + (size_t)(kb + nb + min(wave * 16 + li, nr - 1)) * ld + kb;
-#pragma unroll
-                for (int u = 0; u < 8; ++u) af[u] = arow[min(4 * u + lk, nb - 1)];
-            }
-            for (int t = wave; t < ntile; t += CH_T / 64) {
-                const int r0 = t * 16;
-                {
-                    const int tn = min(t + CH_T / 64, ntile - 1);
-                    const double* arow = A + (size_t)(kb + nb + min(tn * 16 + li, nr - 1)) * ld + kb;
-#pragma unroll
-                    for (int u = 0; u < 8; ++u) an[u] = arow[min(4 * u + lk, nb - 1)];
-                }
-                ch_double4 acc0 = (ch_double4){0.0, 0.0, 0.0, 0.0}, acc1 = acc0;
-#pragma unroll
-                for (int u = 0; u < 8; ++u) {
-                    const int k = 4 * u + lk;
-                    const double a = (k < nb) ? af[u] : 0.0;
-                    acc0 = __builtin_amdgcn_mfma_f64_16x16x4f64(a, Xs[li * LDP + k], acc0, 0, 0, 0);
-                    acc1 = __builtin_amdgcn_mfma_f64_16x16x4f64(a, Xs[(16 + li) * LDP + k], acc1, 0, 0, 0);
-                }
-#pragma unroll
-                for (int r = 0; r < 4; ++r) {
-                    const int row = r0 + lk + 4 * r;
-                    if (row < nr) {
-                        P[row * LDPP + li] = acc0[r];
-                        P[row * LDPP + 16 + li] = acc1[r];
-                    }
-                }
-#pragma unroll
-                for (int u = 0; u < 8; ++u) af[u] = an[u];
-            }
-        }
-        __syncthreads();
-        CH_STAMP(2)
-        for (int r = tid >> 5; r < nr; r += CH_T / 32) {
-            const int j = tid & 31;
-            if (j < nb) A[(size_t)(kb + nb + r) * ld + kb + j] = P[r * LDPP + j];
-        }
-        {
-            const int nt = (nr + 15) / 16;
-            const int wv = __builtin_amdgcn_readfirstlane(wave);
-            const bool look = nt * (nt + 1) / 2 >= 8;
-            const int t_step = look ? (wv == 0 ? 1 : CH_T / 64 - 1) : CH_T / 64;
-            const int nt_mine = (look && wv == 0) ? min(nt, 2) : nt;
-            int ntr = 0, ntc = look ? (wv == 0 ? 0 : 2 + wv) : wv;
-            while (ntc > ntr) { ntc -= ntr + 1; ++ntr; }
-            int tr[CH_G], tc[CH_G], trn[CH_G], tcn[CH_G];
-            double cv[CH_G][4], cn[CH_G][4];
-            double* const a22 = A + (size_t)(kb + nb) * ld + kb + nb;
-#define CH_TAKE(R, C)                                                       \
-            { R = ntr; C = ntc; ntc += t_step; while (ntc > ntr) { ntc -= ntr + 1; ++ntr; } }
-#define CH_LOAD(DST, R, C)                                                  \
-            _Pragma("unroll") for (int e = 0; e < 4; ++e)                   \
-                DST[e] = a22[(size_t)min((R) * 16 + lk + 4 * e, nr - 1) * ld + min((C) * 16 + li, nr - 1)];
-#pragma unroll
-            for (int g = 0; g < CH_G; ++g) { CH_TAKE(tr[g], tc[g]) CH_LOAD(cv[g], tr[g], tc[g]) }
-            while (tr[0] < nt_mine) {
-#pragma unroll
-                for (int g = 0; g < CH_G; ++g) { CH_TAKE(trn[g], tcn[g]) CH_LOAD(cn[g], trn[g], tcn[g]) }
-                ch_double4 acc[CH_G][2];
-#pragma unroll
-                for (int g = 0; g < CH_G; ++g) {
-                    acc[g][0] = (ch_double4){0.0, 0.0, 0.0, 0.0};
-                    acc[g][1] = acc[g][0];
-                    const int ra = min(tr[g] * 16 + li, nr - 1), rb = min(tc[g] * 16 + li, nr - 1);
-#pragma unroll
-                    for (int u = 0; u < 8; u += 2) {
-                        acc[g][0] = __builtin_amdgcn_mfma_f64_16x16x4f64(P[ra * LDPP + 4 * u + lk],
-                                                                         P[rb * LDPP + 4 * u + lk], acc[g][0], 0, 0, 0);
-                        acc[g][1] = __builtin_amdgcn_mfma_f64_16x16x4f64(P[ra * LDPP + 4 * u + 4 + lk],
-                                                                         P[rb * LDPP + 4 * u + 4 + lk], acc[g][1], 0, 0, 0);
-                    }
-                }
-#pragma unroll
-                for (int g = 0; g < CH_G; ++g) {
-#pragma unroll
-                    for (int e = 0; e < 4; ++e) {
-                        const int row = tr[g] * 16 + lk + 4 * e, col = tc[g] * 16 + li;
-                        double* dst = (row < nr && col <= row && tr[g] < nt_mine) ? a22 + (size_t)row * ld + col : ch_sink + tid;
-                        *dst = cv[g][e] - (acc[g][0][e] + acc[g][1][e]);
-                    }
-                }
-#pragma unroll
-                for (int g = 0; g < CH_G; ++g) {
-                    tr[g] = trn[g]; tc[g] = tcn[g];
-#pragma unroll
-                    for (int e = 0; e < 4; ++e) cv[g][e] = cn[g][e];
-                }
-            }
-#undef CH_TAKE
-#undef CH_LOAD
-            if (look && wave == 0) {
-                __builtin_amdgcn_s_waitcnt(0);
-                const int kb2 = kb + nb, nb2 = min(CH_NB, n - kb2);
-#pragma unroll
-                for (int t = lane; t < CH_NB * CH_NB; t += 64) {
-                    const int i = t >> 5, j = t & 31;
-                    double v = (i < nb2 && j <= i) ? A[(size_t)(kb2 + i) * ld + kb2 + j] : 0.0;
-                    if (i == j && i < nb2) v += shift;
-                    D[i * LDP + j] = v;
-                }
-                __builtin_amdgcn_wave_barrier();
-                ch_diag_block(D, Xs, s_dinv, &s_fail, &s_minp, nb2, kb2, lane, xout);
-            }
-            ahead = look;
-        }
-        __threadfence_block();
-        __syncthreads();
-        CH_STAMP(3)
-    }
+    ch_factor<SMALL>(A, n, ld, shift, lds, As, xout, CH_NB, ratio_out != nullptr, &sh CH_STAMP_ARGS);
     if constexpr (SMALL) {
         __syncthreads();
-        for (int i = tid >> 6; i < n; i += CH_T / 64)
-            for (int j = tid & 63; j <= i; j += 64) A_glob[(size_t)i * ld_glob + j] = A[i * (n + 1) + j];
+        ch_store_factor(As, n, A, ld, tid >> 6, CH_T / 64, tid & 63);
     }
 #ifdef CH_STAMPS
     {
         CH_STAMP(4)
         if (tid == 0 && n >= 16)
-            for (int k = 0; k < 5; ++k) A_glob[8 + k] = (double)st_t[k];
+            for (int k = 0; k < 5; ++k) A[8 + k] = (double)st_t[k];
     }
 #endif
-    if (tid == 0) {
-        *info = s_fail;
-        if (min_pivot) *min_pivot = s_minp;
-        if (ratio_out) {
-            double dm = s_dm[0];
-#pragma unroll
-            for (int w = 1; w < CH_T / 64; ++w) dm = fmax(dm, s_dm[w]);
-            *ratio_out = s_minp / dm;
-        }
-    }
+    if (tid == 0) ch_report(&sh, info, min_pivot, ratio_out);
 }
 
 constexpr int CM_G = 8;
@@ -670,69 +701,135 @@
 }
 
 constexpr int TB_WAVES = 2;
+__host__ __device__ constexpr int tb_wave_doubles(int q) { return 16 * (((q + 31) / 32) * 32 + 4) + 16 * 36; }
+
+template <int xld, bool TR>
+__device__ __forceinline__ void tb_solve_rows(const double* __restrict__ Y, int64_t m, int q, int ldy,
+                                              const double* __restrict__ L, int ldl, const double* __restrict__ Xinv,
+                                              double* __restrict__ Q, int ldq, double* __restrict__ stash, int64_t R0, int lane,
+                                              double* __restrict__ Ut, double* __restrict__ P, int ldp,
+                                              const double* __restrict__ mean) {
+    const int li = lane & 15, lk = lane >> 4;
+    const int qpad = ((q + 31) / 32) * 32, LS = qpad + 4;
+    double* tbuf = stash + 16 * LS;
+    const int nblk = qpad / 32;
+    for (int jb = 0; jb < nblk; ++jb) {
+        const int c0 = 32 * jb;
+        ch_double4 acc[2];
+#pragma unroll
+        for (int jt = 0; jt < 2; ++jt)
+#pragma unroll
+            for (int r = 0; r < 4; ++r) {
+                const int64_t row = min(R0 + lk + 4 * r, m - 1);
+                const int col = c0 + 16 * jt + li;
+                const double v = Y[row * ldy + min(col, q - 1)];
+                acc[jt][r] = (col < q) ? v : 0.0;
+            }
+        for (int kb = 0; kb < jb; ++kb) {
+#pragma unroll
+            for (int u = 0; u < 8; ++u) {
+                const int kc = 32 * kb + 4 * u + lk;
+                const double a = -stash[li * LS + kc];
+#pragma unroll
+                for (int jt = 0; jt < 2; ++jt) {
+                    const int lr = c0 + 16 * jt + li;
+                    const double b = L[(size_t)min(lr, q - 1) * ldl + kc];
+                    acc[jt] = __builtin_amdgcn_mfma_f64_16x16x4f64(a, (lr < q) ? b : 0.0, acc[jt], 0, 0, 0);
+                }
+            }
+        }
+#pragma unroll
+        for (int jt = 0; jt < 2; ++jt)
+#pragma unroll
+            for (int r = 0; r < 4; ++r) tbuf[(lk + 4 * r) * 36 + 16 * jt + li] = acc[jt][r];
+        __builtin_amdgcn_wave_barrier();
+        const double* X = Xinv + (size_t)jb * 32 * xld;
+        ch_double4 out[2] = {(ch_double4){0.0, 0.0, 0.0, 0.0}, (ch_double4){0.0, 0.0, 0.0, 0.0}};
+#pragma unroll
+        for (int u = 0; u < 8; ++u) {
+            const double a = tbuf[li * 36 + 4 * u + lk];
+#pragma unroll
+            for (int jt = 0; jt < 2; ++jt)
+                out[jt] = __builtin_amdgcn_mfma_f64_16x16x4f64(a, X[(16 * jt + li) * xld + 4 * u + lk], out[jt], 0, 0, 0);
+        }
+        __builtin_amdgcn_wave_barrier();
+#pragma unroll
+        for (int jt = 0; jt < 2; ++jt)
+#pragma unroll
+            for (int r = 0; r < 4; ++r) {
+                const int64_t row = R0 + lk + 4 * r;
+                const int col = c0 + 16 * jt + li;
+                stash[(lk + 4 * r) * LS + col] = out[jt][r];
+                if (row < m && col < q) {
+                    const double v = out[jt][r];
+                    Q[row * ldq + col] = v;
+                    if constexpr (TR) {
+                        Ut[(size_t)col * m + row] = v;
+                        if (P != nullptr) P[(size_t)col * ldp + row] = mean ? v * mean[row] : v;
+                    }
+                }
+            }
+        __builtin_amdgcn_wave_barrier();
+    }
+}
+
 __global__ __launch_bounds__(TB_WAVES * 64) void k_trsm_blocks(const double* __restrict__ Y, int64_t m, int q, int ldy,
                                                               const double* __restrict__ L, int ldl,
                                                               const double* __restrict__ Xinv,
                                                               double* __restrict__ Q, int ldq) {
     extern __shared__ double tb_lds[];
     const int lane = threadIdx.x & 63, wave = threadIdx.x >> 6;
-    const int li = lane & 15, lk = lane >> 4;
-    const int qpad = ((q + 31) / 32) * 32, LS = qpad + 4;
-    double* stash = tb_lds + (size_t)wave * (16 * LS + 16 * 36);
-    double* tbuf = stash + 16 * LS;
+    double* stash = tb_lds + (size_t)wave * tb_wave_doubles(q);
     const int64_t R0 = ((int64_t)blockIdx.x * TB_WAVES + wave) * 16;
     if (R0 >= m) return;
-    const int nblk = qpad / 32;
-    for (int jb = 0; jb < nblk; ++jb) {
-        const int c0 = 32 * jb;
-        ch_double4 acc[2];
-#pragma unroll
-        for (int jt = 0; jt < 2; ++jt)
-#pragma unroll
-            for (int r = 0; r < 4; ++r) {
-                const int64_t row = min(R0 + lk + 4 * r, m - 1);
-                const int col = c0 + 16 * jt + li;
-                const double v = Y[row * ldy + min(col, q - 1)];
-                acc[jt][r] = (col < q) ? v : 0.0;
-            }
-        for (int kb = 0; kb < jb; ++kb) {
-#pragma unroll
-            for (int u = 0; u < 8; ++u) {
-                const int kc = 32 * kb + 4 * u + lk;
-                const double a = -stash[li * LS + kc];
-#pragma unroll
-                for (int jt = 0; jt < 2; ++jt) {
-                    const int lr = c0 + 16 * jt + li;
-                    const double b = L[(size_t)min(lr, q - 1) * ldl + kc];
-                    acc[jt] = __builtin_amdgcn_mfma_f64_16x16x4f64(a, (lr < q) ? b : 0.0, acc[jt], 0, 0, 0);
-                }
-            }
-        }
-#pragma unroll
-        for (int jt = 0; jt < 2; ++jt)
-#pragma unroll
-            for (int r = 0; r < 4; ++r) tbuf[(lk + 4 * r) * 36 + 16 * jt + li] = acc[jt][r];
-        __builtin_amdgcn_wave_barrier();
-        const double* X = Xinv + (size_t)jb * 32 * 32;
-        ch_double4 out[2] = {(ch_double4){0.0, 0.0, 0.0, 0.0}, (ch_double4){0.0, 0.0, 0.0, 0.0}};
-#pragma unroll
-        for (int u = 0; u < 8; ++u) {
-            const double a = tbuf[li * 36 + 4 * u + lk];
-#pragma unroll
-            for (int jt = 0; jt < 2; ++jt)
-                out[jt] = __builtin_amdgcn_mfma_f64_16x16x4f64(a, X[(16 * jt + li) * 32 + 4 * u + lk], out[jt], 0, 0, 0);
-        }
-        __builtin_amdgcn_wave_barrier();
-#pragma unroll
-        for (int jt = 0; jt < 2; ++jt)
-#pragma unroll
-            for (int r = 0; r < 4; ++r) {
-                const int64_t row = R0 + lk + 4 * r;
-                const int col = c0 + 16 * jt + li;
-                stash[(lk + 4 * r) * LS + col] = out[jt][r];
-                if (row < m && col < q) Q[row * ldq + col] = out[jt][r];
-            }
-        __builtin_amdgcn_wave_barrier();
+    tb_solve_rows<32, false>(Y, m, q, ldy, L, ldl, Xinv, Q, ldq, stash, R0, lane, nullptr, nullptr, 0, nullptr);
+}
+
+constexpr int CS_XLD = CH_LDPP;
+struct cs_layout { int as_off, x_off, total; };
+__host__ __device__ inline cs_layout cs_lds_layout(int q) {
+    const int nr = q > CH_NB ? q - CH_NB : 0;
+    const int fac = 2 * CH_NB * (CH_NB + 1) + nr * CH_LDPP;
+    const int sol = TB_WAVES * tb_wave_doubles(q);
+    cs_layout l;
+    l.as_off = fac > sol ? fac : sol;
+    l.x_off = l.as_off + q * (q + 1);
+    l.total = l.x_off + ((q + CH_NB - 1) / CH_NB) * CH_NB * CS_XLD;
+    return l;
+}
+
+template <bool TR>
+__global__ __launch_bounds__(CH_T) void k_chol_solve(const double* __restrict__ G, int q, int ldg,
+                                                    const double* __restrict__ Y, int64_t m, int ldy,
+                                                    double* __restrict__ Q, int ldq, int32_t* __restrict__ info,
+                                                    double* __restrict__ min_pivot, double* __restrict__ ratio_out,
+                                                    double* __restrict__ xinv, double* __restrict__ Lout, int ldl,
+                                                    double* __restrict__ Ut, double* __restrict__ P, int ldp,
+                                                    const double* __restrict__ mean) {
+    extern __shared__ double lds[];
+    __shared__ ch_verdict sh;
+    const cs_layout lay = cs_lds_layout(q);
+    double* const As = lds + lay.as_off;
+    double* const Xall = lds + lay.x_off;
+    const int tid = threadIdx.x, lane = tid & 63, wave = __builtin_amdgcn_readfirstlane(tid >> 6);
+#ifdef CH_STAMPS
+    long long st_t[5] = {0, 0, 0, 0, 0}, st_last = 0;
+#endif
+    ch_factor<true>(const_cast<double*>(G), q, ldg, 0.0, lds, As, Xall, CS_XLD, ratio_out != nullptr, &sh CH_STAMP_ARGS);
+    __syncthreads();
+    if (wave < TB_WAVES) {
+        const int64_t R0 = ((int64_t)blockIdx.x * TB_WAVES + wave) * 16;
+        if (R0 < m)
+            tb_solve_rows<CS_XLD, TR>(Y, m, q, ldy, As, q + 1, Xall, Q, ldq, lds + (size_t)wave * tb_wave_doubles(q), R0, lane,
+                                      Ut, P, ldp, mean);
+    } else if (blockIdx.x == 0) {
+        constexpr int NW = CH_T / 64 - TB_WAVES;
+        if (Lout != nullptr) ch_store_factor(As, q, Lout, ldl, wave - TB_WAVES, NW, lane);
+        const int nblk = (q + CH_NB - 1) / CH_NB;
+        const int nx = sh.fail != 0 ? (sh.fail - 1) / CH_NB + 1 : nblk;
+        for (int t = (wave - TB_WAVES) * 64 + lane; t < nx * CH_NB * CH_NB; t += NW * 64)
+            xinv[t] = Xall[(t >> 5) * CS_XLD + (t & 31)];
+        if (tid == TB_WAVES * 64) ch_report(&sh, info, min_pivot, ratio_out);
     }
 }
 
@@ -1015,6 +1112,56 @@
     return 0;
 }
 
+int sober::cholqr_pass(double* G, int q, int ldg, const double* Y, int64_t m, int ldy, double* Q, int ldq, int32_t* info,
+                       double* min_pivot, double* ratio, double* xinv, double* L, int ldl, double* Ut, double* P, int ldp,
+                       const double* mean, void* stream) {
+    if (!G || !Y || !Q || !info || !xinv || q <= 0 || m <= 0 || ldg < q || ldy < q || ldq < q || Y == Q) return SOBER_E_ARG;
+    if (L != nullptr && (L == G || ldl < q)) return SOBER_E_ARG;
+    if ((P != nullptr && (!Ut || ldp < m)) || (Ut != nullptr && m > 0x7fffffff)) return SOBER_E_ARG;
+    if (q > sober::CH_MAXN) return SOBER_E_DIM;
+    const sober::cs_layout lay = sober::cs_lds_layout(q);
+    const int64_t groups = ((m + 15) / 16 + sober::TB_WAVES - 1) / sober::TB_WAVES;
+    if (q <= sober::CH_SMALLN && (size_t)lay.total * sizeof(double) <= (size_t)160 * 1024 - 512 && groups <= 0x7fffffff) {
+        static std::atomic<unsigned long long> attr_set{0};
+        if (sober_attr_needed(attr_set)) {
+            HIP_TRY(hipFuncSetAttribute((const void*)sober::k_chol_solve<false>, hipFuncAttributeMaxDynamicSharedMemorySize,
+                                        160 * 1024 - 512));
+            HIP_TRY(hipFuncSetAttribute((const void*)sober::k_chol_solve<true>, hipFuncAttributeMaxDynamicSharedMemorySize,
+                                        160 * 1024 - 512));
+            sober_attr_done(attr_set);
+        }
+        if (Ut != nullptr)
+            hipLaunchKernelGGL(sober::k_chol_solve<true>, dim3((unsigned)groups), dim3(sober::CH_T), (size_t)lay.total * sizeof(double),
+                               (hipStream_t)stream, (const double*)G, q, ldg, Y, m, ldy, Q, ldq, info, min_pivot, ratio, xinv, L,
+                               ldl, Ut, P, ldp, mean);
+        else
+            hipLaunchKernelGGL(sober::k_chol_solve<false>, dim3((unsigned)groups), dim3(sober::CH_T), (size_t)lay.total * sizeof(double),
+                               (hipStream_t)stream, (const double*)G, q, ldg, Y, m, ldy, Q, ldq, info, min_pivot, ratio, xinv, L,
+                               ldl, Ut, P, ldp, mean);
+        LAUNCH_CHECK();
+        return 0;
+    }
+    int rc = sober_cholesky_inv_ratio(G, q, ldg, 0.0, info, min_pivot, xinv, ratio, stream);
+    if (rc != 0) return rc;
+    rc = sober_trsm_blocks(Y, m, q, ldy, G, ldg, xinv, Q, ldq, stream);
+    if (rc != 0) return rc;
+    if (L != nullptr)
+        HIP_TRY(hipMemcpy2DAsync(L, (size_t)ldl * sizeof(double), G, (size_t)ldg * sizeof(double), (size_t)q * sizeof(double),
+                                 (size_t)q, hipMemcpyDeviceToDevice, (hipStream_t)stream));
+    if (Ut != nullptr) {
+        if (ldq != q) return SOBER_E_ARG;
+        return sober::transpose_projection(Q, q, (int)m, mean, Ut, P, ldp, stream);
+    }
+    return 0;
+}
+
+extern "C" int sober_cholqr_pass(double* G, int q, int ldg, const double* Y, int64_t m, int ldy, double* Q, int ldq,
+                                 int32_t* info, double* min_pivot, double* ratio, double* xinv, double* L, int ldl,
+                                 void* stream) {
+    return sober::cholqr_pass(G, q, ldg, Y, m, ldy, Q, ldq, info, min_pivot, ratio, xinv, L, ldl, nullptr, nullptr, 0, nullptr,
+                              stream);
+}
+
 extern "C" int sober_cholesky_probe_piv(const double* src, int n, int ld_src, const double* shifts, int n_shifts,
                                         double* work, int32_t* info, double* min_pivot, void* stream);
 extern "C" int sober_cholesky_probe(const double* src, int n, int ld_src, const double* shifts, int n_shifts,
diff --git a/sober_amd/csrc/dgemm.hip b/sober_amd/csrc/dgemm.hip
--- a/sober_amd/csrc/dgemm.hip
+++ b/sober_amd/csrc/dgemm.hip
@@ -15,7 +15,7 @@
 __global__ __launch_bounds__(256) void k_dgemm(int transa, int transb, int m, int n, int k,
                                                double alpha, const double* __restrict__ A, int lda,
                                                const double* __restrict__ B, int ldb, double beta,
-                                               double* __restrict__ C, int ldc,
+                                               const double* Cin, int ldcin, double* C, int ldc,
                                                const double* __restrict__ coldiv, double* __restrict__ Ct, int ldct) {
     __shared__ double red[SPLIT == 4 ? 3 * 256 : 1];
     const int wave = threadIdx.x >> 6, lane = threadIdx.x & 63;
@@ -71,8 +71,7 @@
             if (Ct != nullptr) {
                 Ct[(size_t)col * ldct + row] = coldiv ? v / coldiv[col] : v;
             } else {
-                double* c = C + (size_t)row * ldc + col;
-                *c = (beta == 0.0) ? v : fma(beta, *c, v);
+                C[(size_t)row * ldc + col] = (beta == 0.0) ? v : fma(beta, Cin[(size_t)row * ldcin + col], v);
             }
         }
     }
@@ -80,23 +79,29 @@
 
 }
 
-extern "C" int sober_dgemm(int transa, int transb, int m, int n, int k, double alpha, const double* A,
-                           int lda, const double* B, int ldb, double beta, double* C, int ldc,
-                           void* stream) {
-    if (!A || !B || !C || m <= 0 || n <= 0 || k <= 0) return SOBER_E_ARG;
-    if (lda < (transa ? m : k) || ldb < (transb ? k : n) || ldc < n) return SOBER_E_ARG;
+extern "C" int sober_dgemm_add(int transa, int transb, int m, int n, int k, double alpha, const double* A,
+                               int lda, const double* B, int ldb, double beta, const double* Cin, int ldcin,
+                               double* C, int ldc, void* stream) {
+    if (!A || !B || !C || !Cin || m <= 0 || n <= 0 || k <= 0) return SOBER_E_ARG;
+    if (lda < (transa ? m : k) || ldb < (transb ? k : n) || ldc < n || ldcin < n) return SOBER_E_ARG;
     const long tiles = (long)((n + 15) / 16) * ((m + 15) / 16);
     if (tiles <= 2048 && k >= 64) {
         dim3 grid((n + 15) / 16, (m + 15) / 16);
         hipLaunchKernelGGL(sober::k_dgemm<4>, grid, dim3(256), 0, (hipStream_t)stream, transa, transb, m, n, k,
-                           alpha, A, lda, B, ldb, beta, C, ldc, (const double*)nullptr, (double*)nullptr, 0);
+                           alpha, A, lda, B, ldb, beta, Cin, ldcin, C, ldc, (const double*)nullptr, (double*)nullptr, 0);
     } else {
         dim3 grid((n + 31) / 32, (m + 31) / 32);
         hipLaunchKernelGGL(sober::k_dgemm<1>, grid, dim3(256), 0, (hipStream_t)stream, transa, transb, m, n, k,
-                           alpha, A, lda, B, ldb, beta, C, ldc, (const double*)nullptr, (double*)nullptr, 0);
+                           alpha, A, lda, B, ldb, beta, Cin, ldcin, C, ldc, (const double*)nullptr, (double*)nullptr, 0);
     }
     LAUNCH_CHECK();
     return 0;
+}
+
+extern "C" int sober_dgemm(int transa, int transb, int m, int n, int k, double alpha, const double* A,
+                           int lda, const double* B, int ldb, double beta, double* C, int ldc,
+                           void* stream) {
+    return sober_dgemm_add(transa, transb, m, n, k, alpha, A, lda, B, ldb, beta, C, ldc, C, ldc, stream);
 }
 
 extern "C" int sober_dgemm_coldiv_t(int m, int n, int k, const double* A, int lda, const double* B, int ldb,
@@ -106,11 +111,11 @@
     if (tiles <= 2048 && k >= 64) {
         dim3 grid((n + 15) / 16, (m + 15) / 16);
         hipLaunchKernelGGL(sober::k_dgemm<4>, grid, dim3(256), 0, (hipStream_t)stream, 0, 0, m, n, k, 1.0, A, lda, B, ldb,
-                           0.0, (double*)nullptr, 0, coldiv, Ct, ldct);
+                           0.0, (const double*)nullptr, 0, (double*)nullptr, 0, coldiv, Ct, ldct);
     } else {
         dim3 grid((n + 31) / 32, (m + 31) / 32);
         hipLaunchKernelGGL(sober::k_dgemm<1>, grid, dim3(256), 0, (hipStream_t)stream, 0, 0, m, n, k, 1.0, A, lda, B, ldb,
-                           0.0, (double*)nullptr, 0, coldiv, Ct, ldct);
+                           0.0, (const double*)nullptr, 0, (double*)nullptr, 0, coldiv, Ct, ldct);
     }
     LAUNCH_CHECK();
     return 0;
diff --git a/sober_amd/csrc/internal.hpp b/sober_amd/csrc/internal.hpp
--- a/sober_amd/csrc/internal.hpp
+++ b/sober_amd/csrc/internal.hpp
@@ -14,6 +14,10 @@
 int cholesky_probe_mc(const double* src, int n, int ld_src, const double* shifts, int n_shifts, double* work, int32_t* info,
                       double* min_pivot, void* ws, int64_t ws_bytes, bool init, void* stream);
 
+int cholqr_pass(double* G, int q, int ldg, const double* Y, int64_t m, int ldy, double* Q, int ldq, int32_t* info,
+                double* min_pivot, double* ratio, double* xinv, double* L, int ldl, double* Ut, double* P, int ldp,
+                const double* mean, void* stream);
+
 int orth_merge(int32_t* info, double* piv, double* ratio, const int32_t* info2, const double* piv2, const double* ratio2, void* stream);
 
 }
diff --git a/sober_amd/csrc/nystrom_exec.cpp b/sober_amd/csrc/nystrom_exec.cpp
--- a/sober_amd/csrc/nystrom_exec.cpp
+++ b/sober_amd/csrc/nystrom_exec.cpp
@@ -40,16 +40,18 @@
 }
 
 static int nx_orth(const sober_nystrom_job* j, double** Y, double** other, int32_t* infos, double* pivs, int slot,
-                   int passes, void* stream) {
+                   int passes, int ldp, void* stream) {
     const int M = j->M, s = j->s;
     for (int it = 0; it < passes; ++it) {
+        const bool fin = ldp > 0 && it == passes - 1;
         if (s > sober_chol_max_n()) {
             NX_TRY(nx_orth_halves(j, *Y, *other, infos + slot + it, pivs + slot + it, passes == 1 ? pivs + slot + 1 : nullptr, stream));
+            if (fin) NX_TRY(sober::transpose_projection(*other, s, M, j->mean_nys, j->Ut, j->P, ldp, stream));
         } else {
             NX_TRY(sober_dgemm(1, 0, s, s, M, 1.0, *Y, s, *Y, s, 0.0, j->Gm, s, stream));
-            NX_TRY(sober_cholesky_inv_ratio(j->Gm, s, s, 0.0, infos + slot + it, pivs + slot + it, j->xinv,
-                                            passes == 1 ? pivs + slot + 1 : nullptr, stream));
-            NX_TRY(sober_trsm_blocks(*Y, M, s, s, j->Gm, s, j->xinv, *other, s, stream));
+            NX_TRY(sober::cholqr_pass(j->Gm, s, s, *Y, M, s, *other, s, infos + slot + it, pivs + slot + it,
+                                      passes == 1 ? pivs + slot + 1 : nullptr, j->xinv, nullptr, 0, fin ? j->Ut : nullptr,
+                                      fin ? j->P : nullptr, ldp, j->mean_nys, stream));
         }
         double* t = *Y; *Y = *other; *other = t;
     }
@@ -93,22 +95,22 @@
     }
     if (phase == 1) return 0;
     const int last = 2 * niter;
+    if (j->P && (j->T ? j->n_obs <= 0 : false)) return SOBER_E_ARG;
+    const int ldp = M + (j->T ? j->n_obs : 0);
     double *Q = j->Y[0], *free_buf = j->Y[1];
     NX_TRY(sober_dgemm(0, 0, M, s, M, 1.0, j->C, M, j->R, s, 0.0, Q, s, stream));
-    NX_TRY(nx_orth(j, &Q, &free_buf, infos_rf, pivs_rf, 0, last > 0 ? 1 : 2, stream));
+    NX_TRY(nx_orth(j, &Q, &free_buf, infos_rf, pivs_rf, 0, last > 0 ? 1 : 2, last > 0 ? 0 : ldp, stream));
     int slot = 2, k = 0;
     for (int it = 0; it < niter; ++it) {
         for (int half = 0; half < 2; ++half) {
             ++k;
             NX_TRY(sober_dgemm(half == 0 ? 1 : 0, 0, M, s, M, 1.0, j->C, M, Q, s, 0.0, free_buf, s, stream));
             double* t = Q; Q = free_buf; free_buf = t;
-            NX_TRY(nx_orth(j, &Q, &free_buf, infos_rf, pivs_rf, slot, (half == 1 && k == last) ? 2 : 1, stream));
+            const bool fin = half == 1 && k == last;
+            NX_TRY(nx_orth(j, &Q, &free_buf, infos_rf, pivs_rf, slot, fin ? 2 : 1, fin ? ldp : 0, stream));
             slot += 2;
         }
     }
-    if (j->P && (j->T ? j->n_obs <= 0 : false)) return SOBER_E_ARG;
-    const int ldp = M + (j->T ? j->n_obs : 0);
-    NX_TRY(sober::transpose_projection(Q, s, M, j->mean_nys, j->Ut, j->P, ldp, stream));
     if (j->P && j->T) NX_TRY(sober_dgemm(0, 0, s, j->n_obs, M, -1.0, j->P, ldp, j->T, j->n_obs, 0.0, j->P + M, ldp, stream));
     NX_HIP(hipMemcpyAsync(j->h_flags_block, j->flags_block, (size_t)sober_nystrom_flags_bytes(n_r, niter),
                           hipMemcpyDeviceToHost, st));
@@ -131,6 +133,5 @@
     NX_TRY(sober_dgemm(0, 1, n_obs, n_obs, n_obs, 1.0, S_cache, ld_s, S_cache, ld_s, 0.0, W, n_obs, stream));
     const double* KXn = Kall + (size_t)M * M;
     NX_TRY(sober_dgemm(1, 0, M, n_obs, n_obs, 1.0, KXn, M, W, n_obs, 0.0, T, n_obs, stream));
-    NX_HIP(hipMemcpyAsync(G, Kall, sizeof(double) * (size_t)M * M, hipMemcpyDeviceToDevice, (hipStream_t)stream));
-    return sober_dgemm(0, 0, M, M, n_obs, -1.0, T, n_obs, KXn, M, 1.0, G, M, stream);
+    return sober_dgemm_add(0, 0, M, M, n_obs, -1.0, T, n_obs, KXn, M, 1.0, Kall, M, G, M, stream);
 }
```

After: 27.74 million (median of 6 runs). 1.01x the previous value.
